# AIDynamicAction/rcognita

Measured on AMD Instinct MI355X. Metric: env-control-steps/sec (whole node), 3wrobot Nactor=10, higher is better.
Workload: dtype f64

## Files before the change

### include/rcg.h

```cpp
#ifndef RCG_H
#define RCG_H

#include <stdint.h>

#ifdef __cplusplus
extern "C" {
#endif

#define RCG_VERSION 124

#define RCG_MAX_DS 5
#define RCG_MAX_DU 2
#define RCG_MAX_CHI 7
#define RCG_MAX_PARS 5
#define RCG_MAX_DC 35
#define RCG_MAX_ROW 64
#define RCG_MAX_NACTOR 4096

typedef enum rcg_status {
  RCG_OK = 0,
  RCG_ERR_BAD_ARG = -1,
  RCG_ERR_HIP = -2,
  RCG_ERR_NO_DEVICE = -3,
  RCG_ERR_UNSUPPORTED = -4,
  RCG_ERR_NONFINITE = -5
} rcg_status;

typedef enum rcg_system { RCG_SYS_3WROBOT = 0, RCG_SYS_3WROBOT_NI = 1, RCG_SYS_2TANK = 2 } rcg_system;
#define RCG_SYS_USER_BASE 16
typedef enum rcg_mode { RCG_MODE_MPC = 0, RCG_MODE_RQL = 1, RCG_MODE_SQL = 2 } rcg_mode;
typedef enum rcg_stage { RCG_STAGE_QUADRATIC = 0, RCG_STAGE_BIQUADRATIC = 1 } rcg_stage;
typedef enum rcg_critic_struct {
  RCG_CRITIC_QUAD_LIN = 0,
  RCG_CRITIC_QUADRATIC = 1,
  RCG_CRITIC_QUAD_NOMIX = 2,
  RCG_CRITIC_QUAD_MIX = 3
} rcg_critic_struct;
typedef enum rcg_dtype { RCG_F32 = 0, RCG_F64 = 1 } rcg_dtype;
typedef enum rcg_where { RCG_HOST = 0, RCG_DEVICE = 1 } rcg_where;

#define RCG_FLAG_HAS_TARGET 0x1
#define RCG_FLAG_PER_ENV_PARS 0x2
#define RCG_FLAG_REF_LAG 0x4
#define RCG_FLAG_ACCUM_EVERY_SUBSTEP 0x8
#define RCG_FLAG_NO_CLIP 0x10
#define RCG_FLAG_DISTURB 0x20

typedef enum rcg_field {
  RCG_FIELD_STATE = 0,
  RCG_FIELD_ACTION = 1,
  RCG_FIELD_ACCUM = 2,
  RCG_FIELD_STEP_IDX = 3,
  RCG_FIELD_EPISODE_IDX = 4,
  RCG_FIELD_STATUS = 5,
  RCG_FIELD_PARS = 6,
  RCG_FIELD_STATE_INIT = 7,
  RCG_FIELD_STATE_PREV = 8,
  RCG_FIELD_BEST_J = 9,
  RCG_FIELD_BEST_IDX = 10,
  RCG_FIELD_W_CRITIC = 11,
  RCG_FIELD_W_PREV = 12,
  RCG_FIELD_OBS_BUF = 13,
  RCG_FIELD_ACT_BUF = 14,
  RCG_FIELD_RETURNS = 15,
  RCG_FIELD_ACTION_SQN = 16,
  RCG_FIELD_DISTURB = 17,
  RCG_FIELD_SUBSTEP_IDX = 18,
  RCG_FIELD_COUNT_ = 19
} rcg_field;

typedef struct rcg_cfg {
  int32_t struct_size;
  int32_t sys_id;
  int32_t batch;
  int32_t dtype;
  int32_t device;
  int32_t n_actor;
  int32_t mode;
  int32_t stage_obj_struct;
  int32_t critic_struct;
  int32_t n_critic;
  int32_t buffer_size;
  int32_t substeps_per_tick;
  int32_t flags;
  int32_t critic_every_ticks;
  double dt_sim;
  double sampling_time;
  double pred_step_size;
  double gamma;
  double pars[8];
  double ctrl_bnds[4];
  double R1[49];
  double R2[49];
  double target[8];
  double action_init[4];
  double w_init[40];
  double w_min[40];
  double w_max[40];
  double pars_disturb[6];
  double disturb_init[2];
  uint64_t seed;
  int64_t env_id_base;
} rcg_cfg;

typedef struct rcg_summary {
  double count;
  double sum;
  double sumsq;
  double min;
  double max;
  double n_failed;
} rcg_summary;

typedef struct rcg_handle rcg_handle;

int rcg_version(void);
const char* rcg_last_error(const rcg_handle* h);
int rcg_device_count(void);

int rcg_register_system(const char* name, const char* policy_src, int32_t ds, int32_t du, int32_t np, int32_t* sys_id);
int rcg_rtc_version(int32_t* major, int32_t* minor);
int rcg_system_info(int32_t sys_id, int32_t* ds, int32_t* du, int32_t* np, int32_t* has_jac);
int rcg_system_output_info(int32_t sys_id, int32_t* dy, int32_t* has_out, int32_t* has_out_jac);
int rcg_system_has_critic(int32_t sys_id, int32_t* has_critic);
int rcg_system_has_search(int32_t sys_id, int32_t* has_search);
int rcg_system_programs(int32_t sys_id, char* buf, int64_t cap, int64_t* need);

int rcg_create(const rcg_cfg* cfg, rcg_handle** out);
int rcg_destroy(rcg_handle* h);
int rcg_set_stream(rcg_handle* h, void* hip_stream);
int rcg_use_own_stream(rcg_handle* h);
int rcg_wait_stream(rcg_handle* h, void* producer_stream);
int rcg_release_stream(rcg_handle* h, void* consumer_stream);
int rcg_synchronize(rcg_handle* h);

int rcg_dev_alloc(rcg_handle* h, uint64_t bytes, void** dev_out);
int rcg_dev_free(rcg_handle* h, void* dev);
int rcg_memcpy_h2d(rcg_handle* h, void* dev_dst, const void* host_src, uint64_t bytes);
int rcg_memcpy_d2h(rcg_handle* h, void* host_dst, const void* dev_src, uint64_t bytes);

int rcg_set_field(rcg_handle* h, int field, const void* src, int where);
int rcg_get_field(rcg_handle* h, int field, void* dst, int where);
int64_t rcg_field_bytes(const rcg_handle* h, int field);
int rcg_field_ptr(rcg_handle* h, int field, void** dev_out);

int rcg_rhs(rcg_handle* h, const void* state, const void* action, void* dstate, void* clipped_action,
            int32_t n, int32_t clip);
int rcg_rhs_full(rcg_handle* h, const void* state, const void* disturb, const void* action, const void* xi,
                 void* dstate, void* ddisturb, void* clipped_action, int32_t n, int32_t clip);
int rcg_disturb_noise(rcg_handle* h, void* bits_out, void* xi_out);
int rcg_stage_obj(rcg_handle* h, const void* obs, const void* act, void* out, int32_t n);
int rcg_out(rcg_handle* h, const void* state, void* obs, int32_t n);
int rcg_critic(rcg_handle* h, const void* obs, const void* act, const void* w, void* out, int32_t n);
int rcg_actor_cost(rcg_handle* h, const void* cand, int32_t K, const void* obs, const void* state_sys,
                   const void* w, void* J);
int rcg_critic_cost(rcg_handle* h, const void* w, void* Jc);

int rcg_sim_step(rcg_handle* h, int32_t n_substeps);
int rcg_sim_step_h(rcg_handle* h, int32_t n_substeps, double step);
#define RCG_LOOP_DECIDE 1
#define RCG_LOOP_PUSH 2
#define RCG_LOOP_FIT 4
int rcg_loop_step(rcg_handle* h, const double* action_in, double step_h, int32_t n_substeps, int32_t flags, int32_t iters,
                  double* out);
int rcg_loop_step_begin(rcg_handle* h, const double* action_in, double step_h, int32_t n_substeps, int32_t flags, int32_t iters);
int rcg_loop_step_end(rcg_handle* h, double* out);
int rcg_actor_argmin(rcg_handle* h, const void* cand, int32_t K, const void* obs, const void* state_sys,
                     void* action, void* best_J, int32_t* best_idx);
int rcg_control_tick(rcg_handle* h, const void* cand, int32_t K);
int rcg_control_ticks(rcg_handle* h, int32_t T, int32_t K);
int rcg_control_tick_n(rcg_handle* h, const void* cand, int32_t K, int32_t T);
int rcg_set_tick_parts(rcg_handle* h, int32_t parts);
int rcg_join(rcg_handle* h);
int rcg_actor_optimize(rcg_handle* h, int32_t iters, const void* obs, const void* state_sys, const void* u_init,
                       void* u_opt, void* action, void* best_J, int32_t* n_iter);
int rcg_set_optimizer(rcg_handle* h, int32_t memory);
int rcg_set_optimizer_tol(rcg_handle* h, double ftol);
int rcg_control_tick_opt(rcg_handle* h, int32_t iters, int32_t warm_start);
int rcg_actor_search(rcg_handle* h, int32_t K, int32_t rounds, const void* obs, const void* state_sys, const void* centre,
                     void* u_best, void* action, void* best_J, int32_t* best_idx);
int rcg_control_tick_search(rcg_handle* h, int32_t K, int32_t rounds, int32_t warm_start);
int rcg_candidates_sample(rcg_handle* h, void* cand, int32_t K, int32_t round, const void* centre);
int rcg_nominal_action(rcg_handle* h, const void* obs, void* action, void* lyap, int32_t n, double ctrl_gain,
                       const double* ctrl_pars, int32_t clip);
int rcg_nominal_theta(rcg_handle* h, const void* obs, void* theta, int32_t n);
int rcg_control_tick_nominal(rcg_handle* h, double ctrl_gain, const double* ctrl_pars);
int rcg_critic_update(rcg_handle* h, int32_t do_fit);
int rcg_critic_fit(rcg_handle* h);
int rcg_episode_reset(rcg_handle* h);
int rcg_episode_stats(rcg_handle* h, int32_t from_accum, void* returns_out, rcg_summary* out);

int64_t rcg_tick_count(const rcg_handle* h);
int rcg_set_tick_count(rcg_handle* h, int64_t ticks);

typedef enum rcg_kernel { RCG_KERNEL_ACTOR = 0, RCG_KERNEL_SIM = 1, RCG_KERNEL_CRITIC = 2, RCG_KERNEL_COUNT_ = 3 } rcg_kernel;
#define RCG_PROFILE_PAUSE 0x80
int rcg_profile(rcg_handle* h, int32_t kernel_mask);
int rcg_profile_read(rcg_handle* h, int32_t kernel, double* total_ms, int64_t* launches);
int rcg_profile_samples(rcg_handle* h, int32_t kernel, double* ms_out, int64_t cap, int64_t* n_out);

typedef enum rcg_kernel_id {
  RCG_KID_NONE = 0,
  RCG_KID_ACTOR = 1,
  RCG_KID_ACTOR_DMA = 2,
  RCG_KID_TICKS = 3,
  RCG_KID_ACTOR_OPT = 4,
  RCG_KID_NOMINAL = 5,
  RCG_KID_SIM = 6,
  RCG_KID_SIM_V = 7,
  RCG_KID_SIM_DIST = 8,
  RCG_KID_CRITIC_FIT = 9,
  RCG_KID_ACTOR_DMA_PACKED = 10,
  RCG_KID_ACTOR_SEARCH = 11,
  RCG_KID_COUNT_ = 12
} rcg_kernel_id;
int rcg_last_launch(const rcg_handle* h, int32_t kind, int32_t* kernel_id, int32_t* variant, int32_t* envs_per_wave);
int rcg_last_launch_zero_w(const rcg_handle* h, int32_t kind, uint32_t* mask);
const char* rcg_kernel_name(int32_t kernel_id);

#ifdef __cplusplus
}
#endif
#endif
```

### rcognita_amd/_native.py

```python
from __future__ import annotations

import ctypes as C
import os
import sys

_HERE = os.path.dirname(os.path.abspath(__file__))
LIB_PATH = os.path.join(_HERE, "lib", "librcg.so")

RCG_VERSION = 124
OK, ERR_BAD_ARG, ERR_HIP, ERR_NO_DEVICE, ERR_UNSUPPORTED, ERR_NONFINITE = 0, -1, -2, -3, -4, -5
SYS_3WROBOT, SYS_3WROBOT_NI, SYS_2TANK = 0, 1, 2
MODE_MPC, MODE_RQL, MODE_SQL = 0, 1, 2
STAGE_QUADRATIC, STAGE_BIQUADRATIC = 0, 1
CRITIC_QUAD_LIN, CRITIC_QUADRATIC, CRITIC_QUAD_NOMIX, CRITIC_QUAD_MIX = 0, 1, 2, 3
F32, F64 = 0, 1
HOST, DEVICE = 0, 1
FLAG_HAS_TARGET, FLAG_PER_ENV_PARS, FLAG_REF_LAG, FLAG_ACCUM_EVERY_SUBSTEP, FLAG_NO_CLIP = 1, 2, 4, 8, 16
FLAG_DISTURB = 32
DIM_DISTURB = {0: 2, 1: 2, 2: 1}

(FIELD_STATE, FIELD_ACTION, FIELD_ACCUM, FIELD_STEP_IDX, FIELD_EPISODE_IDX, FIELD_STATUS, FIELD_PARS,
 FIELD_STATE_INIT, FIELD_STATE_PREV, FIELD_BEST_J, FIELD_BEST_IDX, FIELD_W_CRITIC, FIELD_W_PREV, FIELD_OBS_BUF,
 FIELD_ACT_BUF, FIELD_RETURNS, FIELD_ACTION_SQN, FIELD_DISTURB, FIELD_SUBSTEP_IDX) = range(19)
FIELD_COUNT = 19

MODE_IDS = {"MPC": MODE_MPC, "RQL": MODE_RQL, "SQL": MODE_SQL}
STAGE_IDS = {"quadratic": STAGE_QUADRATIC, "biquadratic": STAGE_BIQUADRATIC}
CRITIC_IDS = {"quad-lin": CRITIC_QUAD_LIN, "quadratic": CRITIC_QUADRATIC, "quad-nomix": CRITIC_QUAD_NOMIX,
              "quad-mix": CRITIC_QUAD_MIX}
SYS_IDS = {"3wrobot": SYS_3WROBOT, "3wrobotNI": SYS_3WROBOT_NI, "2tank": SYS_2TANK}
SYS_DIMS = {SYS_3WROBOT: (5, 2, 2), SYS_3WROBOT_NI: (3, 2, 0), SYS_2TANK: (2, 1, 5)}
SYS_DY = {}
SYS_USER_BASE = 16
MAX_DS, MAX_DU, MAX_PARS = 5, 2, 5

SYMBOLS = [
    "rcg_version", "rcg_last_error", "rcg_device_count", "rcg_create", "rcg_destroy", "rcg_set_stream", "rcg_use_own_stream",
    "rcg_synchronize", "rcg_dev_alloc", "rcg_dev_free", "rcg_memcpy_h2d", "rcg_memcpy_d2h", "rcg_set_field",
    "rcg_get_field", "rcg_field_bytes", "rcg_field_ptr", "rcg_rhs", "rcg_stage_obj", "rcg_critic",
    "rcg_actor_cost", "rcg_critic_cost", "rcg_sim_step", "rcg_sim_step_h", "rcg_actor_argmin", "rcg_control_tick",
    "rcg_critic_update", "rcg_control_ticks", "rcg_control_tick_n", "rcg_actor_optimize", "rcg_control_tick_opt", "rcg_nominal_action",
    "rcg_control_tick_nominal", "rcg_rhs_full", "rcg_disturb_noise", "rcg_episode_reset", "rcg_episode_stats", "rcg_tick_count", "rcg_set_tick_count", "rcg_profile", "rcg_profile_read",
    "rcg_profile_samples", "rcg_last_launch", "rcg_kernel_name", "rcg_wait_stream", "rcg_nominal_theta", "rcg_set_optimizer", "rcg_set_optimizer_tol", "rcg_set_tick_parts", "rcg_join", "rcg_loop_step", "rcg_loop_step_begin", "rcg_loop_step_end",
    "rcg_actor_search", "rcg_control_tick_search", "rcg_candidates_sample", "rcg_release_stream",
    "rcg_register_system", "rcg_rtc_version", "rcg_system_info", "rcg_system_output_info", "rcg_out",
    "rcg_system_has_critic", "rcg_system_programs", "rcg_critic_fit", "rcg_last_launch_zero_w", "rcg_system_has_search",
]
KERNEL_ACTOR, KERNEL_SIM, KERNEL_CRITIC = 0, 1, 2
(KID_NONE, KID_ACTOR, KID_ACTOR_DMA, KID_TICKS, KID_ACTOR_OPT, KID_NOMINAL, KID_SIM, KID_SIM_V, KID_SIM_DIST,
 KID_CRITIC_FIT, KID_ACTOR_DMA_PACKED, KID_ACTOR_SEARCH) = range(12)
DMA_MPC_G1, DMA_MPC, DMA_RQL_0, DMA_SQL_0 = 0, 1, 2, 6
LOOP_DECIDE, LOOP_PUSH, LOOP_FIT = 1, 2, 4
DMA_RQL_GEN_0 = 12
DMA_MPC_GEND, DMA_MPC_GENF = 10, 11


class RcgCfg(C.Structure):

    _fields_ = [
        ("struct_size", C.c_int32), ("sys_id", C.c_int32), ("batch", C.c_int32), ("dtype", C.c_int32),
        ("device", C.c_int32), ("n_actor", C.c_int32), ("mode", C.c_int32), ("stage_obj_struct", C.c_int32),
        ("critic_struct", C.c_int32), ("n_critic", C.c_int32), ("buffer_size", C.c_int32),
        ("substeps_per_tick", C.c_int32), ("flags", C.c_int32), ("critic_every_ticks", C.c_int32),
        ("dt_sim", C.c_double), ("sampling_time", C.c_double), ("pred_step_size", C.c_double), ("gamma", C.c_double),
        ("pars", C.c_double * 8), ("ctrl_bnds", C.c_double * 4), ("R1", C.c_double * 49), ("R2", C.c_double * 49),
        ("target", C.c_double * 8), ("action_init", C.c_double * 4), ("w_init", C.c_double * 40),
        ("w_min", C.c_double * 40), ("w_max", C.c_double * 40),
        ("pars_disturb", C.c_double * 6), ("disturb_init", C.c_double * 2), ("seed", C.c_uint64),
        ("env_id_base", C.c_int64),
    ]


class RcgSummary(C.Structure):
    _fields_ = [("count", C.c_double), ("sum", C.c_double), ("sumsq", C.c_double), ("min", C.c_double),
                ("max", C.c_double), ("n_failed", C.c_double)]


class NativeError(RuntimeError):
    def __init__(self, code, msg):
        super().__init__(f"librcg error {code}: {msg}")
        self.code = code


_lib = None


def use_library(path):
    global LIB_PATH
    if _lib is not None:
        raise RuntimeError("use_library: librcg is already loaded")
    LIB_PATH = os.path.abspath(path)


def lib():
    global _lib
    if _lib is not None:
        return _lib
    if not os.path.exists(LIB_PATH):
        raise ImportError(
            f"{LIB_PATH} not found: build the HIP library first (`make lib` at the repo root, or "
            "`python -c 'import __graft_entry__ as g; g.build()'`).  rcognita_amd has no CPU fallback."
        )
    torch = sys.modules.get("torch")
    if torch is not None and torch.cuda.is_available() and not torch.cuda.is_initialized():
        torch.cuda.init()
    L = C.CDLL(LIB_PATH)
    vp, i32, i64, u64 = C.c_void_p, C.c_int32, C.c_int64, C.c_uint64
    sig = {
        "rcg_version": (C.c_int, []),
        "rcg_last_error": (C.c_char_p, [vp]),
        "rcg_device_count": (C.c_int, []),
        "rcg_create": (C.c_int, [C.POINTER(RcgCfg), C.POINTER(vp)]),
        "rcg_destroy": (C.c_int, [vp]),
        "rcg_set_stream": (C.c_int, [vp, vp]),
        "rcg_use_own_stream": (C.c_int, [vp]),
        "rcg_synchronize": (C.c_int, [vp]),
        "rcg_dev_alloc": (C.c_int, [vp, u64, C.POINTER(vp)]),
        "rcg_dev_free": (C.c_int, [vp, vp]),
        "rcg_memcpy_h2d": (C.c_int, [vp, vp, vp, u64]),
        "rcg_memcpy_d2h": (C.c_int, [vp, vp, vp, u64]),
        "rcg_set_field": (C.c_int, [vp, C.c_int, vp, C.c_int]),
        "rcg_get_field": (C.c_int, [vp, C.c_int, vp, C.c_int]),
        "rcg_field_bytes": (i64, [vp, C.c_int]),
        "rcg_field_ptr": (C.c_int, [vp, C.c_int, C.POINTER(vp)]),
        "rcg_rhs": (C.c_int, [vp, vp, vp, vp, vp, i32, i32]),
        "rcg_stage_obj": (C.c_int, [vp, vp, vp, vp, i32]),
        "rcg_critic": (C.c_int, [vp, vp, vp, vp, vp, i32]),
        "rcg_actor_cost": (C.c_int, [vp, vp, i32, vp, vp, vp, vp]),
        "rcg_critic_cost": (C.c_int, [vp, vp, vp]),
        "rcg_sim_step": (C.c_int, [vp, i32]),
        "rcg_sim_step_h": (C.c_int, [vp, i32, C.c_double]),
        "rcg_actor_argmin": (C.c_int, [vp, vp, i32, vp, vp, vp, vp, vp]),
        "rcg_control_tick": (C.c_int, [vp, vp, i32]),
        "rcg_critic_update": (C.c_int, [vp, i32]),
        "rcg_control_ticks": (C.c_int, [vp, i32, i32]),
        "rcg_control_tick_n": (C.c_int, [vp, vp, i32, i32]),
        "rcg_actor_optimize": (C.c_int, [vp, i32, vp, vp, vp, vp, vp, vp, vp]),
        "rcg_control_tick_opt": (C.c_int, [vp, i32, i32]),
        "rcg_set_optimizer": (C.c_int, [vp, i32]),
        "rcg_set_tick_parts": (C.c_int, [vp, i32]),
        "rcg_set_optimizer_tol": (C.c_int, [vp, C.c_double]),
        "rcg_loop_step_begin": (C.c_int, [vp, vp, C.c_double, i32, i32, i32]),
        "rcg_loop_step_end": (C.c_int, [vp, vp]),
        "rcg_loop_step": (C.c_int, [vp, vp, C.c_double, i32, i32, i32, vp]),
        "rcg_join": (C.c_int, [vp]),
        "rcg_actor_search": (C.c_int, [vp, i32, i32, vp, vp, vp, vp, vp, vp, vp]),
        "rcg_control_tick_search": (C.c_int, [vp, i32, i32, i32]),
        "rcg_candidates_sample": (C.c_int, [vp, vp, i32, i32, vp]),
        "rcg_nominal_action": (C.c_int, [vp, vp, vp, vp, i32, C.c_double, C.POINTER(C.c_double), i32]),
        "rcg_control_tick_nominal": (C.c_int, [vp, C.c_double, C.POINTER(C.c_double)]),
        "rcg_nominal_theta": (C.c_int, [vp, vp, vp, i32]),
        "rcg_rhs_full": (C.c_int, [vp, vp, vp, vp, vp, vp, vp, vp, i32, i32]),
        "rcg_disturb_noise": (C.c_int, [vp, vp, vp]),
        "rcg_episode_reset": (C.c_int, [vp]),
        "rcg_episode_stats": (C.c_int, [vp, i32, vp, C.POINTER(RcgSummary)]),
        "rcg_tick_count": (i64, [vp]),
        "rcg_set_tick_count": (C.c_int, [vp, i64]),
        "rcg_profile": (C.c_int, [vp, i32]),
        "rcg_profile_read": (C.c_int, [vp, i32, C.POINTER(C.c_double), C.POINTER(i64)]),
        "rcg_profile_samples": (C.c_int, [vp, i32, C.POINTER(C.c_double), i64, C.POINTER(i64)]),
        "rcg_last_launch": (C.c_int, [vp, i32, C.POINTER(i32), C.POINTER(i32), C.POINTER(i32)]),
        "rcg_last_launch_zero_w": (C.c_int, [vp, i32, C.POINTER(C.c_uint32)]),
        "rcg_kernel_name": (C.c_char_p, [i32]),
        "rcg_wait_stream": (C.c_int, [vp, vp]),
        "rcg_release_stream": (C.c_int, [vp, vp]),
        "rcg_register_system": (C.c_int, [C.c_char_p, C.c_char_p, i32, i32, i32, C.POINTER(i32)]),
        "rcg_rtc_version": (C.c_int, [C.POINTER(i32), C.POINTER(i32)]),
        "rcg_system_info": (C.c_int, [i32, C.POINTER(i32), C.POINTER(i32), C.POINTER(i32), C.POINTER(i32)]),
        "rcg_system_output_info": (C.c_int, [i32, C.POINTER(i32), C.POINTER(i32), C.POINTER(i32)]),
        "rcg_out": (C.c_int, [vp, vp, vp, i32]),
        "rcg_system_has_critic": (C.c_int, [i32, C.POINTER(i32)]),
        "rcg_system_has_search": (C.c_int, [i32, C.POINTER(i32)]),
        "rcg_critic_fit": (C.c_int, [vp]),
        "rcg_system_programs": (C.c_int, [i32, C.c_char_p, i64, C.POINTER(i64)]),
    }
    for name, (res, args) in sig.items():
        fn = getattr(L, name)
        fn.restype = res
        fn.argtypes = args
    if L.rcg_version() != RCG_VERSION:
        raise ImportError(f"librcg.so version {L.rcg_version()} != binding version {RCG_VERSION}; rebuild")
    _lib = L
    return L


def last_error(handle=None) -> str:
    return lib().rcg_last_error(handle).decode("utf-8", "replace")


def check(rc, handle=None, allow=()):
    if rc != OK and rc not in allow:
        raise NativeError(rc, last_error(handle))
    return rc


def register_system(name: str, src: str, ds: int, du: int, np: int) -> dict:
    import time

    L = lib()
    sid = C.c_int32(-1)
    t0 = time.perf_counter()
    check(L.rcg_register_system(name.encode(), src.encode(), int(ds), int(du), int(np), C.byref(sid)))
    seconds = time.perf_counter() - t0
    SYS_DIMS[sid.value] = (int(ds), int(du), int(np))
    a, b = C.c_int32(0), C.c_int32(0)
    check(L.rcg_rtc_version(C.byref(a), C.byref(b)))
    jac = C.c_int32(0)
    check(L.rcg_system_info(sid.value, None, None, None, C.byref(jac)))
    dy, has_out, has_out_jac = C.c_int32(0), C.c_int32(0), C.c_int32(0)
    check(L.rcg_system_output_info(sid.value, C.byref(dy), C.byref(has_out), C.byref(has_out_jac)))
    SYS_DY[sid.value] = dy.value
    crit = C.c_int32(0)
    check(L.rcg_system_has_critic(sid.value, C.byref(crit)))
    srch = C.c_int32(0)
    check(L.rcg_system_has_search(sid.value, C.byref(srch)))
    return {"sys_id": sid.value, "name": name, "seconds": seconds, "hiprtc": (a.value, b.value), "has_jac": bool(jac.value),
            "dy": dy.value, "has_out": bool(has_out.value), "has_out_jac": bool(has_out_jac.value),
            "has_critic": bool(crit.value), "has_search": bool(srch.value)}


def system_programs(sys_id: int) -> list:
    L = lib()
    need = C.c_int64(0)
    check(L.rcg_system_programs(int(sys_id), None, 0, C.byref(need)))
    buf = C.create_string_buffer(max(int(need.value), 1))
    check(L.rcg_system_programs(int(sys_id), buf, len(buf), None))
    return [tuple(line.split("\t", 1)) for line in buf.value.decode().splitlines() if line]


def sys_dy(sys_id: int) -> int:
    return SYS_DY.get(int(sys_id), SYS_DIMS[int(sys_id)][0])
```

### rcognita_amd/csrc/rcg_actor_dma.hpp

```cpp
#pragma once
#include <hip/hip_ext.h>
#include "rcg_kernels.hpp"

#ifndef RCG_DMA_AUX
#define RCG_DMA_AUX 2
#endif
#ifndef RCG_DMA_PRIO
#define RCG_DMA_PRIO 0
#endif

namespace rcg {

enum : int {
  DMA_MPC_G1 = 0,
  DMA_MPC = 1,
  DMA_RQL_0 = 2 ,
  DMA_SQL_0 = 6 ,
  DMA_MPC_GEND = 10,
  DMA_MPC_GENF = 11,
  DMA_RQL_GEN_0 = 12 ,
  DMA_VARIANTS = 16
};
__host__ __device__ constexpr bool dma_is_sql(int v) { return v >= DMA_SQL_0 && v < DMA_MPC_GEND; }
__host__ __device__ constexpr bool dma_is_rql(int v) { return (v >= DMA_RQL_0 && v < DMA_SQL_0) || v >= DMA_RQL_GEN_0; }
__host__ __device__ constexpr int dma_cs(int v) {
  return v >= DMA_RQL_GEN_0 ? v - DMA_RQL_GEN_0 : (dma_is_sql(v) ? v - DMA_SQL_0 : (dma_is_rql(v) ? v - DMA_RQL_0 : 0));
}

__host__ __device__ constexpr int dma_dc(int cs, int ds, int du) {
  return cs == RCG_CRITIC_QUAD_LIN ? (ds + du) * (ds + du + 1) / 2 + (ds + du)
                                   : (cs == RCG_CRITIC_QUADRATIC ? (ds + du) * (ds + du + 1) / 2
                                                                 : (cs == RCG_CRITIC_QUAD_NOMIX ? ds + du : ds + ds * du + du));
}

__host__ __device__ constexpr int dma_wslot(int esz, int variant, int ds, int du) {
  const int dcmax = (dma_is_sql(variant) || dma_is_rql(variant)) ? dma_dc(dma_cs(variant), ds, du) : 0;
  return dcmax > 9 ? ((dcmax * esz + 15) / 16) * 16 : 0;
}

__device__ __forceinline__ void wave_argmin(float& bestJ, int& bestI) {
  const unsigned long long wkey = wave_min_u64(((unsigned long long)float_order_key(bestJ) << 32) | (unsigned)bestI);
  bestJ = float_from_order_key((unsigned)(wkey >> 32));
  bestI = (int)(unsigned)wkey;
}
__device__ __forceinline__ void wave_argmin(double& bestJ, int& bestI) {
  for (int m = 1; m < 64; m <<= 1) {
    const double oJ = __shfl_xor(bestJ, m, 64);
    const int oI = __shfl_xor(bestI, m, 64);
    if ((oJ < bestJ) || (oJ == bestJ && oI < bestI)) {
      bestJ = oJ;
      bestI = oI;
    }
  }
}
__device__ __forceinline__ void wave_argmin_reg(float& bestJ, int& bestI) { wave_argmin(bestJ, bestI); }
__device__ __forceinline__ void wave_argmin_reg(double& bestJ, int& bestI) {
#ifdef RCG_AB_SHFL_ARGMIN64
  wave_argmin(bestJ, bestI);
#else
  const double Jmin = wave_min_f64(bestJ);
  bestI = (int)wave_min_u32(bestJ == Jmin ? (unsigned)bestI : 0x7fffffffu);
  bestJ = Jmin;
#endif
}

template <typename Sys, typename real>
__host__ __device__ constexpr unsigned dma_zw_preset() {
  if constexpr (sizeof(real) == 8 && !HasOut<Sys>::value)
    return Sys::ZW_PRESET;
  else
    return 0u;
}

template <typename S, typename = void>
struct HasPrefix {
  static constexpr bool value = false;
};
template <typename S>
struct HasPrefix<S, void_t_<decltype(S::PFX_FREE)>> {
  static constexpr bool value = true;
};
template <typename S>
constexpr unsigned pfx_free() {
  if constexpr (HasPrefix<S>::value)
    return S::PFX_FREE;
  else
    return 0u;
}
template <typename S>
constexpr int pfx_heading() {
  if constexpr (HasPrefix<S>::value)
    return S::PFX_HEADING;
  else
    return -1;
}

__device__ __forceinline__ float uniform_r(float v) {
  return __uint_as_float((unsigned)__builtin_amdgcn_readfirstlane((int)__float_as_uint(v)));
}
__device__ __forceinline__ double uniform_r(double v) {
  const unsigned long long b = (unsigned long long)__double_as_longlong(v);
  const unsigned lo = (unsigned)__builtin_amdgcn_readfirstlane((int)(unsigned)b);
  const unsigned hi = (unsigned)__builtin_amdgcn_readfirstlane((int)(unsigned)(b >> 32));
  return __longlong_as_double((long long)(((unsigned long long)hi << 32) | lo));
}

template <int J, int NP, int SZ, int PIECE>
__device__ __forceinline__ void dma_pieces(const unsigned char* g, unsigned off, unsigned char* l) {
  typedef __attribute__((address_space(3))) void lds_void;
  typedef const __attribute__((address_space(1))) void glb_void;
  if constexpr (J < NP) {
    constexpr int BASE = (J * PIECE / 4096) * 4096;
    const unsigned char* const gb = g + (off + (unsigned)BASE);
    if constexpr (SZ == 16)
      __builtin_amdgcn_global_load_lds((glb_void*)gb, (lds_void*)(l + BASE), 16, J * PIECE - BASE, RCG_DMA_AUX);
    else
      __builtin_amdgcn_global_load_lds((glb_void*)gb, (lds_void*)(l + BASE), 4, J * PIECE - BASE, RCG_DMA_AUX);
    dma_pieces<J + 1, NP, SZ, PIECE>(g, off, l);
  }
}

__host__ __device__ constexpr int dma_rpl(int r, int esz) { return r * esz <= 24 ? 4 : (r * esz <= 32 ? 2 : 1); }

template <typename Sys, typename real, int R, bool TGT, int V, unsigned ZW = 0u>
__global__ __launch_bounds__(256) void k_actor_dma(const ActorArgs<real> A, const KParams<real> P) {
  constexpr int DS = Sys::DS, DY = sys_dy<Sys>(), DU = Sys::DU, NCHI = DY + DU, NP = Sys::NP;
  constexpr bool OUT = HasOut<Sys>::value;
  constexpr bool G1 = V == DMA_MPC_G1, SQL = dma_is_sql(V), RQL = dma_is_rql(V), CRIT = RQL || SQL;
  constexpr bool GEND = V == DMA_MPC_GEND, GENF = V == DMA_MPC_GENF, GEN = GEND || GENF;
  constexpr bool GENR = V >= DMA_RQL_GEN_0;
  static_assert(!(GEN || GENR) || TGT, "the generic-cost instances subtract a target (zeros for a handle without one)");
  static_assert(ZW == 0u || (G1 && sizeof(real) == 8 && !OUT && ZW == Sys::ZW_PRESET),
                "the zero-weight instance: DMA_MPC_G1, float64, no output map, the policy's preset mask");
  constexpr int CS = dma_cs(V);
  constexpr int DCMAX = CRIT ? dma_dc(CS, DY, DU) : 1;
  constexpr int ESZ = (int)sizeof(real);
  constexpr int WSLOT = dma_wslot(ESZ, V, DY, DU);
  constexpr bool WLDS = WSLOT > 0;
  constexpr int WREG = WLDS ? 1 : DCMAX;
  static_assert(R % DU == 0 && R >= DU && R <= 40, "row = N*du reals, at most 40 (f32: 160 bytes, f64: 320)");
  constexpr int N = R / DU;
  constexpr bool PFX = HasPrefix<Sys>::value && !OUT;
  constexpr unsigned FREE = PFX ? pfx_free<Sys>() : 0u;
  constexpr int HD = PFX ? pfx_heading<Sys>() : -1;
  constexpr bool TRIG0 = PFX && HD >= 0 && N >= 2;
  constexpr bool TRIG1 = TRIG0 && ((FREE >> (HD >= 0 ? HD : 0)) & 1u) && N >= 3;
  constexpr int RPL = dma_rpl(R, ESZ), TROWS = 64 * RPL;
  constexpr int TILE = TROWS * R * ESZ;
  constexpr int NFULL = TILE / 1024, NREM = (TILE % 1024) / 256;
  static_assert(NFULL * 1024 + NREM * 256 == TILE, "a tile is a whole number of 256-B segments");
  extern __shared__ __attribute__((aligned(16))) unsigned char smem_raw[];
  typedef __attribute__((address_space(3))) void lds_void;
  typedef const __attribute__((address_space(1))) void glb_void;

  const int lane = threadIdx.x & 63;
  const int wave_in_wg = __builtin_amdgcn_readfirstlane((int)(threadIdx.x >> 6));
  const long wave = (long)blockIdx.x * (blockDim.x >> 6) + wave_in_wg;
  const long B = P.B;
  const int K = A.K;
  const int T = (K + TROWS - 1) / TROWS;
  const int rem_rows = K % TROWS;
  const long env_hi = A.env_hi > 0 ? A.env_hi : B;
  const long env0 = A.env_lo + wave * A.gpw;
  if (env0 >= env_hi) return;
  const long env1 = env0 + A.gpw < env_hi ? env0 + A.gpw : env_hi;
  const int n_tiles = (int)(env1 - env0) * T;

  unsigned char* const tile = smem_raw + (size_t)wave_in_wg * TILE;
  const size_t env_stride = (size_t)K * (R * ESZ);
  const unsigned char* envb;
  {
    const unsigned long long p = (unsigned long long)(reinterpret_cast<const unsigned char*>(A.cand) + (size_t)env0 * env_stride);
    const unsigned lo = (unsigned)__builtin_amdgcn_readfirstlane((int)(unsigned)p);
    const unsigned hi = (unsigned)__builtin_amdgcn_readfirstlane((int)(unsigned)(p >> 32));
    envb = reinterpret_cast<const unsigned char*>(((unsigned long long)hi << 32) | lo);
  }
  const unsigned lane16 = (unsigned)lane * 16u, lane4 = (unsigned)lane * 4u;
  const int jspan = A.jwave ? A.gpw * K : K;
  real* const jstage = reinterpret_cast<real*>(smem_raw + (size_t)4 * TILE + (size_t)4 * WSLOT) + (size_t)wave_in_wg * jspan;
  real* const wl = reinterpret_cast<real*>(smem_raw + (size_t)4 * TILE + (size_t)wave_in_wg * WSLOT);

  auto issue_tile = [&](const unsigned char* g, int rows) {
    unsigned o16 = lane16, o4 = lane4;
    if (NFULL) asm volatile("" : "+v"(o16));
    if (NREM) asm volatile("" : "+v"(o4));
    asm volatile("" : "+s"(rows));
    if (rows == TROWS) {
      dma_pieces<0, NFULL, 16, 1024>(g, o16, tile);
      dma_pieces<0, NREM, 4, 256>(g + NFULL * 1024, o4, tile + NFULL * 1024);
    } else {
      const int vb = rows * (R * ESZ);
#pragma unroll
      for (int j = 0; j < NFULL; ++j)
        if ((int)o16 < vb - j * 1024)
          __builtin_amdgcn_global_load_lds((glb_void*)(g + (o16 + (unsigned)(j * 1024))), (lds_void*)(tile + j * 1024), 16, 0,
                                           RCG_DMA_AUX);
#pragma unroll
      for (int j = 0; j < NREM; ++j)
        if ((int)o4 < vb - (NFULL * 1024 + j * 256))
          __builtin_amdgcn_global_load_lds((glb_void*)(g + (o4 + (unsigned)(NFULL * 1024 + j * 256))),
                                           (lds_void*)(tile + NFULL * 1024 + j * 256), 4, 0, RCG_DMA_AUX);
    }
  };
  const int last_rows = rem_rows ? rem_rows : TROWS;
  auto rows_of = [&](int tt) -> int { return tt == T - 1 ? last_rows : TROWS; };

  real y0[DY], yn[sys_dxy<Sys>()], x0[DS], xn[DS], pv[NP > 0 ? NP : 1], pn[NP > 0 ? NP : 1], wc[WREG], wn[WREG];
  real wnl = 0;
  const bool lag = A.state_sys != A.obs;
#pragma unroll
  for (int i = 0; i < NP; ++i) pn[i] = P.pars[i];
#pragma unroll
  for (int i = 0; i < WREG; ++i) wn[i] = wc[i] = 0;
  constexpr int dc_rt = CRIT ? DCMAX : 0;
  auto fetch_env = [&](long b) {
    if (RCG_DBG(A, 4)) {
#pragma unroll
      for (int c = 0; c < sys_dxy<Sys>(); ++c) yn[c] = (real)0.5;
#pragma unroll
      for (int c = 0; c < DS; ++c) xn[c] = (real)0.5;
      return;
    }
    if constexpr (OUT) {
      load_obs_raw<Sys, real>(A.obs, A.obs_x, B, b, yn);
    } else {
#pragma unroll
      for (int c = 0; c < DS; ++c) yn[c] = A.obs[(long)c * B + b];
    }
    if (lag) {
#pragma unroll
      for (int c = 0; c < DS; ++c) xn[c] = A.state_sys[(long)c * B + b];
    }
    if (A.pars_env) {
#pragma unroll
      for (int i = 0; i < NP; ++i) pn[i] = A.pars_env[(long)i * B + b];
    }
    if (CRIT && WLDS) {
      if (lane < dc_rt) wnl = A.w[(long)lane * B + b];
    } else if (CRIT) {
#pragma unroll
      for (int i = 0; i < WREG; ++i) wn[i] = A.w[(long)i * B + b];
    }
  };

  constexpr bool TRI = GENF || GENR;
  constexpr int NSYM = TRI ? sym_len<NCHI>() : 1;
  real S1[NSYM], S2[NSYM];
  const bool biq = (GEN || GENR) && (P.stage_kind & STAGE_BIQUAD);
  const bool full_rt = GENF || (GENR && (P.stage_kind & STAGE_FULL));
  if constexpr (TRI) {
    if (full_rt) {
      load_sym<NCHI, real>(P.Rfull, S1);
    } else {
#pragma unroll
      for (int i = 0; i < NSYM; ++i) S1[i] = 0;
    }
    if (full_rt && biq) {
      load_sym<NCHI, real>(P.Rfull + 49, S2);
    } else {
#pragma unroll
      for (int i = 0; i < NSYM; ++i) S2[i] = 0;
    }
  }
  auto gen_stage = [&](const real* chi) -> real {
    real q;
    if (TRI && full_rt)
      q = quad_sym<NCHI, real>(S1, chi);
    else
      q = stage_diag<NCHI, real>(P, chi);
    if (biq) {
      real c2[NCHI];
#pragma unroll
      for (int i = 0; i < NCHI; ++i) c2[i] = chi[i] * chi[i];
      real q4;
      if (TRI && full_rt) {
        q4 = quad_sym<NCHI, real>(S2, c2);
      } else {
        q4 = 0;
#pragma unroll
        for (int i = 0; i < NCHI; ++i) q4 = fma_r(P.R2d[i] * c2[i], c2[i], q4);
      }
      q = q4 + q;
    }
    return q;
  };

  fetch_env(env0);
  issue_tile(envb, rows_of(0));

  const real h = P.h_pred;
  long b = env0;
  int t = 0;
  const bool env_pars = A.pars_env != nullptr;
  auto pre_env = Sys::template prepare<real>(pn);
  real x1s[DS], trig0[2] = {0, 0}, trig1[2] = {0, 0}, Sini[DY];
  real zw0 = 0;
#pragma unroll
  for (int c = 0; c < DS; ++c) x1s[c] = 0;
#pragma unroll
  for (int c = 0; c < DY; ++c) Sini[c] = 0;
  real bestJ = inf_r<real>();
  int bestI = 0x7fffffff;
  real bu[DU];
#pragma unroll
  for (int c = 0; c < DU; ++c) bu[c] = 0;
  real resJ = 0, resAcc = 0, resU[DU];
  int resI = 0;
#pragma unroll
  for (int c = 0; c < DU; ++c) resU[c] = 0;

  auto adopt_regs = [&]() {
    if constexpr (OUT) {
#pragma unroll
      for (int c = 0; c < DS; ++c) x0[c] = lag ? xn[c] : yn[c];
#pragma unroll
      for (int i = 0; i < NP; ++i) pv[i] = pn[i];
      pre_env = Sys::template prepare<real>(pv);
      obs_of_raw<Sys, real>(pre_env, A.obs_x, yn, y0);
    } else {
#pragma unroll
      for (int c = 0; c < DS; ++c) {
        y0[c] = yn[c];
        x0[c] = lag ? xn[c] : yn[c];
      }
    }
    if (CRIT && WLDS) {
      if (lane < dc_rt) wl[lane] = wnl;
      asm volatile("s_waitcnt lgkmcnt(0)" ::: "memory");
      __builtin_amdgcn_wave_barrier();
    } else if (CRIT) {
#pragma unroll
      for (int i = 0; i < WREG; ++i) wc[i] = wn[i];
    }
  };
  auto adopt_rest = [&]() {
    if constexpr (PFX) {
#pragma unroll
      for (int c = 0; c < DS; ++c) x0[c] = uniform_r(x0[c]);
      if constexpr (TRIG0) {
        sincos_sel<real, true>(x0[HD], &trig0[0], &trig0[1]);
        if constexpr (FREE != 0) {
          real uz[DU], d[DS];
#pragma unroll
          for (int c = 0; c < DU; ++c) uz[c] = 0;
          Sys::template rhs_trig<real>(pre_env, x0, uz, trig0[0], trig0[1], d);
#pragma unroll
          for (int c = 0; c < DS; ++c)
            if ((FREE >> c) & 1u) x1s[c] = uniform_r(fma_r(h, d[c], x0[c]));
        }
        if constexpr (TRIG1) {
          sincos_sel<real, true>(x1s[HD], &trig1[0], &trig1[1]);
          trig1[0] = uniform_r(trig1[0]);
          trig1[1] = uniform_r(trig1[1]);
        }
        if constexpr (FREE == 0) {
          trig0[0] = uniform_r(trig0[0]);
          trig0[1] = uniform_r(trig0[1]);
        }
      }
      if constexpr (G1) {
#pragma unroll
        for (int c = 0; c < DY; ++c) {
          if ((ZW >> c) & 1u) continue;
          const real chi0 = TGT ? y0[c] - P.target[c] : y0[c];
          real a = fma_r(chi0, chi0, (real)0);
          if (N >= 2 && ((FREE >> c) & 1u)) {
            const real chi1 = TGT ? x1s[c] - P.target[c] : x1s[c];
            a = fma_r(chi1, chi1, a);
          }
          Sini[c] = uniform_r(a);
        }
      }
    }
    if constexpr (ZW != 0u) {
      real z = 0;
#pragma unroll
      for (int i = 0; i < DY; ++i)
        if ((ZW >> i) & 1u) z = fma_r(P.R1d[i], y0[i] * y0[i], z);
      zw0 = uniform_r(z);
    }
    bestJ = inf_r<real>();
    bestI = 0x7fffffff;
  };
  const bool adopt_early = OUT || T == 1;

  for (int g = 0; g < n_tiles; ++g) {
    if (t == 0) {
      if constexpr (!OUT) {
        if (env_pars) pre_env = Sys::template prepare<real>(pn);
      }
      if (adopt_early) adopt_regs();
    }
    if constexpr (RCG_DMA_PRIO > 0 && ESZ == 8) __builtin_amdgcn_s_setprio(RCG_DMA_PRIO);
    asm volatile("s_waitcnt vmcnt(0)" ::: "memory");
    real rows[RPL][R];
#pragma unroll
    for (int j = 0; j < RPL; ++j) {
      const real* const myrow = reinterpret_cast<const real*>(tile) + (j * 64 + lane) * R;
#pragma unroll
      for (int i = 0; i < R; ++i) rows[j][i] = myrow[i];
    }
    asm volatile("s_waitcnt lgkmcnt(0)" ::: "memory");
    __builtin_amdgcn_wave_barrier();
    if (g + 1 < n_tiles) {
      if (t == T - 1) {
        fetch_env(b + 1);
        envb += env_stride;
        issue_tile(envb, rows_of(0));
      } else {
        issue_tile(envb + (size_t)(t + 1) * TILE, rows_of(t + 1));
      }
    }
    if constexpr (RCG_DMA_PRIO > 0 && ESZ == 8) __builtin_amdgcn_s_setprio(0);
    if (t == 0) {
      if (!adopt_early) adopt_regs();
      adopt_rest();
    }

#pragma unroll
    for (int j = 0; j < RPL; ++j) {
      const real* const cur = rows[j];
      real x[DS], y[DY];
      if constexpr (OUT) {
#pragma unroll
        for (int c = 0; c < DS; ++c) x[c] = x0[c];
#pragma unroll
        for (int c = 0; c < DY; ++c) y[c] = y0[c];
      } else {
#pragma unroll
        for (int c = 0; c < DS; ++c) {
          x[c] = x0[c];
          y[c] = y0[c];
        }
      }
      real J = 0, gk = 1;
      real S[NCHI];
#pragma unroll
      for (int i = 0; i < NCHI; ++i) S[i] = (PFX && G1 && i < DY) ? Sini[i < DY ? i : 0] : (real)0;
      real Phi[SQL ? DCMAX : 1];
#pragma unroll
      for (int i = 0; i < (SQL ? DCMAX : 1); ++i) Phi[i] = 0;
      auto wget = [&](int i) -> real { return WLDS ? wl[i] : wc[WLDS ? 0 : i]; };
      if (RCG_DBG(A, 1)) {
#pragma unroll
        for (int i = 0; i < R; ++i) J += cur[i];
      } else {
#pragma unroll
        for (int kk = 0; kk < N; ++kk) {
          if (kk > 0) {
            real d[DS];
            if constexpr (TRIG0 || TRIG1) {
              if (kk == 1 && TRIG0)
                Sys::template rhs_trig<real>(pre_env, x, &cur[(kk - 1) * DU], trig0[0], trig0[1], d);
              else if (kk == 2 && TRIG1)
                Sys::template rhs_trig<real>(pre_env, x, &cur[(kk - 1) * DU], trig1[0], trig1[1], d);
              else
                Sys::template rhs<real, true>(pre_env, x, &cur[(kk - 1) * DU], d);
            } else {
              Sys::template rhs<real, true>(pre_env, x, &cur[(kk - 1) * DU], d);
            }
#pragma unroll
            for (int c = 0; c < DS; ++c) {
              if (PFX && kk == 1 && ((FREE >> c) & 1u))
                x[c] = x1s[c];
              else
                x[c] = fma_r(h, d[c], x[c]);
              if constexpr (!OUT) y[c] = x[c];
            }
            if constexpr (OUT) sys_out<Sys, real, true>(pre_env, x, y);
          }
          real chi[NCHI];
#pragma unroll
          for (int c = 0; c < DY; ++c) chi[c] = TGT ? y[c] - P.target[c] : y[c];
#pragma unroll
          for (int c = 0; c < DU; ++c) chi[DY + c] = cur[kk * DU + c];
          if (G1) {
#pragma unroll
            for (int i = 0; i < NCHI; ++i) {
              if (PFX && i < DY && (kk == 0 || (kk == 1 && ((FREE >> i) & 1u)))) continue;
              if ((ZW >> i) & 1u) continue;
              S[i] = fma_r(chi[i], chi[i], S[i]);
            }
          } else if (SQL) {
            critic_phi_accum<DY, DU, real>(chi, y, &cur[kk * DU], Phi, CS);
          } else if (RQL && kk == N - 1) {
            J += critic_with<DY, DU, real>(chi, y, &cur[kk * DU], wget, CS);
          } else if (GEN || GENR) {
            J = fma_r(gk, gen_stage(chi), J);
            gk *= P.gamma;
          } else {
            J = fma_r(gk, stage_diag<NCHI, real>(P, chi), J);
            gk *= P.gamma;
          }
        }
        if (G1) {
#pragma unroll
          for (int i = 0; i < NCHI; ++i)
            if (!((ZW >> i) & 1u)) J = fma_r(P.R1d[i], S[i], J);
          if constexpr (ZW != 0u) {
#pragma unroll
            for (int i = 0; i < DY; ++i)
              if ((ZW >> i) & 1u) J = fma_r(P.R1d[i], y[i] * y[i], J);
#pragma unroll
            for (int c = 0; c < DU; ++c)
              if ((ZW >> (DY + c)) & 1u) J = fma_r(P.R1d[DY + c], cur[(N - 1) * DU + c] * cur[(N - 1) * DU + c], J);
            J += zw0;
          }
        }
        if (SQL) {
#pragma unroll
          for (int i = 0; i < DCMAX; ++i) J = fma_r(wget(i), Phi[i], J);
        }
      }

      const int k = t * TROWS + j * 64 + lane;
      const bool has_row = k < K;
      if (A.J && has_row) jstage[(A.jwave ? (int)(b - env0) * K : 0) + k] = J;
      const real Jc = (J != J) ? inf_r<real>() : J;
      if (has_row && (Jc < bestJ || bestI == 0x7fffffff)) {
        bestJ = Jc;
        bestI = k;
#pragma unroll
        for (int c = 0; c < DU; ++c) bu[c] = cur[c];
      }
    }

    if (A.J && (A.jwave ? g == n_tiles - 1 : t == T - 1)) {
      asm volatile("s_waitcnt lgkmcnt(0)" ::: "memory");
      __builtin_amdgcn_wave_barrier();
      real* const Jout = A.J + (A.jwave ? env0 : b) * K;
      const int n = A.jwave ? (int)(env1 - env0) * K : K;
      const int nbytes = n * ESZ;
      if ((nbytes & 1023) == 0) {
        const unsigned char* const src = reinterpret_cast<const unsigned char*>(jstage);
        unsigned char* const dst = reinterpret_cast<unsigned char*>(Jout);
        for (int i = lane * 16; i < nbytes; i += 1024)
          __builtin_nontemporal_store(*reinterpret_cast<const v4f*>(src + i), reinterpret_cast<v4f*>(dst + i));
      } else {
        for (int i = lane; i < n; i += 64) Jout[i] = jstage[i];
      }
    }
    if (++t == T) {
      if (RCG_DBG(A, 2)) {
        if (bestJ == (real)-12345.678f) A.best_J[b] = bestJ;
        if (lane == 0 && A.step_idx) atomicAdd(&A.step_idx[b], 1);
        t = 0;
        ++b;
        continue;
      }
      if constexpr (ZW != 0u)
        wave_argmin_reg(bestJ, bestI);
      else
        wave_argmin(bestJ, bestI);
      const int wl = __builtin_amdgcn_readfirstlane(bestI & 63);
#pragma unroll
      for (int c = 0; c < DU; ++c) bu[c] = readlane_r(bu[c], wl);
      real acc_inc = 0;
      if (A.accum) {
        real chi[NCHI];
#pragma unroll
        for (int c = 0; c < DY; ++c) chi[c] = TGT ? y0[c] - P.target[c] : y0[c];
#pragma unroll
        for (int c = 0; c < DU; ++c) chi[DY + c] = bu[c];
        acc_inc = ((GEN || GENR || SQL) ? stage_any<NCHI, real>(P, chi) : stage_diag<NCHI, real>(P, chi)) * P.sampling_time;
      }
      if (lane == (int)(b - env0)) {
        resJ = bestJ;
        resI = bestI;
        resAcc = acc_inc;
#pragma unroll
        for (int c = 0; c < DU; ++c) resU[c] = bu[c];
      }
      t = 0;
      ++b;
    }
  }

  if (lane < (int)(env1 - env0) && !RCG_DBG(A, 2)) {
    const long bb = env0 + lane;
#pragma unroll
    for (int c = 0; c < DU; ++c)
      if (A.action_out) A.action_out[(long)c * B + bb] = resU[c];
    if (A.best_J) A.best_J[bb] = resJ;
    if (A.best_idx) A.best_idx[bb] = resI;
    if (A.accum) atomicAdd(&A.accum[bb], resAcc);
    if (A.step_idx) atomicAdd(&A.step_idx[bb], 1);
  }
}

#if !defined(__HIPCC_RTC__)
template <typename real>
static inline unsigned dma_zero_w(unsigned preset, int variant, const ActorArgs<real>& A, const KParams<real>& P) {
#ifdef RCG_AB_NO_DMA_ZW
  return 0u;
#else
  return (preset != 0u && variant == DMA_MPC_G1 && !A.J && (P.zero_w & preset) == preset) ? preset : 0u;
#endif
}
template <typename Sys, typename real, int GROUP>
bool launch_dma(int r, int variant, dim3 grid, dim3 block, size_t lds, hipStream_t s, const ActorArgs<real>& A,
                const KParams<real>& P, hipEvent_t ev_a, hipEvent_t ev_b);
#endif

template <typename real>
constexpr int dma_max_row() {
  return 40;
}

}
```

### rcognita_amd/csrc/rcg_api.hip

```cpp
#include <cstdarg>
#include <cstdio>
#include <cstdlib>
#include <cstring>

#include "rcg_disturb.hpp"
#include "rcg_handle.hpp"
#include "rcg_search.hpp"

using namespace rcg;

static thread_local std::string g_err = "";

int rcg_fail(rcg_handle* h, int code, const char* fmt, ...) {
  char buf[512];
  va_list ap;
  va_start(ap, fmt);
  vsnprintf(buf, sizeof buf, fmt, ap);
  va_end(ap);
  if (h)
    h->err = buf;
  else
    g_err = buf;
  return code;
}
// ... 82 lines not shown
  bool full = false;
  const bool biq = c.stage_obj_struct == RCG_STAGE_BIQUADRATIC;
  for (int i = 0; i < n; ++i)
    for (int j = 0; j < n; ++j) {
      rfull_host[i * n + j] = (real)c.R1[i * n + j];
      rfull_host[49 + i * n + j] = biq ? (real)c.R2[i * n + j] : (real)0;
      if (i != j && (c.R1[i * n + j] != 0.0 || (biq && c.R2[i * n + j] != 0.0))) full = true;
    }
  for (int i = 0; i < n; ++i) {
    P->R1d[i] = (real)c.R1[i * n + i];
    P->R2d[i] = biq ? (real)c.R2[i * n + i] : (real)0;
  }
  for (int i = 0; i < h->dy; ++i) P->target[i] = (c.flags & RCG_FLAG_HAS_TARGET) ? (real)c.target[i] : (real)0;
  P->gamma = (real)c.gamma;
  P->h_pred = (real)c.pred_step_size;
  P->dt_sim = (real)c.dt_sim;
  P->sampling_time = (real)c.sampling_time;
  P->B = c.batch;
  P->n_actor = c.n_actor;
  P->mode = c.mode;
  P->critic_struct = c.critic_struct;
  P->dc = h->dc;
  P->n_critic = c.n_critic;
  P->buffer_size = c.buffer_size;
  P->stage_kind = (full ? STAGE_FULL : 0) | (biq ? STAGE_BIQUAD : 0);
  P->zero_w = 0u;
  if (!full && !biq)
    for (int i = 0; i < n; ++i)
      if (c.R1[i * n + i] == 0.0) P->zero_w |= 1u << i;
  P->has_target = (c.flags & RCG_FLAG_HAS_TARGET) ? 1 : 0;
  P->clip = (c.flags & RCG_FLAG_NO_CLIP) ? 0 : 1;
  P->per_env_pars = (c.flags & RCG_FLAG_PER_ENV_PARS) ? 1 : 0;
  P->ref_lag = (c.flags & RCG_FLAG_REF_LAG) ? 1 : 0;
  P->accum_every_substep = (c.flags & RCG_FLAG_ACCUM_EVERY_SUBSTEP) ? 1 : 0;
}

template <typename real>
__global__ void k_fill(real* p, long n, real v) {
  const long i = (long)blockIdx.x * blockDim.x + threadIdx.x;
  if (i < n) p[i] = v;
}

template <typename real>
static int fill_rows(rcg_handle* h, void* base, int rows, const double* vals) {
  const long B = h->cfg.batch;
  for (int r = 0; r < rows; ++r)
    hipLaunchKernelGGL(k_fill<real>, dim3(blocks_for(B)), dim3(256), 0, h->stream, (real*)base + (long)r * B, B,
                       (real)vals[r]);
  HIPCHK(h, hipGetLastError());
  return RCG_OK;
}

extern "C" {

int rcg_version(void) { return RCG_VERSION; }

const char* rcg_last_error(const rcg_handle* h) { return h ? h->err.c_str() : g_err.c_str(); }

int rcg_system_info(int32_t sys_id, int32_t* ds, int32_t* du, int32_t* np, int32_t* has_jac) {
  RtcDims d{0, 0, 0, true, 0, false, false};
  if (sys_id >= 0 && sys_id <= 2)
    d = RtcDims{kDims[sys_id][0], kDims[sys_id][1], kDims[sys_id][2], true, kDims[sys_id][0], false, false};
  else if (!(sys_id >= RCG_SYS_USER_BASE && rtc_lookup(sys_id, &d)))
    return rcg_fail(nullptr, RCG_ERR_BAD_ARG, "rcg_system_info: bad sys_id %d", sys_id);
  if (ds) *ds = d.ds;
  if (du) *du = d.du;
  if (np) *np = d.np;
  if (has_jac) *has_jac = d.has_jac ? 1 : 0;
  return RCG_OK;
}

int rcg_system_output_info(int32_t sys_id, int32_t* dy, int32_t* has_out, int32_t* has_out_jac) {
  RtcDims d{0, 0, 0, false, 0, false, false};
  if (sys_id >= 0 && sys_id <= 2)
    d.dy = kDims[sys_id][0];
  else if (!(sys_id >= RCG_SYS_USER_BASE && rtc_lookup(sys_id, &d)))
    return rcg_fail(nullptr, RCG_ERR_BAD_ARG, "rcg_system_output_info: bad sys_id %d", sys_id);
  if (dy) *dy = d.dy;
  if (has_out) *has_out = d.has_out ? 1 : 0;
  if (has_out_jac) *has_out_jac = d.has_out_jac ? 1 : 0;
  return RCG_OK;
}

int rcg_device_count(void) {
  int n = 0;
  if (hipGetDeviceCount(&n) != hipSuccess) return 0;
  return n;
}

int rcg_create(const rcg_cfg* cfg, rcg_handle** out) {
  if (!cfg || !out) return rcg_fail(nullptr, RCG_ERR_BAD_ARG, "rcg_create: null argument");
  *out = nullptr;
  if (cfg->struct_size != (int32_t)sizeof(rcg_cfg))
    return rcg_fail(nullptr, RCG_ERR_BAD_ARG, "rcg_create: struct_size %d != sizeof(rcg_cfg) %zu (ABI mismatch)",
                    cfg->struct_size, sizeof(rcg_cfg));
  RtcDims rd{0, 0, 0, false, 0, false, false};
  const RtcSystem* rtc = cfg->sys_id >= RCG_SYS_USER_BASE ? rtc_lookup(cfg->sys_id, &rd) : nullptr;
  if ((cfg->sys_id < 0 || cfg->sys_id > 2) && !rtc)
    return rcg_fail(nullptr, RCG_ERR_BAD_ARG, "rcg_create: bad sys_id %d", cfg->sys_id);
  if (cfg->batch < 1) return rcg_fail(nullptr, RCG_ERR_BAD_ARG, "rcg_create: batch must be >= 1");
  if (cfg->dtype != RCG_F32 && cfg->dtype != RCG_F64) return rcg_fail(nullptr, RCG_ERR_BAD_ARG, "rcg_create: bad dtype");
  if (cfg->mode < 0 || cfg->mode > 2) return rcg_fail(nullptr, RCG_ERR_BAD_ARG, "rcg_create: bad mode %d", cfg->mode);
  if (cfg->stage_obj_struct < 0 || cfg->stage_obj_struct > 1)
    return rcg_fail(nullptr, RCG_ERR_BAD_ARG, "rcg_create: bad stage_obj_struct");
  if (cfg->critic_struct < 0 || cfg->critic_struct > 3)
    return rcg_fail(nullptr, RCG_ERR_BAD_ARG, "rcg_create: bad critic_struct");
  const int ds = rtc ? rd.ds : kDims[cfg->sys_id][0], du = rtc ? rd.du : kDims[cfg->sys_id][1], np = rtc ? rd.np : kDims[cfg->sys_id][2];
  if (rtc && cfg->mode != RCG_MODE_MPC && !rd.has_critic)
    return rcg_fail(nullptr, RCG_ERR_UNSUPPORTED, "rcg_create: a system registered at run time runs MPC only (no RQL / SQL critic kernels)");
  if (dim_critic(cfg->critic_struct, rtc ? rd.dy : ds, du) > RCG_MAX_DC)
    return rcg_fail(nullptr, RCG_ERR_UNSUPPORTED, "rcg_create: dim_critic %d (dim_output %d, dim_input %d) beyond the limit %d",
                    dim_critic(cfg->critic_struct, rtc ? rd.dy : ds, du), rtc ? rd.dy : ds, du, RCG_MAX_DC);
  if (rtc && (cfg->flags & RCG_FLAG_DISTURB))
    return rcg_fail(nullptr, RCG_ERR_UNSUPPORTED, "rcg_create: a system registered at run time has no disturbance model");
  if (cfg->n_actor < 1 || cfg->n_actor > RCG_MAX_NACTOR)
    return rcg_fail(nullptr, RCG_ERR_BAD_ARG, "rcg_create: need 1 <= Nactor <= %d", RCG_MAX_NACTOR);
  if (cfg->substeps_per_tick < 1)
    return rcg_fail(nullptr, RCG_ERR_BAD_ARG, "rcg_create: substeps_per_tick must be >= 1");
  if (cfg->buffer_size < 0) return rcg_fail(nullptr, RCG_ERR_BAD_ARG, "rcg_create: buffer_size < 0");
  if (cfg->mode != RCG_MODE_MPC && cfg->buffer_size < 2)
    return rcg_fail(nullptr, RCG_ERR_BAD_ARG, "rcg_create: RQL/SQL need buffer_size >= 2");

  int ndev = 0;
  if (hipGetDeviceCount(&ndev) != hipSuccess || ndev < 1)
    return rcg_fail(nullptr, RCG_ERR_NO_DEVICE, "rcg_create: no HIP device visible; librcg has no CPU fallback");
  if (cfg->device < 0 || cfg->device >= ndev)
    return rcg_fail(nullptr, RCG_ERR_BAD_ARG, "rcg_create: device %d out of range (%d visible)", cfg->device, ndev);
  DeviceGuard dev_guard(cfg->device);
  {
    int cur = -1;
    if (hipGetDevice(&cur) != hipSuccess || cur != cfg->device)
      return rcg_fail(nullptr, RCG_ERR_HIP, "rcg_create: cannot make device %d current", cfg->device);
  }

  rcg_handle* h = new rcg_handle();
  h->cfg = *cfg;
  h->ds = ds;
  h->du = du;
  h->np = np;
  h->rtc_has_out = rtc && rd.has_out;
  h->dy = rtc ? rd.dy : ds;
  h->nchi = h->dy + du;
  h->dc = dim_critic(cfg->critic_struct, h->dy, du);
  h->esz = cfg->dtype == RCG_F64 ? 8 : 4;
  h->stream = nullptr;
  h->own_stream = nullptr;
  h->bounce = nullptr;
  h->tick_parts = 0;
  h->split_stream[0] = h->split_stream[1] = nullptr;
  h->split_fork = h->split_join[0] = h->split_join[1] = nullptr;
  h->split_pending = false;
  h->sub_lo = h->sub_hi = 0;
  h->probe = 0;
  h->d_summary = nullptr;
  h->d_const = nullptr;
  h->fit_scratch = nullptr;
  h->fit_scratch_bytes = 0;
  h->loop_seq = 0;
  h->loop_io.on = false;
  h->loop_pending = false;
  h->loop_pin = nullptr;
  h->sqn_alt = nullptr;
  h->loop_pending_decided = false;
  h->prof_mask = 0;
  h->prof_stride = 1;
  memset(h->prof_seen, 0, sizeof h->prof_seen);
  h->tick_count = 0;
  h->opt_ftol = 0.0;
  h->opt_memory = -1;
  h->cur_a = h->cur_b = nullptr;
  h->scope_due = false;
  h->order_ev = nullptr;
  h->release_ev = nullptr;
  memset(h->last, 0, sizeof h->last);
  h->rtc = rtc;
  h->sys = rtc ? &kVtRtc
               : (cfg->sys_id == RCG_SYS_3WROBOT ? &kVt3WRobot : (cfg->sys_id == RCG_SYS_3WROBOT_NI ? &kVt3WRobotNI : &kVt2Tank));
  memset(h->prof_ms, 0, sizeof h->prof_ms);
  memset(h->prof_n, 0, sizeof h->prof_n);
  memset(h->f, 0, sizeof h->f);
  memset(h->fbytes, 0, sizeof h->fbytes);
  if (h->cfg.buffer_size > 0) {
    if (h->cfg.n_critic > h->cfg.buffer_size - 1) h->cfg.n_critic = h->cfg.buffer_size - 1;
  }
  bool any_bnd = false;
  for (int i = 0; i < 2 * du; ++i) any_bnd = any_bnd || cfg->ctrl_bnds[i] != 0.0;
  if (!any_bnd) h->cfg.flags |= RCG_FLAG_NO_CLIP;

  if (hipMalloc(&h->d_const, kConstBytes) != hipSuccess) {
    rcg_fail(nullptr, RCG_ERR_HIP, "rcg_create: allocating the constant block");
    delete h;
    return RCG_ERR_HIP;
  }
  {
    unsigned char blk[kConstBytes];
    memset(blk, 0, sizeof blk);
    build_params<float>(h, &h->p32, reinterpret_cast<float*>(blk), reinterpret_cast<const float*>(h->d_const));
    build_params<double>(h, &h->p64, reinterpret_cast<double*>(blk + kConstR64),
                         reinterpret_cast<const double*>((unsigned char*)h->d_const + kConstR64));
    double* wc = reinterpret_cast<double*>(blk + kConstW);
    for (int i = 0; i < 40; ++i) {
      wc[i] = cfg->w_init[i];
      wc[40 + i] = cfg->w_min[i];
      wc[80 + i] = cfg->w_max[i];
    }
    hipError_t er = hipMemcpy(h->d_const, blk, sizeof blk, hipMemcpyHostToDevice);
    if (er != hipSuccess) {
      rcg_fail(nullptr, RCG_ERR_HIP, "rcg_create: uploading the constant block: %s", hipGetErrorString(er));
      rcg_destroy(h);
      return RCG_ERR_HIP;
    }
  }

  const size_t B = (size_t)cfg->batch, e = h->esz;
  h->fbytes[RCG_FIELD_STATE] = ds * B * e;
  h->fbytes[RCG_FIELD_ACTION] = du * B * e;
  h->fbytes[RCG_FIELD_ACCUM] = B * e;
  h->fbytes[RCG_FIELD_STEP_IDX] = B * 4;
  h->fbytes[RCG_FIELD_EPISODE_IDX] = B * 4;
  h->fbytes[RCG_FIELD_STATUS] = B * 4;
  h->fbytes[RCG_FIELD_PARS] = ((cfg->flags & RCG_FLAG_PER_ENV_PARS) && np > 0) ? np * B * e : 0;
  h->fbytes[RCG_FIELD_STATE_INIT] = ds * B * e;
  h->fbytes[RCG_FIELD_STATE_PREV] = ds * B * e;
  h->fbytes[RCG_FIELD_BEST_J] = B * e;
  h->fbytes[RCG_FIELD_BEST_IDX] = B * 4;
  h->fbytes[RCG_FIELD_RETURNS] = B * e;
  h->fbytes[RCG_FIELD_ACTION_SQN] = (size_t)cfg->n_actor * du * B * e;
  const int dd = cfg->sys_id == RCG_SYS_2TANK ? 1 : 2;
  if (cfg->flags & RCG_FLAG_DISTURB) {
    h->fbytes[RCG_FIELD_DISTURB] = dd * B * e;
    h->fbytes[RCG_FIELD_SUBSTEP_IDX] = B * 4;
  }
  if (cfg->buffer_size > 0) {
    h->fbytes[RCG_FIELD_W_CRITIC] = h->dc * B * e;
    h->fbytes[RCG_FIELD_W_PREV] = h->dc * B * e;
    h->fbytes[RCG_FIELD_OBS_BUF] = (size_t)cfg->buffer_size * h->dy * B * e;
    h->fbytes[RCG_FIELD_ACT_BUF] = (size_t)cfg->buffer_size * du * B * e;
  }
  for (int i = 0; i < RCG_FIELD_COUNT_; ++i) {
    if (!h->fbytes[i]) continue;
    hipError_t er = hipMalloc(&h->f[i], h->fbytes[i]);
    if (er == hipSuccess) er = hipMemsetAsync(h->f[i], 0, h->fbytes[i], h->stream);
    if (er != hipSuccess) {
      rcg_fail(nullptr, RCG_ERR_HIP, "rcg_create: allocating field %d (%zu bytes): %s", i, h->fbytes[i],
               hipGetErrorString(er));
      rcg_destroy(h);
      return RCG_ERR_HIP;
    }
  }
  if (hipMalloc((void**)&h->d_summary, 6 * sizeof(double)) != hipSuccess) {
    rcg_fail(nullptr, RCG_ERR_HIP, "rcg_create: allocating summary scratch");
    rcg_destroy(h);
    return RCG_ERR_HIP;
  }
  int rc = RCG_OK;
  const bool crit = cfg->buffer_size > 0;
  if (cfg->dtype == RCG_F64) {
    rc = fill_rows<double>(h, h->f[RCG_FIELD_ACTION], du, cfg->action_init);
    if (rc == RCG_OK && crit) rc = fill_rows<double>(h, h->f[RCG_FIELD_W_CRITIC], h->dc, cfg->w_init);
    if (rc == RCG_OK && crit) rc = fill_rows<double>(h, h->f[RCG_FIELD_W_PREV], h->dc, cfg->w_init);
  } else {
    rc = fill_rows<float>(h, h->f[RCG_FIELD_ACTION], du, cfg->action_init);
    if (rc == RCG_OK && crit) rc = fill_rows<float>(h, h->f[RCG_FIELD_W_CRITIC], h->dc, cfg->w_init);
    if (rc == RCG_OK && crit) rc = fill_rows<float>(h, h->f[RCG_FIELD_W_PREV], h->dc, cfg->w_init);
  }
  if (rc == RCG_OK && (cfg->flags & RCG_FLAG_DISTURB))
    rc = cfg->dtype == RCG_F64 ? fill_rows<double>(h, h->f[RCG_FIELD_DISTURB], dd, cfg->disturb_init)
                               : fill_rows<float>(h, h->f[RCG_FIELD_DISTURB], dd, cfg->disturb_init);
  if (rc == RCG_OK && hipStreamSynchronize(h->stream) != hipSuccess)
    rc = rcg_fail(h, RCG_ERR_HIP, "rcg_create: synchronising the initial fills");
  if (rc != RCG_OK) {
    g_err = h->err;
    rcg_destroy(h);
    return rc;
  }
  *out = h;
  return RCG_OK;
}

int rcg_destroy(rcg_handle* h) {
  DeviceGuard dev_guard(h);
  if (!h) return RCG_OK;
  (void)hipStreamSynchronize(h->stream);
  for (int i = 0; i < RCG_FIELD_COUNT_; ++i)
    if (h->f[i]) (void)hipFree(h->f[i]);
  if (h->own_stream) (void)hipStreamDestroy(h->own_stream);
  for (int p = 0; p < 2; ++p) {
    if (h->split_stream[p]) {
      (void)hipStreamSynchronize(h->split_stream[p]);
      (void)hipStreamDestroy(h->split_stream[p]);
    }
    if (h->split_join[p]) (void)hipEventDestroy(h->split_join[p]);
  }
  if (h->split_fork) (void)hipEventDestroy(h->split_fork);
  if (h->bounce) (void)hipHostFree(h->bounce);
  if (h->loop_pin) (void)hipHostFree(h->loop_pin);
  if (h->sqn_alt) (void)hipFree(h->sqn_alt);
  if (h->d_summary) (void)hipFree(h->d_summary);
  if (h->d_const) (void)hipFree(h->d_const);
  if (h->fit_scratch) (void)hipFree(h->fit_scratch);
  for (auto& p : h->ev_pending) {
    (void)hipEventDestroy(p.a);
    (void)hipEventDestroy(p.b);
  }
  for (auto e : h->ev_free) (void)hipEventDestroy(e);
  if (h->order_ev) (void)hipEventDestroy(h->order_ev);
  if (h->release_ev) (void)hipEventDestroy(h->release_ev);
  delete h;
  return RCG_OK;
}

int rcg_set_stream(rcg_handle* h, void* hip_stream) {
  DeviceGuard dev_guard(h);
  if (!h) return RCG_ERR_BAD_ARG;
  if ((hipStream_t)hip_stream == h->stream) return RCG_OK;
  (void)prof_drain(h);
  HIPCHK(h, hipStreamSynchronize(h->stream));
  h->stream = (hipStream_t)hip_stream;
  return RCG_OK;
}

int rcg_use_own_stream(rcg_handle* h) {
  DeviceGuard dev_guard(h);
  if (!h) return RCG_ERR_BAD_ARG;
  if (!h->own_stream) HIPCHK(h, hipStreamCreateWithFlags(&h->own_stream, hipStreamNonBlocking));
  return rcg_set_stream(h, (void*)h->own_stream);
}

int rcg_wait_stream(rcg_handle* h, void* producer_stream) {
  DeviceGuard dev_guard(h);
  if (!h) return RCG_ERR_BAD_ARG;
  if ((hipStream_t)producer_stream == h->stream) return RCG_OK;
  if (!h->order_ev) HIPCHK(h, hipEventCreateWithFlags(&h->order_ev, hipEventDisableTiming));
  HIPCHK(h, hipEventRecord(h->order_ev, (hipStream_t)producer_stream));
  HIPCHK(h, hipStreamWaitEvent(h->stream, h->order_ev, 0));
  return RCG_OK;
}

int rcg_release_stream(rcg_handle* h, void* consumer_stream) {
  DeviceGuard dev_guard(h);
  if (!h) return RCG_ERR_BAD_ARG;
  if ((hipStream_t)consumer_stream == h->stream) return RCG_OK;
  if (!h->release_ev) HIPCHK(h, hipEventCreateWithFlags(&h->release_ev, hipEventDisableTiming));
  HIPCHK(h, hipEventRecord(h->release_ev, h->stream));
  HIPCHK(h, hipStreamWaitEvent((hipStream_t)consumer_stream, h->release_ev, 0));
  return RCG_OK;
}

int rcg_synchronize(rcg_handle* h) {
  DeviceGuard dev_guard(h);
  if (!h) return RCG_ERR_BAD_ARG;
  HIPCHK(h, hipStreamSynchronize(h->stream));
  return RCG_OK;
}

int rcg_dev_alloc(rcg_handle* h, uint64_t bytes, void** dev_out) {
  DeviceGuard dev_guard(h);
  if (!h || !dev_out) return RCG_ERR_BAD_ARG;
  HIPCHK(h, hipMalloc(dev_out, bytes ? bytes : 16));
  return RCG_OK;
}

int rcg_dev_free(rcg_handle* h, void* dev) {
  DeviceGuard dev_guard(h);
// ... 649 lines not shown
  DeviceGuard dev_guard(h);
  if (!h || !obs || (!action && !lyap) || n < 1)
    return rcg_fail(h, RCG_ERR_BAD_ARG, "rcg_nominal_action: obs and one of action/lyap are required, n >= 1");
  return h->sys->nominal(h, obs, action, lyap, nullptr, n, ctrl_gain, ctrl_pars, clip, false);
}

int rcg_nominal_theta(rcg_handle* h, const void* obs, void* theta, int32_t n) {
  DeviceGuard dev_guard(h);
  if (!h || !obs || !theta || n < 1) return rcg_fail(h, RCG_ERR_BAD_ARG, "rcg_nominal_theta: obs, theta and n >= 1 are required");
  if (h->cfg.sys_id != RCG_SYS_3WROBOT)
    return rcg_fail(h, RCG_ERR_UNSUPPORTED, "rcg_nominal_theta: only CtrlNominal3WRobot has a theta search");
  return h->sys->nominal(h, obs, nullptr, nullptr, theta, n, 1.0, nullptr, 0, false);
}

int rcg_control_tick_nominal(rcg_handle* h, double ctrl_gain, const double* ctrl_pars) {
  DeviceGuard dev_guard(h);
  if (!h) return RCG_ERR_BAD_ARG;
  if (h->cfg.sys_id == RCG_SYS_2TANK)
    return rcg_fail(h, RCG_ERR_UNSUPPORTED, "rcg_control_tick_nominal: the reference defines no nominal controller for 2tank");
  if (h->rtc)
    return rcg_fail(h, RCG_ERR_UNSUPPORTED, "rcg_control_tick_nominal: not available for a system registered at run time");
  int rc = h->sys->sim_step(h, h->cfg.substeps_per_tick);
  if (rc) return rc;
  rc = h->sys->nominal(h, h->f[RCG_FIELD_STATE], h->f[RCG_FIELD_ACTION], nullptr, nullptr, h->cfg.batch, ctrl_gain,
                       ctrl_pars, 1, true);
  if (rc == RCG_OK) h->tick_count += 1;
  return rc;
}

int rcg_episode_reset(rcg_handle* h) {
  DeviceGuard dev_guard(h);
  if (!h) return RCG_ERR_BAD_ARG;
  const long B = h->cfg.batch;
  h->tick_count = 0;
  if (h->cfg.dtype == RCG_F64)
    hipLaunchKernelGGL((k_episode_reset<double>), dim3(blocks_for(B)), dim3(256), 0, h->stream,
                       (double*)h->f[RCG_FIELD_STATE], (double*)h->f[RCG_FIELD_STATE_PREV],
                       (const double*)h->f[RCG_FIELD_STATE_INIT], (double*)h->f[RCG_FIELD_ACTION],
                       (double*)h->f[RCG_FIELD_ACCUM], (double*)h->f[RCG_FIELD_RETURNS],
                       (int32_t*)h->f[RCG_FIELD_STEP_IDX], (int32_t*)h->f[RCG_FIELD_EPISODE_IDX],
                       (uint32_t*)h->f[RCG_FIELD_STATUS], h->ds, h->du, h->cfg.action_init[0], h->cfg.action_init[1], B);
  else
    hipLaunchKernelGGL((k_episode_reset<float>), dim3(blocks_for(B)), dim3(256), 0, h->stream,
                       (float*)h->f[RCG_FIELD_STATE], (float*)h->f[RCG_FIELD_STATE_PREV],
                       (const float*)h->f[RCG_FIELD_STATE_INIT], (float*)h->f[RCG_FIELD_ACTION],
                       (float*)h->f[RCG_FIELD_ACCUM], (float*)h->f[RCG_FIELD_RETURNS],
                       (int32_t*)h->f[RCG_FIELD_STEP_IDX], (int32_t*)h->f[RCG_FIELD_EPISODE_IDX],
                       (uint32_t*)h->f[RCG_FIELD_STATUS], h->ds, h->du, (float)h->cfg.action_init[0],
                       (float)h->cfg.action_init[1], B);
  HIPCHK(h, hipGetLastError());
  if (h->cfg.flags & RCG_FLAG_DISTURB) {
    const int dd = h->cfg.sys_id == RCG_SYS_2TANK ? 1 : 2;
    const int rc = h->cfg.dtype == RCG_F64 ? fill_rows<double>(h, h->f[RCG_FIELD_DISTURB], dd, h->cfg.disturb_init)
                                           : fill_rows<float>(h, h->f[RCG_FIELD_DISTURB], dd, h->cfg.disturb_init);
    if (rc) return rc;
    HIPCHK(h, hipMemsetAsync(h->f[RCG_FIELD_SUBSTEP_IDX], 0, h->fbytes[RCG_FIELD_SUBSTEP_IDX], h->stream));
  }
  return RCG_OK;
}

int rcg_episode_stats(rcg_handle* h, int32_t from_accum, void* returns_out, rcg_summary* out) {
  DeviceGuard dev_guard(h);
  if (!h || !out) return rcg_fail(h, RCG_ERR_BAD_ARG, "rcg_episode_stats: out is required");
  const int field = from_accum ? RCG_FIELD_ACCUM : RCG_FIELD_RETURNS;
  const long B = h->cfg.batch;
  if (h->cfg.dtype == RCG_F64)
    hipLaunchKernelGGL((k_stats<double>), dim3(1), dim3(1024), 0, h->stream, (const double*)h->f[field],
                       (const uint32_t*)h->f[RCG_FIELD_STATUS], B, h->d_summary);
  else
    hipLaunchKernelGGL((k_stats<float>), dim3(1), dim3(1024), 0, h->stream, (const float*)h->f[field],
                       (const uint32_t*)h->f[RCG_FIELD_STATUS], B, h->d_summary);
  HIPCHK(h, hipGetLastError());
  double s[6];
  HIPCHK(h, hipMemcpyAsync(s, h->d_summary, sizeof s, hipMemcpyDeviceToHost, h->stream));
  if (returns_out)
    HIPCHK(h, hipMemcpyAsync(returns_out, h->f[field], h->fbytes[field], hipMemcpyDeviceToHost, h->stream));
  HIPCHK(h, hipStreamSynchronize(h->stream));
  out->count = s[0];
  out->sum = s[1];
  out->sumsq = s[2];
  out->min = s[3];
  out->max = s[4];
  out->n_failed = s[5];
  return s[5] > 0 ? rcg_fail(h, RCG_ERR_NONFINITE, "rcg_episode_stats: %.0f env(s) hit a non-finite state", s[5])
                  : RCG_OK;
}

int64_t rcg_tick_count(const rcg_handle* h) { return h ? (int64_t)h->tick_count : -1; }

int rcg_set_tick_count(rcg_handle* h, int64_t ticks) {
  if (!h) return RCG_ERR_BAD_ARG;
  if (ticks < 0) return rcg_fail(h, RCG_ERR_BAD_ARG, "rcg_set_tick_count: ticks must be >= 0");
  h->tick_count = (long)ticks;
  return RCG_OK;
}

int rcg_profile(rcg_handle* h, int32_t enable) {
  DeviceGuard dev_guard(h);
  if (!h) return RCG_ERR_BAD_ARG;
  if (((unsigned)enable & 0xffu) == RCG_PROFILE_PAUSE) {
    h->prof_mask = 0;
    return RCG_OK;
  }
  const int drain_rc = prof_drain(h);
  h->prof_mask = (unsigned)enable & 0x7fu;
  h->prof_stride = (((unsigned)enable >> 8) & 0xfffu) ? (((unsigned)enable >> 8) & 0xfffu) : 1u;
  const unsigned skip = (unsigned)enable >> 20;
  for (int k = 0; k < RCG_KERNEL_COUNT_; ++k)
    h->prof_seen[k] = skip ? (uint64_t)h->prof_stride - (uint64_t)(skip % h->prof_stride) : 0;
  if (enable) {
    memset(h->prof_ms, 0, sizeof h->prof_ms);
    memset(h->prof_n, 0, sizeof h->prof_n);
    for (auto& v : h->prof_samples) v.clear();
  }
  return drain_rc;
}

int rcg_profile_read(rcg_handle* h, int32_t kernel, double* total_ms, int64_t* launches) {
  DeviceGuard dev_guard(h);
  if (!h || kernel < 0 || kernel >= RCG_KERNEL_COUNT_)
    return rcg_fail(h, RCG_ERR_BAD_ARG, "rcg_profile_read: bad kernel id");
  const int drain_rc = prof_drain(h);
  if (total_ms) *total_ms = h->prof_ms[kernel];
  if (launches) *launches = h->prof_n[kernel];
  return drain_rc;
}

int rcg_profile_samples(rcg_handle* h, int32_t kernel, double* ms_out, int64_t cap, int64_t* n_out) {
  DeviceGuard dev_guard(h);
  if (!h || kernel < 0 || kernel >= RCG_KERNEL_COUNT_ || cap < 0 || (cap > 0 && !ms_out))
    return rcg_fail(h, RCG_ERR_BAD_ARG, "rcg_profile_samples: bad argument");
  const int drain_rc = prof_drain(h);
  const std::vector<float>& v = h->prof_samples[kernel];
  const int64_t n = (int64_t)v.size();
  for (int64_t i = 0; i < n && i < cap; ++i) ms_out[i] = (double)v[(size_t)i];
  if (n_out) *n_out = n;
  return drain_rc;
}

int rcg_last_launch(const rcg_handle* h, int32_t kind, int32_t* kernel_id, int32_t* variant, int32_t* envs_per_wave) {
  if (!h || kind < 0 || kind >= RCG_KERNEL_COUNT_) return RCG_ERR_BAD_ARG;
  if (kernel_id) *kernel_id = h->last[kind].kernel_id;
  if (variant) *variant = h->last[kind].variant;
  if (envs_per_wave) *envs_per_wave = h->last[kind].envs_per_wave;
  return RCG_OK;
}

int rcg_last_launch_zero_w(const rcg_handle* h, int32_t kind, uint32_t* mask) {
  if (!h || !mask || kind < 0 || kind >= RCG_KERNEL_COUNT_) return RCG_ERR_BAD_ARG;
  *mask = h->last[kind].zero_w;
  return RCG_OK;
}

const char* rcg_kernel_name(int32_t kernel_id) {
  static const char* const names[RCG_KID_COUNT_] = {"none",        "k_actor",   "k_actor_dma", "k_ticks",    "k_actor_opt",
                                                    "k_nominal",   "k_sim",     "k_sim_v",     "k_sim_dist", "k_critic_fit",
                                                    "k_actor_dma_packed", "k_actor_search"};
  return (kernel_id >= 0 && kernel_id < RCG_KID_COUNT_) ? names[kernel_id] : "?";
}

}
```

### rcognita_amd/csrc/rcg_dma_launch.hpp

```cpp
#pragma once

#include "rcg_actor_dma.hpp"
#include "rcg_actor_dma_packed.hpp"

namespace rcg {

template <typename Sys, typename real, int GROUP, int R>
static bool launch_dma_r(int r, int variant, dim3 grid, dim3 block, size_t lds, hipStream_t s, const ActorArgs<real>& A,
                         const KParams<real>& P, hipEvent_t ev_a, hipEvent_t ev_b) {
  if constexpr (R > dma_max_row<real>()) {
    return false;
  } else {
    if (r != R) return launch_dma_r<Sys, real, GROUP, R + 1>(r, variant, grid, block, lds, s, A, P, ev_a, ev_b);
    if constexpr (R % Sys::DU != 0) {
      return false;
    } else {
#define RCG_DMA_LAUNCH(FN)                                                                                           \
  {                                                                                                                  \
    auto fn = FN;                                                                                                    \
    if (lds > 64 * 1024)      \
      (void)hipFuncSetAttribute(reinterpret_cast<const void*>(fn), hipFuncAttributeMaxDynamicSharedMemorySize,       \
                                (int)lds);                                                                           \
    if (ev_a)                                                                                                        \
      hipExtLaunchKernelGGL(fn, grid, block, (std::uint32_t)lds, s, ev_a, ev_b, 0, A, P);                            \
    else                                                                                                             \
      hipLaunchKernelGGL(fn, grid, block, lds, s, A, P);                                                             \
    return true;                                                                                                     \
  }
#define RCG_DMA_CASE(V) \
  case V:               \
    RCG_DMA_LAUNCH((k_actor_dma<Sys, real, R, ((V) >= DMA_MPC_GEND ? true : Sys::TGT), V>))
      if constexpr (GROUP == 0) {
        constexpr unsigned ZWP = dma_zw_preset<Sys, real>();
        if constexpr (ZWP != 0u) {
          if (dma_zero_w<real>(ZWP, variant, A, P) != 0u) RCG_DMA_LAUNCH((k_actor_dma<Sys, real, R, Sys::TGT, DMA_MPC_G1, ZWP>))
        }
        switch (variant) {
          RCG_DMA_CASE(DMA_MPC_G1)
          RCG_DMA_CASE(DMA_MPC)
        }
      } else if constexpr (GROUP == 6) {
        switch (variant) {
          RCG_DMA_CASE(DMA_MPC_GEND)
          RCG_DMA_CASE(DMA_MPC_GENF)
        }
      } else if constexpr (GROUP == 7) {
        switch (variant) {
          RCG_DMA_CASE(DMA_RQL_GEN_0 + RCG_CRITIC_QUAD_LIN)
          RCG_DMA_CASE(DMA_RQL_GEN_0 + RCG_CRITIC_QUADRATIC)
          RCG_DMA_CASE(DMA_RQL_GEN_0 + RCG_CRITIC_QUAD_NOMIX)
          RCG_DMA_CASE(DMA_RQL_GEN_0 + RCG_CRITIC_QUAD_MIX)
        }
      } else if constexpr (GROUP == 1) {
        switch (variant) {
          RCG_DMA_CASE(DMA_SQL_0 + RCG_CRITIC_QUAD_LIN)
          RCG_DMA_CASE(DMA_SQL_0 + RCG_CRITIC_QUADRATIC)
          RCG_DMA_CASE(DMA_SQL_0 + RCG_CRITIC_QUAD_NOMIX)
          RCG_DMA_CASE(DMA_SQL_0 + RCG_CRITIC_QUAD_MIX)
        }
      } else {
        switch (variant) {
          RCG_DMA_CASE(DMA_RQL_0 + RCG_CRITIC_QUAD_LIN)
          RCG_DMA_CASE(DMA_RQL_0 + RCG_CRITIC_QUADRATIC)
          RCG_DMA_CASE(DMA_RQL_0 + RCG_CRITIC_QUAD_NOMIX)
          RCG_DMA_CASE(DMA_RQL_0 + RCG_CRITIC_QUAD_MIX)
        }
      }
#undef RCG_DMA_CASE
#undef RCG_DMA_LAUNCH
      return false;
    }
  }
}

template <typename Sys, typename real, int GROUP>
bool launch_dma(int r, int variant, dim3 grid, dim3 block, size_t lds, hipStream_t s, const ActorArgs<real>& A,
                const KParams<real>& P, hipEvent_t ev_a, hipEvent_t ev_b) {
  return launch_dma_r<Sys, real, GROUP, 1>(r, variant, grid, block, lds, s, A, P, ev_a, ev_b);
}

template <typename Sys, typename real, int GROUP, int R>
static bool launch_dma_packed_r(int r, int variant, dim3 grid, dim3 block, size_t lds, hipStream_t s,
                                const ActorArgs<real>& A, const KParams<real>& P, hipEvent_t ev_a, hipEvent_t ev_b) {
  if constexpr (R > dma_max_row<real>()) {
    return false;
  } else {
    if (r != R) return launch_dma_packed_r<Sys, real, GROUP, R + 1>(r, variant, grid, block, lds, s, A, P, ev_a, ev_b);
    if constexpr (R % Sys::DU != 0) {
      return false;
    } else {
#define RCG_DMAP_CASE(V)                                                                                             \
  case V: {                                                                                                          \
    if constexpr ((V) >= DMA_RQL_0 &&                                                                                \
                  !packed_critic_ok(dma_dc(((V) >= DMA_SQL_0 ? (V)-DMA_SQL_0 : (V)-DMA_RQL_0), sys_dy<Sys>(), Sys::DU), \
                                    (int)sizeof(real))) {                                                            \
      return false;       \
    } else {                                                                                                         \
      auto fn = k_actor_dma_packed<Sys, real, R, Sys::TGT, V>;                                                       \
      if (lds > 64 * 1024)                                                                                           \
        (void)hipFuncSetAttribute(reinterpret_cast<const void*>(fn), hipFuncAttributeMaxDynamicSharedMemorySize,     \
                                  (int)lds);                                                                         \
      if (ev_a)                                                                                                      \
        hipExtLaunchKernelGGL(fn, grid, block, (std::uint32_t)lds, s, ev_a, ev_b, 0, A, P);                          \
      else                                                                                                           \
        hipLaunchKernelGGL(fn, grid, block, lds, s, A, P);                                                           \
      return true;                                                                                                   \
    }                                                                                                                \
  }
      if constexpr (GROUP == 3) {
        switch (variant) {
          RCG_DMAP_CASE(DMA_MPC_G1)
          RCG_DMAP_CASE(DMA_MPC)
        }
      } else if constexpr (GROUP == 4) {
        switch (variant) {
          RCG_DMAP_CASE(DMA_SQL_0 + RCG_CRITIC_QUAD_LIN)
          RCG_DMAP_CASE(DMA_SQL_0 + RCG_CRITIC_QUADRATIC)
          RCG_DMAP_CASE(DMA_SQL_0 + RCG_CRITIC_QUAD_NOMIX)
          RCG_DMAP_CASE(DMA_SQL_0 + RCG_CRITIC_QUAD_MIX)
        }
      } else {
        switch (variant) {
          RCG_DMAP_CASE(DMA_RQL_0 + RCG_CRITIC_QUAD_LIN)
          RCG_DMAP_CASE(DMA_RQL_0 + RCG_CRITIC_QUADRATIC)
          RCG_DMAP_CASE(DMA_RQL_0 + RCG_CRITIC_QUAD_NOMIX)
          RCG_DMAP_CASE(DMA_RQL_0 + RCG_CRITIC_QUAD_MIX)
        }
      }
#undef RCG_DMAP_CASE
      return false;
    }
  }
}

template <typename Sys, typename real, int GROUP>
bool launch_dma_packed(int r, int variant, dim3 grid, dim3 block, size_t lds, hipStream_t s, const ActorArgs<real>& A,
                       const KParams<real>& P, hipEvent_t ev_a, hipEvent_t ev_b) {
  return launch_dma_packed_r<Sys, real, GROUP, 1>(r, variant, grid, block, lds, s, A, P, ev_a, ev_b);
}

}
```

### rcognita_amd/csrc/rcg_handle.hpp

```cpp
#pragma once
#include <hip/hip_ext.h>
#include <hip/hip_runtime.h>

#include <cstdint>
#include <cstdio>
#include <cstdlib>
#include <map>
#include <string>
#include <vector>

#include "rcg_actor_opt.hpp"
#include "rcg_kernels.hpp"

struct rcg_handle {
  rcg_cfg cfg;
  int ds, du, np, dc, nchi;
  int dy;
  bool rtc_has_out;
  size_t esz;
  hipStream_t stream;
  hipStream_t own_stream;
  void* f[RCG_FIELD_COUNT_];
  size_t fbytes[RCG_FIELD_COUNT_];
  double* d_summary;
  long tick_count;
  int opt_memory;
  double opt_ftol;
  void* d_const;
  struct {
    bool on;
    const double* act_in;
    int n_substeps, dc;
    double *out, *flag, seq;
  } loop_io;
  bool loop_pending;
  int loop_pending_row;
  bool loop_pending_decided;
  void* sqn_alt;
  void* loop_pin;
  uint64_t loop_seq;
  void* fit_scratch;
  size_t fit_scratch_bytes;
  rcg::KParams<float> p32;
  rcg::KParams<double> p64;
  const struct SysVTable* sys;
  const struct RtcSystem* rtc;
  std::map<std::string, hipFunction_t> rtc_fn;
  std::string err;
  unsigned prof_mask;
  unsigned prof_stride;
  uint64_t prof_seen[RCG_KERNEL_COUNT_];
  std::vector<hipEvent_t> ev_free;
  struct Pending {
    hipEvent_t a, b;
    int kernel;
  };
  std::vector<Pending> ev_pending;
  double prof_ms[RCG_KERNEL_COUNT_];
  int64_t prof_n[RCG_KERNEL_COUNT_];
  std::vector<float> prof_samples[RCG_KERNEL_COUNT_];
  hipEvent_t cur_a, cur_b;
  bool scope_due;
  hipEvent_t order_ev;
  hipEvent_t release_ev;
  void* bounce;
  int tick_parts;
  hipStream_t split_stream[2];
  hipEvent_t split_fork, split_join[2];
  bool split_pending;
  int sub_lo, sub_hi;
  int probe;
  struct LastLaunch {
    int32_t kernel_id, variant, envs_per_wave;
    uint32_t zero_w;
  } last[RCG_KERNEL_COUNT_];
};
static constexpr size_t kProfMaxSamples = 65536;

static constexpr size_t kBounceBytes = 16384;
static constexpr int kSplitMinBatch = 65536;
static constexpr int kVariantSplitBit = 4096;
static inline void note_launch(rcg_handle* h, int kind, int kernel_id, int variant, int envs_per_wave) {
  h->last[kind].kernel_id = kernel_id;
  h->last[kind].variant = variant | (h->sub_hi > 0 ? kVariantSplitBit : 0);
  h->last[kind].envs_per_wave = envs_per_wave;
  h->last[kind].zero_w = 0u;
}

static constexpr size_t kConstR64 = 512, kConstW = 1296, kConstBytes = 2256;
static constexpr int kFitMaxRows = 8;

int rcg_fail(rcg_handle* h, int code, const char* fmt, ...);

#define HIPCHK(h, call)                                                                                 \
  do {                                                                                                  \
    hipError_t e_ = (call);                                                                             \
    if (e_ != hipSuccess)                                                                               \
      return rcg_fail((h), RCG_ERR_HIP, "%s failed: %s (%s:%d)", #call, hipGetErrorString(e_), __FILE__, \
                      __LINE__);                                                                        \
  } while (0)

struct ProfScope {
  rcg_handle* h;
  hipEvent_t a, b;
  int kernel;
  bool on;
  ProfScope(rcg_handle* h_, int kernel_)
      : h(h_), a(nullptr), b(nullptr), kernel(kernel_), on((h_->prof_mask >> kernel_) & 1u) {
    if (!on) return;
    if ((h->prof_seen[kernel]++ % h->prof_stride) != 0) {
      on = false;
      return;
    }
    for (hipEvent_t* e : {&a, &b}) {
      if (!h->ev_free.empty()) {
        *e = h->ev_free.back();
        h->ev_free.pop_back();
      } else if (hipEventCreate(e) != hipSuccess) {
        if (a) h->ev_free.push_back(a);
        a = b = nullptr;
        on = false;
        return;
      }
    }
    h->cur_a = a;
    h->cur_b = b;
    h->scope_due = true;
  }
  ~ProfScope() {
    if (!on) return;
    h->scope_due = false;
    if (h->cur_a == nullptr) {
      h->ev_pending.push_back({a, b, kernel});
    } else {
      h->cur_a = h->cur_b = nullptr;
      h->ev_free.push_back(a);
      h->ev_free.push_back(b);
    }
  }
  ProfScope(const ProfScope&) = delete;
  ProfScope& operator=(const ProfScope&) = delete;
};

struct ProfPair {
  hipEvent_t a, b;
};
static inline ProfPair prof_take(rcg_handle* h) {
  const ProfPair p{h->cur_a, h->cur_b};
  h->cur_a = h->cur_b = nullptr;
#ifdef RCG_DEV
  if (h->scope_due) {
    if (!p.a) {
      fprintf(stderr, "librcg (dev): a second launch inside one due ProfScope would go untimed\n");
      abort();
    }
  }
#endif
  return p;
}
static inline void prof_give_back(rcg_handle* h, const ProfPair& p) {
  h->cur_a = p.a;
  h->cur_b = p.b;
}

#define RCG_LAUNCH(h, kern, grid, block, lds, ...)                                                                 \
  do {                                                                                                             \
    rcg_handle* h__ = (h);                                                                                         \
    const ProfPair pp__ = prof_take(h__);                                                                          \
    if (pp__.a) {                                                                                                  \
      hipExtLaunchKernelGGL(kern, grid, block, (std::uint32_t)(lds), h__->stream, pp__.a, pp__.b, 0, __VA_ARGS__); \
    } else {                                                                                                       \
      hipLaunchKernelGGL(kern, grid, block, lds, h__->stream, __VA_ARGS__);                                        \
    }                                                                                                              \
  } while (0)

template <typename real>
inline const rcg::KParams<real>& params(const rcg_handle* h);
template <>
inline const rcg::KParams<float>& params<float>(const rcg_handle* h) {
  return h->p32;
}
template <>
inline const rcg::KParams<double>& params<double>(const rcg_handle* h) {
  return h->p64;
}

static inline int opt_memory_of(const rcg_handle* h) {
  if (h->opt_memory >= 0) return h->opt_memory;
  const bool generic = !(h->cfg.mode == RCG_MODE_MPC && h->p32.stage_kind == 0);
  const int dcw = h->cfg.mode != RCG_MODE_MPC ? h->dc : 0;
  int mem = generic ? 4 : 0;
  while (mem > 0 && (size_t)rcg::opt_lds_reals(h->cfg.n_actor, h->ds, h->du, h->np, dcw, mem, h->dy) * h->esz > (size_t)160 * 1024) --mem;
  return mem;
}
static inline size_t opt_wave_lds_bytes(const rcg_handle* h) {
  const int dcw = h->cfg.mode != RCG_MODE_MPC ? h->dc : 0;
  return (size_t)rcg::opt_lds_reals(h->cfg.n_actor, h->ds, h->du, h->np, dcw, opt_memory_of(h), h->dy) * h->esz;
}

static inline unsigned blocks_for(long n, int bs = 256) { return (unsigned)((n + bs - 1) / bs); }

struct SysVTable {
  int (*rhs)(rcg_handle*, const void* state, const void* action, void* dstate, void* clipped, int32_t n, int32_t clip);
  int (*stage_obj)(rcg_handle*, const void* obs, const void* act, void* out, int32_t n);
  int (*critic)(rcg_handle*, const void* obs, const void* act, const void* w, void* out, int32_t n);
  int (*critic_cost)(rcg_handle*, const void* w, void* Jc);
  int (*actor)(rcg_handle*, const char* who, const void* cand, int K, const void* obs, const void* state_sys,
               const void* w, void* J, void* action, void* best_J, int32_t* best_idx, bool tick, bool sim_first);
  int (*sim_step)(rcg_handle*, int32_t n_substeps);
  int (*critic_update)(rcg_handle*, int32_t n_substeps , int32_t do_push, int32_t do_fit);
  int (*optimize)(rcg_handle*, int32_t iters, const void* obs, const void* state_sys, const void* u_init, int shift,
                  void* u_opt, void* action, void* best_J, int32_t* n_iter, bool tick, bool sim_first);
  int (*nominal)(rcg_handle*, const void* obs, void* action, void* lyap, void* theta, int32_t n, double gain,
                 const double* ctrl_pars, int32_t clip, bool tick);
  int (*ticks)(rcg_handle*, int32_t T, int32_t K, const void* cand);
  int (*rhs_full)(rcg_handle*, const void* state, const void* disturb, const void* action, const void* xi, void* dstate,
                  void* ddisturb, void* clipped, int32_t n, int32_t clip);
  int (*search)(rcg_handle*, int32_t K, int32_t rounds, int32_t round0, const void* obs, const void* state_sys,
                const void* centre, int shift, void* u_best, void* action, void* best_J, int32_t* best_idx, bool tick,
                bool sim_first);
  int (*ticks_mem)(rcg_handle*, int32_t T, int32_t K, const void* cand);
  int (*loop)(rcg_handle*, const double* act_in, int32_t n_substeps, int32_t do_sim, int32_t do_tail, int32_t decided, int32_t dc,
              double* out, double* flag, double seq);
};
extern const SysVTable kVt3WRobot, kVt3WRobotNI, kVt2Tank;

struct RtcDims {
  int ds, du, np;
  bool has_jac;
  int dy;
  bool has_out;
  bool has_out_jac;
  bool has_critic;
  bool has_search;
};
const RtcSystem* rtc_lookup(int sys_id, RtcDims* dims);
int rtc_out(rcg_handle* h, const void* state, void* obs, int32_t n);
int rtc_prepare_tick(rcg_handle* h, const void* cand, int32_t K);
int rtc_prepare_tick_opt(rcg_handle* h);
int rtc_prepare_tick_search(rcg_handle* h, int32_t K, int32_t rounds, int32_t warm);
extern const SysVTable kVtRtc;
void rcg_set_thread_error(const std::string& text);
// ... 1 lines not shown
```

### rcognita_amd/csrc/rcg_kernels.hpp

```cpp
#pragma once
#include <stdint.h>

#include <type_traits>

#include "../../include/rcg.h"
#include "rcg_systems.hpp"

namespace rcg {

enum : int { STAGE_FULL = 1, STAGE_BIQUAD = 2 };

#ifdef RCG_DEV
#define RCG_DBG(A, bit) ((A).dbg & (bit))
#else
#define RCG_DBG(A, bit) 0
#endif

template <typename real>
struct KParams {
  real pars[RCG_MAX_PARS];
  real lo[RCG_MAX_DU], hi[RCG_MAX_DU];
  const real* __restrict__ Rfull;
  real R1d[RCG_MAX_CHI], R2d[RCG_MAX_CHI];
  real target[RCG_MAX_DS];
// ... 134 lines not shown
    }
  }
  return q;
}
template <int NCHI, typename real>
__device__ __forceinline__ real stage_any(const KParams<real>& P, const real* chi) {
  return stage_with<NCHI, real>(P, chi, P.stage_kind);
}

template <int DS, int DU, typename real, typename WGet>
__device__ __forceinline__ real critic_with(const real* chi, const real* y, const real* u, WGet w, const int cs) {
  constexpr int NCHI = DS + DU;
  real acc = 0;
  if (cs == RCG_CRITIC_QUAD_LIN || cs == RCG_CRITIC_QUADRATIC) {
    int idx = 0;
#pragma unroll
    for (int i = 0; i < NCHI; ++i)
#pragma unroll
      for (int j = i; j < NCHI; ++j) acc = fma_r(w(idx++), chi[i] * chi[j], acc);
    if (cs == RCG_CRITIC_QUAD_LIN) {
#pragma unroll
      for (int i = 0; i < NCHI; ++i) acc = fma_r(w(idx++), chi[i], acc);
    }
  } else if (cs == RCG_CRITIC_QUAD_NOMIX) {
#pragma unroll
    for (int i = 0; i < NCHI; ++i) acc = fma_r(w(i), chi[i] * chi[i], acc);
  } else {
#pragma unroll
    for (int i = 0; i < DS; ++i) acc = fma_r(w(i), y[i] * y[i], acc);
#pragma unroll
    for (int i = 0; i < DS; ++i)
#pragma unroll
      for (int c = 0; c < DU; ++c) acc = fma_r(w(DS + i * DU + c), y[i] * u[c], acc);
#pragma unroll
    for (int c = 0; c < DU; ++c) acc = fma_r(w(DS + DS * DU + c), u[c] * u[c], acc);
  }
  return acc;
}
template <int DS, int DU>
__host__ __device__ constexpr int critic_dim(int cs) {
  return cs == RCG_CRITIC_QUAD_LIN ? (DS + DU) * (DS + DU + 1) / 2 + (DS + DU)
                                   : (cs == RCG_CRITIC_QUADRATIC ? (DS + DU) * (DS + DU + 1) / 2
                                                                 : (cs == RCG_CRITIC_QUAD_NOMIX ? DS + DU : DS + DS * DU + DU));
}
template <int DS, int DU, typename real>
__device__ __forceinline__ void critic_phi_accum(const real* chi, const real* y, const real* u, real* Phi, const int cs) {
  constexpr int NCHI = DS + DU;
  if (cs == RCG_CRITIC_QUAD_LIN || cs == RCG_CRITIC_QUADRATIC) {
    int idx = 0;
#pragma unroll
    for (int i = 0; i < NCHI; ++i)
#pragma unroll
      for (int j = i; j < NCHI; ++j) {
        Phi[idx] = fma_r(chi[i], chi[j], Phi[idx]);
        ++idx;
      }
    if (cs == RCG_CRITIC_QUAD_LIN) {
#pragma unroll
      for (int i = 0; i < NCHI; ++i) {
        Phi[idx] += chi[i];
        ++idx;
      }
    }
  } else if (cs == RCG_CRITIC_QUAD_NOMIX) {
#pragma unroll
    for (int i = 0; i < NCHI; ++i) Phi[i] = fma_r(chi[i], chi[i], Phi[i]);
  } else {
#pragma unroll
    for (int i = 0; i < DS; ++i) Phi[i] = fma_r(y[i], y[i], Phi[i]);
#pragma unroll
    for (int i = 0; i < DS; ++i)
#pragma unroll
      for (int c = 0; c < DU; ++c) Phi[DS + i * DU + c] = fma_r(y[i], u[c], Phi[DS + i * DU + c]);
#pragma unroll
    for (int c = 0; c < DU; ++c) Phi[DS + DS * DU + c] = fma_r(u[c], u[c], Phi[DS + DS * DU + c]);
  }
}

template <int DS, int DU, typename real, typename WGet>
__device__ __forceinline__ real critic_value(const KParams<real>& P, const real* chi, const real* y,
                                             const real* u, WGet w) {
  return critic_with<DS, DU, real>(chi, y, u, w, P.critic_struct);
}

template <typename Sys, typename real>
__device__ __forceinline__ typename Sys::template Pre<real> load_pre(const KParams<real>& P,
                                                                     const real* pars_env, long b) {
  real pv[Sys::NP > 0 ? Sys::NP : 1];
#pragma unroll
  for (int i = 0; i < Sys::NP; ++i) pv[i] = pars_env ? pars_env[(long)i * P.B + b] : P.pars[i];
  return Sys::template prepare<real>(pv);
}

__device__ __forceinline__ void pin_value(float& v) { asm volatile("" : "+v"(v)); }
__device__ __forceinline__ void pin_value(double& v) { asm volatile("" : "+v"(v)); }

template <typename Sys, typename real>
__device__ __forceinline__ void rk4_step(const typename Sys::template Pre<real>& pre, real* x, const real* u,
                                         real dt) {
  constexpr int DS = Sys::DS;
  const real h = dt, hh = (real)0.5 * dt, h6 = dt / (real)6;
  real k1[DS], k2[DS], k3[DS], k4[DS], t[DS];
  Sys::template rhs<real>(pre, x, u, k1);
#pragma unroll
  for (int c = 0; c < DS; ++c) t[c] = fma_r(hh, k1[c], x[c]);
  Sys::template rhs<real>(pre, t, u, k2);
#pragma unroll
  for (int c = 0; c < DS; ++c) t[c] = fma_r(hh, k2[c], x[c]);
  Sys::template rhs<real>(pre, t, u, k3);
#pragma unroll
  for (int c = 0; c < DS; ++c) t[c] = fma_r(h, k3[c], x[c]);
  Sys::template rhs<real>(pre, t, u, k4);
#pragma unroll
  for (int c = 0; c < DS; ++c) {
    pin_value(k1[c]);
    pin_value(k2[c]);
    pin_value(k3[c]);
    pin_value(k4[c]);
  }
#pragma unroll
  for (int c = 0; c < DS; ++c) x[c] = fma_r(h6, ((k1[c] + (real)2 * k2[c]) + (real)2 * k3[c]) + k4[c], x[c]);
}

template <typename real>
struct ActorArgs {
  const real* cand;
  const real* obs;
  const real* state_sys;
  const real* pars_env;
  const real* w;
  real* J;
  real* action_out;
  real* best_J;
  int32_t* best_idx;
  real* accum;
  int32_t* step_idx;
  int K;
  int Kp;
  int G;
  int n_tiles;
  int grid_g;
  int vec_ok;
  int gpw;
  int jwave;
  int no_multi;
  int dbg;
  int env_lo, env_hi;
  real* sim_state;
  real* sim_state_prev;
  const real* sim_action;
  uint32_t* sim_status;
  int sim_n_sub;
  int obs_x;
};

typedef float v4f __attribute__((ext_vector_type(4)));

template <typename real>
__device__ __forceinline__ void stage_tile(const real* __restrict__ g, real* __restrict__ l, int n,
                                           int lane, int vec_ok) {
  if (vec_ok) {
    const int nv = (int)(((long)n * (long)sizeof(real)) >> 4);
    const v4f* __restrict__ gv = reinterpret_cast<const v4f*>(g);
    v4f* __restrict__ lv = reinterpret_cast<v4f*>(l);
    const int nfull = nv >> 6;
    for (int base = 0; base < nfull; base += 8) {
      const int cnt = nfull - base;
      v4f r[8];
#pragma unroll
      for (int j = 0; j < 8; ++j)
        if (j < cnt) r[j] = __builtin_nontemporal_load(&gv[(base + j) * 64 + lane]);
#pragma unroll
      for (int j = 0; j < 8; ++j)
        if (j < cnt) lv[(base + j) * 64 + lane] = r[j];
    }
    const int i = nfull * 64 + lane;
    if (i < nv) lv[i] = __builtin_nontemporal_load(&gv[i]);
  } else {
    for (int i = lane; i < n; i += 64) l[i] = g[i];
  }
}

template <int DU, typename real>
__device__ __forceinline__ void gen_candidate(const KParams<real>& P, int g, int k, real* ugen) {
  const real den = (real)(g > 1 ? g - 1 : 1);
  if (DU == 1) {
    ugen[0] = fma_r((real)k, (P.hi[0] - P.lo[0]) / den, P.lo[0]);
  } else {
    const int gi = k / g, gj = k - gi * g;
    ugen[0] = fma_r((real)gi, (P.hi[0] - P.lo[0]) / den, P.lo[0]);
    ugen[DU - 1] = fma_r((real)gj, (P.hi[DU - 1] - P.lo[DU - 1]) / den, P.lo[DU - 1]);
  }
}

template <typename Sys, typename real, bool TGT, bool STREAM, int MODE_C, int SK_C, int CS_C, bool G1 = false, unsigned ZW = 0u,
          int NC = 0, typename WGet>
__device__ __forceinline__ real rollout_cost(const KParams<real>& P, const typename Sys::template Pre<real>& pre, int N_rt,
                                             const real* xs, const real* y0, const real* urow, const real* ugen,
                                             WGet wget, real* u0) {
  constexpr int DS = Sys::DS, DY = sys_dy<Sys>(), DU = Sys::DU, NCHI = DY + DU;
  const int N = NC > 0 ? NC : N_rt;
  const int mode = MODE_C >= 0 ? MODE_C : P.mode;
  const int sk = SK_C >= 0 ? SK_C : P.stage_kind;
  const int cs = CS_C >= 0 ? CS_C : P.critic_struct;
  const real h = P.h_pred;
  constexpr bool OUT = HasOut<Sys>::value;
  real x[DS], y[DY];
  if constexpr (OUT) {
#pragma unroll
    for (int c = 0; c < DS; ++c) x[c] = xs[c];
#pragma unroll
    for (int c = 0; c < DY; ++c) y[c] = y0[c];
  } else {
#pragma unroll
    for (int c = 0; c < DS; ++c) {
      x[c] = xs[c];
      y[c] = y0[c];
    }
  }
  static_assert(!G1 || ((MODE_C == RCG_MODE_MPC || MODE_C == RCG_MODE_RQL) && SK_C == 0),
                "the per-component sum is a variant of the diagonal-R1 stage sums (MPC: all N steps, RQL: the first N - 1)");
  real J = 0, gk = 1;
  real u[DU], up[DU];
  real S[G1 ? NCHI : 1];
#pragma unroll
  for (int i = 0; i < (G1 ? NCHI : 1); ++i) S[i] = 0;
  constexpr bool SUMF = MODE_C == RCG_MODE_SQL && CS_C >= 0;
  constexpr int NPHI = SUMF ? critic_dim<DY, DU>(CS_C >= 0 ? CS_C : 0) : 1;
  real Phi[NPHI];
#pragma unroll
  for (int i = 0; i < NPHI; ++i) Phi[i] = 0;
#pragma unroll
  for (int c = 0; c < DU; ++c) up[c] = 0;
  real zw0 = 0;
#pragma unroll
  for (int i = 0; i < DY; ++i)
    if (G1 && ((ZW >> i) & 1u)) zw0 = fma_r(P.R1d[i], y0[i] * y0[i], zw0);
#define RCG_ROLLOUT_STEP                                                                                             \
_Pragma("unroll")                                                                                                        \
    for (int c = 0; c < DU; ++c) u[c] = STREAM ? urow[kk * DU + c] : ugen[c];                                         \
    if (kk == 0) {                                                                                                    \
_Pragma("unroll")                                                                                                        \
      for (int c = 0; c < DU; ++c) u0[c] = u[c];                                                                      \
    } else {                                                                                                          \
      real d[DS];                                                                                                     \
                                                                                                                      \
                                                                                                                      \
      Sys::template rhs<real, true>(pre, x, up, d);                                                                   \
_Pragma("unroll")                                                                                                        \
      for (int c = 0; c < DS; ++c) {                                                                                  \
        x[c] = fma_r(h, d[c], x[c]);                                                                                  \
        if constexpr (!OUT) y[c] = x[c];                                                    \
      }                                                                                                               \
      if constexpr (OUT) sys_out<Sys, real, true>(pre, x, y);                                                         \
    }                                                                                                                 \
    real chi[NCHI];                                                                                                   \
    make_chi<DY, DU, TGT, real>(P, y, u, chi);                                                                        \
    if (G1 && (MODE_C == RCG_MODE_MPC || kk < N - 1)) {                                                               \
_Pragma("unroll")                                                                                                        \
      for (int i = 0; i < NCHI; ++i)                                                                                  \
        if (!((ZW >> i) & 1u)) S[G1 ? i : 0] = fma_r(chi[i], chi[i], S[G1 ? i : 0]);                                  \
    } else if (G1) {                                                                                                  \
      J += critic_with<DY, DU, real>(chi, y, u, wget, cs);                                                            \
    } else if (mode == RCG_MODE_MPC) {                                                                                \
      J = fma_r(gk, stage_with<NCHI, real>(P, chi, sk), J);                                                           \
    } else if (mode == RCG_MODE_RQL) {                                                                                \
      if (kk < N - 1)                                                                                                 \
        J = fma_r(gk, stage_with<NCHI, real>(P, chi, sk), J);                                                         \
      else                                                                                                            \
        J += critic_with<DY, DU, real>(chi, y, u, wget, cs);                                                          \
    } else if (SUMF) {                                                                                                \
      critic_phi_accum<DY, DU, real>(chi, y, u, Phi, CS_C);                                                           \
    } else {                                                                                                          \
      J += critic_with<DY, DU, real>(chi, y, u, wget, cs);                                                            \
    }                                                                                                                 \
    if (!G1) gk *= P.gamma;                                                                                           \
_Pragma("unroll")                                                                                                        \
    for (int c = 0; c < DU; ++c) up[c] = u[c];                                                                        \
                                                                                                                      \
  if constexpr (NC > 0) {
#pragma unroll
    for (int kk = 0; kk < NC; ++kk) {
      RCG_ROLLOUT_STEP
    }
  } else {
    for (int kk = 0; kk < N; ++kk) {
      RCG_ROLLOUT_STEP
    }
  }
#undef RCG_ROLLOUT_STEP
  if (G1) {
#pragma unroll
    for (int i = 0; i < NCHI; ++i)
      if (!((ZW >> i) & 1u)) J = fma_r(P.R1d[i], S[G1 ? i : 0], J);
#ifndef RCG_AB_NO_ZWP
#pragma unroll
    for (int i = 0; i < DY; ++i)
      if ((ZW >> i) & 1u) J = fma_r(P.R1d[i], y[i] * y[i], J);
    J += zw0;
#endif
  }
  if (SUMF) {
#pragma unroll
    for (int i = 0; i < NPHI; ++i) J = fma_r(wget(i), Phi[i], J);
  }
  return J;
// ... 814 lines not shown
```

### rcognita_amd/csrc/rcg_rtc.hip

```cpp
#include <hip/hiprtc.h>

#include <cctype>
#include <map>
#include <memory>
#include <mutex>
#include <tuple>

#include "rcg_rtc_headers.inc"
#include "rcg_sysops.hpp"

using namespace rcg;

namespace {

struct RtcProgram {
  std::string code;
  std::map<std::string, std::string> lowered;
  std::map<int, hipModule_t> module;
  std::map<std::pair<int, std::string>, hipFunction_t> fn;
};

}

struct RtcSystem {
  int id;
  std::string name, src;
  RtcDims dims;
  bool tgt;
  unsigned zw;
  RtcProgram core[2];
  std::map<std::tuple<int, int, int, int>, std::unique_ptr<RtcProgram>> dma;
  std::map<std::tuple<int, int, int>, std::unique_ptr<RtcProgram>> critic;
  std::map<std::tuple<int, int, int, int>, std::unique_ptr<RtcProgram>> search;
  std::vector<std::string> compiled;
};

namespace {

std::mutex g_mu;
std::vector<std::unique_ptr<RtcSystem>> g_sys;

const char* const kSysExpr = "rcg::RcgRtcSys";
const char* const kOpts[] = {"--offload-arch=gfx950", "-O3", "-std=c++17", "-ffp-contract=fast"};

template <typename real>
const char* real_name() {
  return sizeof(real) == 8 ? "double" : "float";
}

bool is_identifier(const char* s) {
  if (!s || !(isalpha((unsigned char)s[0]) || s[0] == '_')) return false;
  for (const char* p = s; *p; ++p)
    if (!(isalnum((unsigned char)*p) || *p == '_')) return false;
  return strlen(s) < 128;
}

std::string unit_source(const RtcSystem& S, bool critic = false, bool search = false) {
  char dims[1536];
  snprintf(dims, sizeof dims,
           "static_assert(RcgRtcSys::DS == %d, \"rcg_register_system: %s::DS differs from the declared ds\");\n"
           "static_assert(RcgRtcSys::DU == %d, \"rcg_register_system: %s::DU differs from the declared du\");\n"
           "static_assert(RcgRtcSys::NP == %d, \"rcg_register_system: %s::NP differs from the declared np\");\n"
           "static_assert(RcgRtcSys::HAS_OUT || RcgRtcSys::DY == RcgRtcSys::DS, \"rcg_register_system: %s::DY differs from DS "
           "but %s defines no out (without an output map the observation is the state)\");\n",
           S.dims.ds, S.name.c_str(), S.dims.du, S.name.c_str(), S.dims.np, S.name.c_str(), S.name.c_str(), S.name.c_str());
  const std::string& N = S.name;
  return std::string(critic ? "#include \"rcg_critic_fit_ml.hpp\"\n#include \"rcg_critic_fit_gen.hpp\"\n" : "") +
         (search ? "#include \"rcg_search.hpp\"\n" : "") +
         "#include \"rcg_actor_dma_packed.hpp\"\n#include \"rcg_actor_opt.hpp\"\nnamespace rcg {\n#line 1 \"" + N + ".policy\"\n" +
         S.src +
         "\n#line 1 \"rcg_rtc_adapter\"\n"
         "namespace rtc {\n"
         "template <class...> using void_t = void;\n"
         "template <class S, class = void> struct tgt { static constexpr bool v = false; };\n"
         "template <class S> struct tgt<S, void_t<decltype(S::TGT)>> { static constexpr bool v = S::TGT; };\n"
         "template <class S, class = void> struct zw { static constexpr unsigned v = 0u; };\n"
         "template <class S> struct zw<S, void_t<decltype(S::ZW_PRESET)>> { static constexpr unsigned v = S::ZW_PRESET; };\n"
         "template <class S, class = void> struct su1 { static constexpr unsigned v = 0u; };\n"
         "template <class S> struct su1<S, void_t<decltype(S::SHARED_U1)>> { static constexpr unsigned v = S::SHARED_U1; };\n"
         "template <class S, class = void> struct jac { static constexpr bool v = false; };\n"
         "template <class S> struct jac<S, void_t<decltype(&S::template jac_T<float, true>)>> { static constexpr bool v = true; };\n"
         "template <class S, class = void> struct out { static constexpr bool v = false; };\n"
         "template <class S> struct out<S, void_t<decltype(&S::template out<float, true>)>> { static constexpr bool v = true; };\n"
         "template <class S, class = void> struct ojac { static constexpr bool v = false; };\n"
         "template <class S> struct ojac<S, void_t<decltype(&S::template out_jac_T<float, true>)>> { static constexpr bool v = true; };\n"
         "template <class S, class = void> struct dy { static constexpr int v = S::DS; };\n"
         "template <class S> struct dy<S, void_t<decltype(S::DY)>> { static constexpr int v = S::DY; };\n"
         "template <class S, class = void> struct crit { static constexpr bool v = false; };\n"
         "template <class S> struct crit<S, void_t<decltype(S::CRITIC)>> { static constexpr bool v = S::CRITIC; };\n"
         "template <class S, class = void> struct srch { static constexpr bool v = false; };\n"
         "template <class S> struct srch<S, void_t<decltype(S::SEARCH)>> { static constexpr bool v = S::SEARCH; };\n"
         "template <bool TGT, bool JAC, int DY, bool OUT, bool OJAC, bool CRIT, bool SRCH, unsigned ZW> __global__ void k_rtc_probe() {}\n"
         "}  // namespace rtc\n"
         "struct RcgRtcSys : " + N + " {\n"
         "  static constexpr bool TGT = rtc::tgt<" + N + ">::v;\n"
         "  static constexpr unsigned ZW_PRESET = rtc::zw<" + N + ">::v;\n"
         "  static constexpr unsigned SHARED_U1 = rtc::su1<" + N + ">::v;\n"
         "  static constexpr bool HAS_OUT = rtc::out<" + N + ">::v;\n"
         "  static constexpr int DY = rtc::dy<" + N + ">::v;\n"
         "};\n" +
         dims + "}  // namespace rcg\n";
}

int compile(const std::string& src, const std::string& file, const std::vector<std::string>& exprs, RtcProgram* out,
            std::string* log) {
  std::vector<const char*> names, texts;
  for (int i = 0; i < kRtcHeaderCount; ++i) {
    names.push_back(kRtcHeaderNames[i]);
    texts.push_back(kRtcHeaderTexts[i]);
  }
  for (const char* stub : {"hip/hip_runtime.h", "hip/hip_ext.h"}) {
    names.push_back(stub);
    texts.push_back("\n");
  }
  hiprtcProgram prog;
  if (hiprtcCreateProgram(&prog, src.c_str(), file.c_str(), (int)names.size(), texts.data(), names.data()) != HIPRTC_SUCCESS) {
    *log = "hiprtcCreateProgram failed";
    return RCG_ERR_HIP;
  }
  for (const auto& e : exprs) hiprtcAddNameExpression(prog, e.c_str());
  const hiprtcResult rc = hiprtcCompileProgram(prog, (int)(sizeof kOpts / sizeof kOpts[0]), kOpts);
  size_t n = 0;
  hiprtcGetProgramLogSize(prog, &n);
  std::string text(n, '\0');
  if (n) hiprtcGetProgramLog(prog, &text[0]);
  while (!text.empty() && text.back() == '\0') text.pop_back();
  if (rc != HIPRTC_SUCCESS) {
    *log = std::string(hiprtcGetErrorString(rc)) + ":\n" + text;
    hiprtcDestroyProgram(&prog);
    return RCG_ERR_BAD_ARG;
  }
  n = 0;
  hiprtcGetCodeSize(prog, &n);
  out->code.assign(n, '\0');
  if (n) hiprtcGetCode(prog, &out->code[0]);
  for (const auto& e : exprs) {
    const char* low = nullptr;
    if (hiprtcGetLoweredName(prog, e.c_str(), &low) != HIPRTC_SUCCESS || !low) {
      *log = "hiprtcGetLoweredName: no instance " + e;
      hiprtcDestroyProgram(&prog);
      return RCG_ERR_HIP;
    }
    out->lowered[e] = low;
  }
  hiprtcDestroyProgram(&prog);
  return n ? RCG_OK : RCG_ERR_HIP;
}

std::string tf(bool b) { return b ? "true" : "false"; }

template <typename real>
std::string expr_rhs() {
  return std::string("rcg::k_rhs<") + kSysExpr + ", " + real_name<real>() + ">";
}
template <typename real>
std::string expr_stage_obj() {
  return std::string("rcg::k_stage_obj<") + kSysExpr + ", " + real_name<real>() + ">";
}
template <typename real>
std::string expr_out() {
  return std::string("rcg::k_out<") + kSysExpr + ", " + real_name<real>() + ">";
}
template <typename real>
std::string expr_sim(bool tgt) {
  return std::string("rcg::k_sim<") + kSysExpr + ", " + real_name<real>() + ", " + tf(tgt) + ">";
}
template <typename real>
std::string expr_actor(bool gen, bool tgt, bool str, bool direct) {
  return std::string("rcg::k_actor<") + kSysExpr + ", " + real_name<real>() + ", " + tf(gen) + ", " + tf(tgt) + ", " + tf(str) +
         (direct ? ", false, true>" : ">");
}
template <typename real>
std::string expr_opt(bool tgt, bool gen, bool pairs) {
  return std::string("rcg::k_actor_opt<") + kSysExpr + ", " + real_name<real>() + ", " + tf(tgt) + ", " + tf(gen) + ", " + tf(pairs) +
         ">";
}
template <typename real>
std::string expr_dma(bool packed, int R, int variant, bool sys_tgt, unsigned zw) {
  const bool tgt = (!packed && variant >= DMA_MPC_GEND) ? true : sys_tgt;
  return std::string(packed ? "rcg::k_actor_dma_packed<" : "rcg::k_actor_dma<") + kSysExpr + ", " + real_name<real>() + ", " +
         std::to_string(R) + ", " + tf(tgt) + ", " + std::to_string(variant) + (zw ? ", " + std::to_string(zw) + "u>" : ">");
}

template <typename real>
std::string expr_critic() {
  return std::string("rcg::k_critic<") + kSysExpr + ", " + real_name<real>() + ">";
}
template <typename real>
std::string expr_critic_cost() {
  return std::string("rcg::k_critic_cost<") + kSysExpr + ", " + real_name<real>() + ">";
}
template <typename real>
std::string expr_fit(int cs, int form) {
  const std::string head = std::string("<") + kSysExpr + ", " + real_name<real>() + ", " + std::to_string(cs);
  if (form == FIT_FORM_GEN) return "rcg::k_critic_fit_gen" + head + ">";
  if (form == FIT_FORM_3ML) return "rcg::k_critic_fit_ml" + head + ", 3>";
  return "rcg::k_critic_fit" + head + ", " + std::to_string(form == FIT_FORM_3 ? 3 : kFitMaxRows) + ">";
}
template <typename real>
std::string expr_search(bool generic, bool tgt, int nc) {
  return std::string("rcg::k_actor_search<") + kSysExpr + ", " + real_name<real>() + ", " + tf(generic) + ", " + tf(tgt) + ", " +
         std::to_string(nc) + ">";
}

template <typename real>
std::vector<std::string> core_exprs(const RtcDims& d) {
  const bool has_jac = d.has_jac && (!d.has_out || d.has_out_jac);
  std::vector<std::string> e{expr_rhs<real>(), expr_stage_obj<real>(), expr_sim<real>(false), expr_sim<real>(true)};
  if (d.has_out) e.push_back(expr_out<real>());
  for (int g = 0; g < 2; ++g)
    for (int t = 0; t < 2; ++t) {
      for (int s = 0; s < 2; ++s) e.push_back(expr_actor<real>(g, t, s, false));
      if (g) e.push_back(expr_actor<real>(true, t, true, true));
    }
  if (has_jac)
    for (int sel = 0; sel < 8; ++sel) e.push_back(expr_opt<real>(sel & 2, sel & 4, sel & 1));
  return e;
}

int function(rcg_handle* h, RtcProgram& P, const std::string& expr, hipFunction_t* fn) {
  const int dev = h->cfg.device;
  auto it = P.fn.find({dev, expr});
  if (it != P.fn.end()) {
    *fn = it->second;
    return RCG_OK;
  }
  auto low = P.lowered.find(expr);
  if (low == P.lowered.end()) return rcg_fail(h, RCG_ERR_HIP, "runtime system: no compiled instance %s", expr.c_str());
  if (!P.module.count(dev)) {
    hipModule_t m = nullptr;
    HIPCHK(h, hipModuleLoadData(&m, P.code.data()));
    P.module[dev] = m;
  }
  hipFunction_t f = nullptr;
  HIPCHK(h, hipModuleGetFunction(&f, P.module[dev], low->second.c_str()));
  P.fn[{dev, expr}] = f;
  *fn = f;
  return RCG_OK;
}

template <typename real>
int core_function(rcg_handle* h, const std::string& expr, hipFunction_t* fn) {
  auto hit = h->rtc_fn.find(expr);
  if (hit != h->rtc_fn.end()) {
    *fn = hit->second;
    return RCG_OK;
  }
  std::lock_guard<std::mutex> lock(g_mu);
  RtcSystem& S = *const_cast<RtcSystem*>(h->rtc);
  const int rc = function(h, S.core[sizeof(real) == 8 ? 1 : 0], expr, fn);
  if (rc == RCG_OK) h->rtc_fn[expr] = *fn;
  return rc;
}

template <typename real>
int dma_function(rcg_handle* h, bool packed, int R, int variant, unsigned zw, hipFunction_t* fn) {
  RtcSystem& S = *const_cast<RtcSystem*>(h->rtc);
  const std::string expr = expr_dma<real>(packed, R, variant, S.tgt, zw);
  auto hit = h->rtc_fn.find(expr);
  if (hit != h->rtc_fn.end()) {
    *fn = hit->second;
    return RCG_OK;
  }
  const auto key = std::make_tuple(sizeof(real) == 8 ? 1 : 0, packed ? 1 : 0, R, variant | (zw ? 256 : 0));
  bool have;
  {
    std::lock_guard<std::mutex> lock(g_mu);
    have = S.dma.count(key) != 0;
  }
  std::unique_ptr<RtcProgram> P;
  if (!have) {
    P.reset(new RtcProgram);
    std::string log;
    const int rc = compile(unit_source(S), S.name + "_dma.hip", {expr}, P.get(), &log);
    if (rc) {
      h->err = "runtime system " + S.name + ": compiling " + expr + ": " + log;
      return RCG_ERR_HIP;
    }
  }
  std::lock_guard<std::mutex> lock(g_mu);
  auto it = S.dma.find(key);
  if (it == S.dma.end()) {
    it = S.dma.emplace(key, std::move(P)).first;
    S.compiled.push_back(S.name + "_dma.hip\t" + expr);
  }
  const int rc = function(h, *it->second, expr, fn);
  if (rc == RCG_OK) h->rtc_fn[expr] = *fn;
  return rc;
}

template <typename real>
int critic_functions(rcg_handle* h, int form, hipFunction_t* f_critic, hipFunction_t* f_cost, hipFunction_t* f_fit) {
  RtcSystem& S = *const_cast<RtcSystem*>(h->rtc);
  if (!S.dims.has_critic) return RCG_ERR_UNSUPPORTED;
  const int cs = h->cfg.critic_struct;
  const std::string e[3] = {expr_critic<real>(), expr_critic_cost<real>(), expr_fit<real>(cs, form)};
  hipFunction_t* const out[3] = {f_critic, f_cost, f_fit};
  bool all = true;
  for (int i = 0; i < 3; ++i) {
    if (!out[i]) continue;
    auto hit = h->rtc_fn.find(e[i]);
    if (hit != h->rtc_fn.end())
      *out[i] = hit->second;
    else
      all = false;
  }
  if (all) return RCG_OK;
  const auto key = std::make_tuple(sizeof(real) == 8 ? 1 : 0, cs, form);
  bool have;
  {
    std::lock_guard<std::mutex> lock(g_mu);
    have = S.critic.count(key) != 0;
  }
  const std::string file = S.name + "_critic.hip";
  std::unique_ptr<RtcProgram> P;
  if (!have) {
    P.reset(new RtcProgram);
    std::string log;
    const int rc = compile(unit_source(S, true), file, {e[0], e[1], e[2]}, P.get(), &log);
    if (rc) {
      h->err = "runtime system " + S.name + ": compiling the critic program (" + e[2] + "): " + log;
      return RCG_ERR_HIP;
    }
  }
  std::lock_guard<std::mutex> lock(g_mu);
  auto it = S.critic.find(key);
  if (it == S.critic.end()) {
    it = S.critic.emplace(key, std::move(P)).first;
    for (const auto& x : e) S.compiled.push_back(file + "\t" + x);
  }
  for (int i = 0; i < 3; ++i) {
    if (!out[i]) continue;
    const int rc = function(h, *it->second, e[i], out[i]);
    if (rc) return rc;
    h->rtc_fn[e[i]] = *out[i];
  }
  return RCG_OK;
}

template <typename real>
int search_function(rcg_handle* h, const SearchPlan& L, hipFunction_t* fn) {
  RtcSystem& S = *const_cast<RtcSystem*>(h->rtc);
  const bool tgt = L.tgt;
  const std::string expr = expr_search<real>(L.generic, tgt, L.nc);
  auto hit = h->rtc_fn.find(expr);
  if (hit != h->rtc_fn.end()) {
    *fn = hit->second;
    return RCG_OK;
  }
  const auto key = std::make_tuple(sizeof(real) == 8 ? 1 : 0, L.generic ? 1 : 0, tgt ? 1 : 0, L.nc);
  bool have;
  {
    std::lock_guard<std::mutex> lock(g_mu);
    have = S.search.count(key) != 0;
  }
  const std::string file = S.name + "_search.hip";
  std::unique_ptr<RtcProgram> P;
  if (!have) {
    P.reset(new RtcProgram);
    std::string log;
    const int rc = compile(unit_source(S, false, true), file, {expr}, P.get(), &log);
    if (rc) {
      h->err = "runtime system " + S.name + ": compiling " + expr + ": " + log;
      return rc;
    }
  }
  std::lock_guard<std::mutex> lock(g_mu);
  auto it = S.search.find(key);
  if (it == S.search.end()) {
    it = S.search.emplace(key, std::move(P)).first;
    S.compiled.push_back(file + "\t" + expr);
  }
  const int rc = function(h, *it->second, expr, fn);
  if (rc == RCG_OK) h->rtc_fn[expr] = *fn;
  return rc;
}

int refuse_search(rcg_handle* h, const char* who) {
  return rcg_fail(h, RCG_ERR_UNSUPPORTED,
                  "%s: not available for a system registered at run time whose policy does not opt in with SEARCH (%s)", who,
                  h->rtc ? h->rtc->name.c_str() : "?");
}

int refuse_critic(rcg_handle* h, const char* who) {
  return rcg_fail(h, RCG_ERR_UNSUPPORTED,
                  "%s: not available for a system registered at run time whose policy does not opt in with CRITIC (%s)", who,
                  h->rtc ? h->rtc->name.c_str() : "?");
}

int launch(rcg_handle* h, hipFunction_t f, dim3 grid, dim3 block, size_t lds, void** args) {
  const ProfPair pp = prof_take(h);
  hipError_t e;
  if (pp.a)
    e = hipExtModuleLaunchKernel(f, grid.x * block.x, grid.y * block.y, grid.z * block.z, block.x, block.y, block.z, lds,
                                 h->stream, args, nullptr, pp.a, pp.b, 0);
  else
    e = hipModuleLaunchKernel(f, grid.x, grid.y, grid.z, block.x, block.y, block.z, (unsigned)lds, h->stream, args, nullptr);
  if (e != hipSuccess) return rcg_fail(h, RCG_ERR_HIP, "runtime system: kernel launch failed: %s", hipGetErrorString(e));
  return RCG_OK;
}

int refuse(rcg_handle* h, const char* who) {
  return rcg_fail(h, RCG_ERR_UNSUPPORTED, "%s: not available for a system registered at run time (%s)", who,
                  h->rtc ? h->rtc->name.c_str() : "?");
}

int rtc_rhs(rcg_handle* h, const void* state, const void* action, void* dstate, void* clipped, int32_t n, int32_t clip) {
  return by_dtype(h, [&](auto r) {
    using real = decltype(r);
    hipFunction_t f;
    int rc = core_function<real>(h, expr_rhs<real>(), &f);
    if (rc) return rc;
    const real* st = (const real*)state;
    const real* ac = (const real*)action;
    real* ds = (real*)dstate;
    real* cl = (real*)clipped;
    const real* pe = (h->f[RCG_FIELD_PARS] && n == h->cfg.batch) ? (const real*)h->f[RCG_FIELD_PARS] : nullptr;
    long nn = n;
    int ci = clip;
    KParams<real> P = params<real>(h);
    void* args[] = {&st, &ac, &ds, &cl, &pe, &nn, &ci, &P};
    return launch(h, f, dim3(blocks_for(n)), dim3(256), 0, args);
  });
}

int rtc_stage_obj(rcg_handle* h, const void* obs, const void* act, void* out, int32_t n) {
  return by_dtype(h, [&](auto r) {
    using real = decltype(r);
    hipFunction_t f;
    int rc = core_function<real>(h, expr_stage_obj<real>(), &f);
    if (rc) return rc;
    const real* o = (const real*)obs;
    const real* a = (const real*)act;
    real* y = (real*)out;
    long nn = n;
    KParams<real> P = params<real>(h);
    void* args[] = {&o, &a, &y, &nn, &P};
    return launch(h, f, dim3(blocks_for(n)), dim3(256), 0, args);
  });
}

template <typename real>
int sim_step(rcg_handle* h, int32_t n_substeps) {
  hipFunction_t f;
  int rc = core_function<real>(h, expr_sim<real>((h->cfg.flags & RCG_FLAG_HAS_TARGET) != 0), &f);
  if (rc) return rc;
  SimArgs<real> A = sim_args<real>(h, n_substeps);
  KParams<real> P = params<real>(h);
  void* args[] = {&A, &P};
  ProfScope prof_scope(h, RCG_KERNEL_SIM);
  note_launch(h, RCG_KERNEL_SIM, RCG_KID_SIM, 0, 64);
  return launch(h, f, dim3(blocks_for(h->cfg.batch)), dim3(256), 0, args);
}

int rtc_sim_step(rcg_handle* h, int32_t n_substeps) {
  return by_dtype(h, [&](auto r) { return sim_step<decltype(r)>(h, n_substeps); });
}

struct ActorPick {
  bool packed, dma;
  unsigned zero_w;
  hipFunction_t f;
};
template <typename real>
int resolve_actor_instance(rcg_handle* h, const ActorArgs<real>& A, const ActorPlan& L, bool streamed, ActorPick* p) {
  p->packed = L.pack_ok && !(L.variant >= DMA_RQL_0 && !packed_critic_ok(h->dc, (int)sizeof(real)));
  p->dma = !p->packed && L.dma_ok;
  const RtcSystem& S = *h->rtc;
  p->zero_w = (p->dma && sizeof(real) == 8 && !S.dims.has_out) ? dma_zero_w<real>(S.zw, L.variant, A, params<real>(h)) : 0u;
  if (p->packed || p->dma) return dma_function<real>(h, p->packed, L.R, L.variant, p->zero_w, &p->f);
  return core_function<real>(h, expr_actor<real>(L.long_row || L.generic, L.tgt, streamed, L.long_row), &p->f);
}

template <typename real>
int actor(rcg_handle* h, const char* who, const void* cand, int K, const void* obs, const void* state_sys, const void* w, void* J,
          void* action, void* best_J, int32_t* best_idx, bool tick, bool sim_first) {
  const RtcSystem& S = *h->rtc;
  ActorArgs<real> A;
  ActorPlan L;
  int rc = actor_plan<real>(h, who, S.dims.ds, S.dims.du, S.tgt, cand, K, obs, state_sys, w, J, action, best_J, best_idx, tick,
                            sim_first, A, L);
  if (rc) return rc;
  if (h->probe == 1) {
    h->probe = (L.dma_ok && !L.pack_ok) ? 3 : 2;
    return RCG_OK;
  }
  if (h->sub_hi > 0 && !(L.dma_ok && !L.pack_ok))
    return rcg_fail(h, RCG_ERR_UNSUPPORTED, "%s: a split tick needs the k_actor_dma shape", who);
  ActorPick pick;
  rc = resolve_actor_instance<real>(h, A, L, cand != nullptr, &pick);
  if (rc) return rc;
  const bool packed = pick.packed, dma = pick.dma;
  hipFunction_t const f = pick.f;
  const bool fuse_sim = packed && L.fuse_sim;
  if (sim_first && !fuse_sim) {
    rc = sim_step<real>(h, h->cfg.substeps_per_tick);
    if (rc) return rc;
  }
  KParams<real> P = params<real>(h);
  ProfScope prof_scope(h, RCG_KERNEL_ACTOR);
  if (packed) {
    ActorArgs<real> Ap = packed_args(h, A, L);
    void* args[] = {&Ap, &P};
    rc = launch(h, f, L.pack_grid, dim3(256), L.pack_lds, args);
    if (rc == RCG_OK) note_launch(h, RCG_KERNEL_ACTOR, RCG_KID_ACTOR_DMA_PACKED, L.variant | (fuse_sim ? 16 : 0), (int)L.pack_gpw);
    return rc;
  }
  if (dma) {
    ActorArgs<real> Ad = dma_args(h, A, L);
    void* args[] = {&Ad, &P};
    rc = launch(h, f, L.dma_grid, dim3(256), L.dma_lds, args);
    if (rc == RCG_OK) {
      note_launch(h, RCG_KERNEL_ACTOR, RCG_KID_ACTOR_DMA, L.variant, (int)L.dma_gpw);
      h->last[RCG_KERNEL_ACTOR].zero_w = pick.zero_w;
    }
    return rc;
  }
  void* args[] = {&A, &P};
  rc = launch(h, f, dim3(L.blocks), dim3(64 * L.wpb), L.long_row ? 0 : L.lds, args);
  if (rc == RCG_OK)
    note_launch(h, RCG_KERNEL_ACTOR, RCG_KID_ACTOR,
                L.long_row ? (1 | (L.tgt ? 2 : 0) | 4 | 16) : ((L.generic ? 1 : 0) | (L.tgt ? 2 : 0) | (cand ? 4 : 0)), A.G);
  return rc;
}

int rtc_actor(rcg_handle* h, const char* who, const void* cand, int K, const void* obs, const void* state_sys, const void* w,
              void* J, void* action, void* best_J, int32_t* best_idx, bool tick, bool sim_first) {
  return by_dtype(h, [&](auto r) {
    return actor<decltype(r)>(h, who, cand, K, obs, state_sys, w, J, action, best_J, best_idx, tick, sim_first);
  });
}

int rtc_optimize(rcg_handle* h, int32_t iters, const void* obs, const void* state_sys, const void* u_init, int shift, void* u_opt,
                 void* action, void* best_J, int32_t* n_iter, bool tick, bool sim_first) {
  if (!h->rtc->dims.has_jac)
    return rcg_fail(h, RCG_ERR_UNSUPPORTED, "rcg_actor_optimize: the policy %s defines no jac_T (the optimiser's adjoint sweep)",
                    h->rtc->name.c_str());
  if (h->rtc->dims.has_out && !h->rtc->dims.has_out_jac)
    return rcg_fail(h, RCG_ERR_UNSUPPORTED,
                    "rcg_actor_optimize: the policy %s defines out but no out_jac_T (the adjoint of its output map)",
                    h->rtc->name.c_str());
  if (h->loop_io.on) return refuse(h, "rcg_loop_step");
  return by_dtype(h, [&](auto r) {
    using real = decltype(r);
    const rcg_cfg& c = h->cfg;
    OptArgs<real> A;
    int wpb;
    size_t lds;
    int rc = opt_plan<real>(h, h->du, iters, obs, state_sys, u_init, shift, u_opt, action, best_J, n_iter, tick, A, wpb, lds);
    if (rc) return rc;
    KParams<real> P = params<real>(h);
    const bool generic = !(c.mode == RCG_MODE_MPC && P.stage_kind == 0);
    const bool tgt = c.flags & RCG_FLAG_HAS_TARGET;
    const bool pairs = A.memory > 0;
    hipFunction_t f;
    rc = core_function<real>(h, expr_opt<real>(tgt, generic, pairs), &f);
    if (rc) return rc;
    if (tick && sim_first) {
      rc = sim_step<real>(h, c.substeps_per_tick);
      if (rc) return rc;
    }
    ProfScope prof_scope(h, RCG_KERNEL_ACTOR);
    void* args[] = {&A, &P};
    rc = launch(h, f, dim3(blocks_for(c.batch, wpb * OPT_G)), dim3(64 * wpb), lds, args);
    if (rc == RCG_OK)
      note_launch(h, RCG_KERNEL_ACTOR, RCG_KID_ACTOR_OPT, (generic ? 1 : 0) | (tgt ? 2 : 0) | (pairs ? 4 : 0), OPT_G);
    return rc;
  });
}

int rtc_critic(rcg_handle* h, const void* obs, const void* act, const void* w, void* out, int32_t n) {
  if (!h->rtc->dims.has_critic) return refuse(h, "rcg_critic");
  return by_dtype(h, [&](auto r) {
    using real = decltype(r);
    hipFunction_t f;
    int rc = critic_functions<real>(h, fit_form_of(h->cfg.n_critic - 1, h->dc, false), &f, nullptr, nullptr);
    if (rc) return rc;
    const real* o = (const real*)obs;
    const real* a = (const real*)act;
    const real* ww = (const real*)w;
    real* y = (real*)out;
    long nn = n;
    KParams<real> P = params<real>(h);
    void* args[] = {&o, &a, &ww, &y, &nn, &P};
    return launch(h, f, dim3(blocks_for(n)), dim3(256), 0, args);
  });
}

int rtc_critic_cost(rcg_handle* h, const void* w, void* Jc) {
  if (!h->rtc->dims.has_critic) return refuse(h, "rcg_critic_cost");
  return by_dtype(h, [&](auto r) {
    using real = decltype(r);
    hipFunction_t f;
    int rc = critic_functions<real>(h, fit_form_of(h->cfg.n_critic - 1, h->dc, false), nullptr, &f, nullptr);
    if (rc) return rc;
    const real* ww = w ? (const real*)w : (const real*)h->f[RCG_FIELD_W_CRITIC];
    const real* wp = (const real*)h->f[RCG_FIELD_W_PREV];
    const real* ob = (const real*)h->f[RCG_FIELD_OBS_BUF];
    const real* ab = (const real*)h->f[RCG_FIELD_ACT_BUF];
    real* jc = (real*)Jc;
    KParams<real> P = params<real>(h);
    void* args[] = {&ww, &wp, &ob, &ab, &jc, &P};
    return launch(h, f, dim3(blocks_for(h->cfg.batch)), dim3(256), 0, args);
  });
}

int rtc_critic_update(rcg_handle* h, int32_t n_substeps, int32_t do_push, int32_t do_fit) {
  if (!h->rtc->dims.has_critic) return refuse(h, "the critic update");
  return by_dtype(h, [&](auto r) {
    using real = decltype(r);
    hipFunction_t f;
    int rc = critic_functions<real>(h, fit_form_of(h->cfg.n_critic - 1, h->dc, false), nullptr, nullptr, &f);
    if (rc) return rc;
    ProfScope prof_scope(h, RCG_KERNEL_CRITIC);
    FitArgs<real> F;
    FitPlan L;
    rc = fit_plan<real>(h, n_substeps, do_push, do_fit, false, F, L);
    if (rc) return rc;
    KParams<double> P64 = h->p64;
    KParams<real> P = params<real>(h);
    double* scratch = (double*)h->fit_scratch;
    void* args[] = {&F, &P64, &P, &scratch};
    rc = launch(h, f, L.grid, L.block, 0, args);
    if (rc == RCG_OK) note_launch(h, RCG_KERNEL_CRITIC, RCG_KID_CRITIC_FIT, L.variant, L.epw);
    return rc;
  });
}
int rtc_nominal(rcg_handle* h, const void*, void*, void*, void*, int32_t, double, const double*, int32_t, bool) {
  return refuse(h, "the nominal controller");
}
int rtc_ticks(rcg_handle* h, int32_t, int32_t, const void*) { return refuse(h, "rcg_control_ticks"); }
int rtc_rhs_full(rcg_handle* h, const void*, const void*, const void*, const void*, void*, void*, void*, int32_t, int32_t) {
  return refuse(h, "rcg_rhs_full");
}
int rtc_search(rcg_handle* h, int32_t K, int32_t rounds, int32_t round0, const void* obs, const void* state_sys, const void* centre,
               int shift, void* u_best, void* action, void* best_J, int32_t* best_idx, bool tick, bool sim_first) {
  if (!h->rtc->dims.has_search) return refuse_search(h, "rcg_actor_search");
  return by_dtype(h, [&](auto r) {
    using real = decltype(r);
    const RtcSystem& S = *h->rtc;
    SearchArgs<real> A;
    SearchPlan L;
    int rc = search_plan<real>(h, S.dims.du, S.tgt, K, rounds, round0, obs, state_sys, centre, shift, u_best, action, best_J,
                               best_idx, tick, A, L);
    if (rc) return rc;
    hipFunction_t f;
    rc = search_function<real>(h, L, &f);
    if (rc) return rc;
    if (tick && sim_first) {
      rc = sim_step<real>(h, h->cfg.substeps_per_tick);
      if (rc) return rc;
    }
    KParams<real> P = params<real>(h);
    ProfScope prof_scope(h, RCG_KERNEL_ACTOR);
    void* args[] = {&A, &P};
    rc = launch(h, f, L.grid, L.block, L.lds, args);
    if (rc == RCG_OK) note_launch(h, RCG_KERNEL_ACTOR, RCG_KID_ACTOR_SEARCH, L.variant, 1);
    return rc;
  });
}
int rtc_loop(rcg_handle* h, const double*, int32_t, int32_t, int32_t, int32_t, int32_t, double*, double*, double) {
  return refuse(h, "rcg_loop_step");
}

int probe(RtcSystem& S, std::string* log) {
  const std::string pol = "rcg::" + S.name;
  const std::string e = std::string("rcg::rtc::k_rtc_probe<") + kSysExpr + "::TGT, rcg::rtc::jac<" + pol + ">::v, " + kSysExpr +
// ... 218 lines not shown
```

### rcognita_amd/csrc/rcg_sysops.hpp

```cpp
#pragma once
#include <cmath>
#include <cstdlib>
#include <cstring>
#include <type_traits>

#include "rcg_actor_dma.hpp"
#include "rcg_actor_dma_packed.hpp"
#include "rcg_critic_fit_ml.hpp"
#include "rcg_actor_opt.hpp"
#include "rcg_critic_fit.hpp"
#include "rcg_critic_fit_gen.hpp"
#include "rcg_disturb.hpp"
#include "rcg_handle.hpp"
#include "rcg_loop.hpp"
#include "rcg_nominal.hpp"
#include "rcg_search.hpp"
#include "rcg_ticks.hpp"

namespace rcg {

template <typename F>
static int by_dtype(rcg_handle* h, F&& f) {
  return h->cfg.dtype == RCG_F64 ? f(double{}) : f(float{});
}
// ... 151 lines not shown
      const dim3 gridv(blocks_for(h->cfg.batch / VEC));
      if (h->cfg.flags & RCG_FLAG_HAS_TARGET)
        RCG_LAUNCH(h, (k_sim_v<Sys, real, true>), gridv, dim3(256), 0, A, params<real>(h));
      else
        RCG_LAUNCH(h, (k_sim_v<Sys, real, false>), gridv, dim3(256), 0, A, params<real>(h));
      note_launch(h, RCG_KERNEL_SIM, RCG_KID_SIM_V, 0, 64 * (int)VEC);
    } else if (h->cfg.flags & RCG_FLAG_HAS_TARGET)
      RCG_LAUNCH(h, (k_sim<Sys, real, true>), dim3(blocks_for(h->cfg.batch)), dim3(256), 0, A,
                         params<real>(h));
    else
      RCG_LAUNCH(h, (k_sim<Sys, real, false>), dim3(blocks_for(h->cfg.batch)), dim3(256), 0, A,
                         params<real>(h));
    HIPCHK(h, hipGetLastError());
    return (int)RCG_OK;
  });
}

#ifdef RCG_DEV
static int fit_lanes_knob();
#endif

constexpr int kFitLanesMinDc = 9;

enum { FIT_FORM_3 = 0, FIT_FORM_3ML = 1, FIT_FORM_ROWS = 2, FIT_FORM_GEN = 3 };
struct FitPlan {
  int form;
  dim3 grid, block;
  int variant;
  int epw;
};
static inline int fit_form_of(int m, int dc, bool force_ml) {
  if (m > kFitMaxRows) return FIT_FORM_GEN;
  if (m > 3) return FIT_FORM_ROWS;
  return (dc >= kFitLanesMinDc || force_ml) ? FIT_FORM_3ML : FIT_FORM_3;
}
template <typename real>
static int fit_plan(rcg_handle* h, int32_t n_substeps, int32_t do_push, int32_t do_fit, bool force_ml, FitArgs<real>& F, FitPlan& L) {
  const int m = h->cfg.n_critic - 1;
  memset(&F, 0, sizeof F);
  F.w_critic = (real*)h->f[RCG_FIELD_W_CRITIC];
  F.w_prev = (real*)h->f[RCG_FIELD_W_PREV];
  F.obs_buf = (real*)h->f[RCG_FIELD_OBS_BUF];
  F.act_buf = (real*)h->f[RCG_FIELD_ACT_BUF];
  F.wcfg = reinterpret_cast<const double*>((unsigned char*)h->d_const + kConstW);
  F.do_sim = n_substeps > 0;
  F.do_push = do_push;
  F.do_fit = do_fit;
  F.state = (const real*)h->f[RCG_FIELD_STATE];
  F.action = (const real*)h->f[RCG_FIELD_ACTION];
  F.sim.state = (real*)h->f[RCG_FIELD_STATE];
  F.sim.state_prev = (real*)h->f[RCG_FIELD_STATE_PREV];
  F.sim.action = (const real*)h->f[RCG_FIELD_ACTION];
  F.sim.pars_env = (const real*)h->f[RCG_FIELD_PARS];
  F.sim.accum = (real*)h->f[RCG_FIELD_ACCUM];
  F.sim.status = (uint32_t*)h->f[RCG_FIELD_STATUS];
  F.sim.n_sub = n_substeps;
  F.env_lo = h->sub_lo;
  F.env_hi = h->sub_hi;
  const long n_env = h->sub_hi > 0 ? h->sub_hi - h->sub_lo : h->cfg.batch;
  L.form = fit_form_of(m, h->dc, force_ml);
  const bool gen = L.form == FIT_FORM_GEN, fit_ml = L.form == FIT_FORM_3ML;
  L.block = dim3(64);
  L.grid = dim3(blocks_for(n_env, fit_ml ? 64 / FIT_L : 64));
  L.variant = h->cfg.critic_struct + 16 * (m <= 3 ? 3 : (gen ? 0 : kFitMaxRows)) + (F.do_sim ? 256 : 0) + (do_fit ? 512 : 0) +
              (fit_ml ? 1024 : 0) + (gen ? 2048 : 0);
  L.epw = fit_ml ? 16 : 64;
  if (gen && do_fit) {
    const size_t need = (size_t)fit_gen_scratch_doubles(m, h->dc) * (size_t)h->cfg.batch * sizeof(double);
    if (h->fit_scratch_bytes < need) {
      if (h->fit_scratch) {
        HIPCHK(h, hipStreamSynchronize(h->stream));
        HIPCHK(h, hipFree(h->fit_scratch));
        h->fit_scratch = nullptr;
        h->fit_scratch_bytes = 0;
      }
      if (hipMalloc(&h->fit_scratch, need) != hipSuccess) {
        (void)hipGetLastError();
        return rcg_fail(h, RCG_ERR_HIP, "critic fit with %d TD rows: cannot allocate %zu bytes of scratch for %d envs", m, need,
                        h->cfg.batch);
      }
      h->fit_scratch_bytes = need;
    }
  }
  return RCG_OK;
}

template <typename Sys, typename real, int CS>
static void launch_fit3(rcg_handle* h, const FitArgs<real>& F, const FitPlan& L) {
  constexpr int DC = CriticDim<CS, sys_dy<Sys>(), Sys::DU>::value;
  if constexpr (DC >= kFitLanesMinDc) {
    RCG_LAUNCH(h, (k_critic_fit_ml<Sys, real, CS, 3>), L.grid, L.block, 0, F, h->p64, params<real>(h));
  } else {
#ifdef RCG_DEV
    if (L.form == FIT_FORM_3ML) {
      RCG_LAUNCH(h, (k_critic_fit_ml<Sys, real, CS, 3>), L.grid, L.block, 0, F, h->p64, params<real>(h));
      return;
    }
#endif
    RCG_LAUNCH(h, (k_critic_fit<Sys, real, CS, 3>), L.grid, L.block, 0, F, h->p64, params<real>(h));
  }
}

template <typename Sys>
int op_critic_update(rcg_handle* h, int32_t n_substeps, int32_t do_push, int32_t do_fit) {
  return by_dtype(h, [&](auto r) {
    using real = decltype(r);
    ProfScope prof_scope(h, RCG_KERNEL_CRITIC);
    FitArgs<real> F;
    FitPlan L;
#ifdef RCG_DEV
    const bool force_ml = fit_lanes_knob() == FIT_L;
#else
    const bool force_ml = false;
#endif
    const int rc = fit_plan<real>(h, n_substeps, do_push, do_fit, force_ml, F, L);
    if (rc) return rc;
#define RCG_FIT(CS)                                                                                                    \
  do {                                                                                                                 \
    if (L.form == FIT_FORM_3 || L.form == FIT_FORM_3ML)                                                                \
      launch_fit3<Sys, real, CS>(h, F, L);                                                                             \
    else if (L.form == FIT_FORM_ROWS)                                                                                  \
      RCG_LAUNCH(h, (k_critic_fit<Sys, real, CS, kFitMaxRows>), L.grid, L.block, 0, F, h->p64, params<real>(h));       \
    else                                                                                                               \
      RCG_LAUNCH(h, (k_critic_fit_gen<Sys, real, CS>), L.grid, L.block, 0, F, h->p64, params<real>(h),                 \
                 (double*)h->fit_scratch);                                                                             \
  } while (0)
    switch (h->cfg.critic_struct) {
      case RCG_CRITIC_QUAD_LIN: RCG_FIT(RCG_CRITIC_QUAD_LIN); break;
      case RCG_CRITIC_QUADRATIC: RCG_FIT(RCG_CRITIC_QUADRATIC); break;
      case RCG_CRITIC_QUAD_NOMIX: RCG_FIT(RCG_CRITIC_QUAD_NOMIX); break;
      default: RCG_FIT(RCG_CRITIC_QUAD_MIX); break;
    }
#undef RCG_FIT
    note_launch(h, RCG_KERNEL_CRITIC, RCG_KID_CRITIC_FIT, L.variant, L.epw);
    HIPCHK(h, hipGetLastError());
    return (int)RCG_OK;
  });
}

struct DevKnobs {
  int dbg = 0;
  bool force_plain = false, no_g1 = false;
  long gpw = 0;
  long lds_pad = 0;
  int per_cu = 0;
  long plain_lds = 0;
  bool mpc_only = false;
  bool no_gen_multi = false;
  bool no_pack = false;
  int fit_lanes = 0;
  int dma_min_k = 33;
  bool no_tick_fuse = false;
  bool no_pk = false;
};
static inline const DevKnobs& dev_knobs() {
  static const DevKnobs k = [] {
    DevKnobs v;
#ifdef RCG_DEV
    if (const char* e = getenv("RCG_DBG")) v.dbg = atoi(e);
    if (const char* e = getenv("RCG_ACTOR_KERNEL")) v.force_plain = !strcmp(e, "plain");
    if (const char* e = getenv("RCG_GPW")) v.gpw = atol(e);
    if (const char* e = getenv("RCG_LDS_PAD")) v.lds_pad = atol(e);
    if (const char* e = getenv("RCG_PER_CU")) v.per_cu = atoi(e);
    if (const char* e = getenv("RCG_PLAIN_LDS")) v.plain_lds = atol(e);
    v.mpc_only = getenv("RCG_DMA_MPC_ONLY") != nullptr;
    v.no_gen_multi = getenv("RCG_NO_GEN_MULTI") != nullptr;
    v.no_g1 = getenv("RCG_NO_G1") != nullptr;
    v.no_pack = getenv("RCG_NO_PACK") != nullptr;
    v.no_pk = getenv("RCG_NO_PK") != nullptr;
    v.no_tick_fuse = getenv("RCG_NO_TICK_FUSE") != nullptr;
    if (const char* e = getenv("RCG_DMA_MINK")) v.dma_min_k = atoi(e);
    if (const char* e = getenv("RCG_FIT_LANES")) v.fit_lanes = atoi(e);
#endif
    return v;
  }();
  return k;
}
#ifdef RCG_DEV
static int fit_lanes_knob() { return dev_knobs().fit_lanes; }
#endif

template <typename Sys>
int op_ticks(rcg_handle* h, int32_t T, int32_t K, const void* cand);

struct ActorPlan {
  int R;
  size_t row_bytes;
  bool long_row;
  bool generic, tgt;
  int wpb;
  size_t lds;
  unsigned blocks;
  int variant;
  bool dma_ok, pack_ok;
  bool fuse_sim;
  long pack_gpw;
  dim3 pack_grid;
  size_t pack_lds;
  long dma_gpw;
  dim3 dma_grid;
  size_t dma_lds;
  int dma_jwave;
};

template <typename real>
static int actor_plan(rcg_handle* h, const char* who, int DS, int DU, bool sys_tgt, const void* cand, int K, const void* obs,
                      const void* state_sys, const void* w, void* J, void* action, void* best_J, int32_t* best_idx, bool tick,
                      bool sim_first, ActorArgs<real>& A, ActorPlan& L) {
  const rcg_cfg& c = h->cfg;
  if (K < 1) return rcg_fail(h, RCG_ERR_BAD_ARG, "%s: K must be >= 1", who);
  memset(&A, 0, sizeof A);
  A.cand = (const real*)cand;
  A.obs = obs ? (const real*)obs : (const real*)h->f[RCG_FIELD_STATE];
  if (state_sys)
    A.state_sys = (const real*)state_sys;
  else if (obs)
    A.state_sys = (const real*)obs;
  else
    A.state_sys = (const real*)h->f[(tick && (c.flags & RCG_FLAG_REF_LAG)) ? RCG_FIELD_STATE_PREV : RCG_FIELD_STATE];
  A.obs_x = obs ? 0 : 1;
  if (obs && !state_sys && h->dy != h->ds)
    return rcg_fail(h, RCG_ERR_BAD_ARG, "%s: an observation of dim_output %d != dim_state %d needs state_sys", who, h->dy, h->ds);
  A.pars_env = (const real*)h->f[RCG_FIELD_PARS];
  A.w = w ? (const real*)w : (const real*)h->f[RCG_FIELD_W_CRITIC];
  if (c.mode != RCG_MODE_MPC && !A.w)
    return rcg_fail(h, RCG_ERR_BAD_ARG, "%s: RQL/SQL need critic weights (buffer_size > 0 or an explicit w)", who);
  A.J = (real*)J;
  A.action_out = (real*)action;
  A.best_J = (real*)best_J;
  A.best_idx = best_idx;
  A.accum = (tick && !(c.flags & RCG_FLAG_ACCUM_EVERY_SUBSTEP)) ? (real*)h->f[RCG_FIELD_ACCUM] : nullptr;
  A.step_idx = tick ? (int32_t*)h->f[RCG_FIELD_STEP_IDX] : nullptr;
  A.K = K;
  if (K >= 64) {
    A.Kp = 64;
    A.G = 1;
    A.n_tiles = (K + 63) / 64;
  } else {
    int kp = 1;
    while (kp < K) kp <<= 1;
    A.Kp = kp;
    A.G = 64 / kp;
    A.n_tiles = 1;
  }
  A.grid_g = 0;
  A.no_multi = dev_knobs().no_gen_multi ? 1 : 0;
  if (!cand) {
    if (DU == 1) {
      A.grid_g = K;
    } else {
      int g = (int)std::floor(std::sqrt((double)K) + 1e-9);
      if (g * g != K)
        return rcg_fail(h, RCG_ERR_BAD_ARG, "%s: generated grid for du = 2 needs a square K (got %d)", who, K);
      A.grid_g = g;
    }
  }
  const int R = c.n_actor * DU;
  const size_t row_bytes = (size_t)R * sizeof(real);
  L.R = R;
  L.row_bytes = row_bytes;
  A.vec_ok = (cand && row_bytes % 16 == 0 && ((uintptr_t)cand % 16) == 0) ? 1 : 0;
  const long B = c.batch;
  const long n_waves = (B + A.G - 1) / A.G;
  int wpb = 4;
  const bool long_row = cand && R > RCG_MAX_ROW;
  size_t lds_per_wave = (cand && !long_row) ? 64 * row_bytes : 0;
  while (wpb > 1 && lds_per_wave * wpb > 64 * 1024) wpb >>= 1;
  size_t lds = lds_per_wave * wpb;
  if (cand && (size_t)dev_knobs().plain_lds > lds) lds = (size_t)dev_knobs().plain_lds;
  L.long_row = long_row;
  L.wpb = wpb;
  L.lds = lds;
  L.blocks = (unsigned)((n_waves + wpb - 1) / wpb);
  const KParams<real>& P = params<real>(h);
  const bool generic = !(c.mode == RCG_MODE_MPC && P.stage_kind == 0);
  const bool tgt = (c.flags & RCG_FLAG_HAS_TARGET) != 0;
  L.generic = generic;
  L.tgt = tgt;

  const DevKnobs& knobs = dev_knobs();
  A.dbg = knobs.dbg;
  constexpr size_t esz = sizeof(real);
  const size_t tile = (size_t)64 * dma_rpl(R, (int)esz) * R * esz;
  const bool mode_ok = c.mode == RCG_MODE_MPC || !knobs.mpc_only;
  const bool std_cost = P.stage_kind == 0 && (tgt == sys_tgt || !tgt);
  const bool gen_cost = c.mode == RCG_MODE_MPC && P.stage_kind != 0 && !knobs.force_plain;
  const bool gen_rql = c.mode == RCG_MODE_RQL && !std_cost && !knobs.force_plain;
  const bool sql_any = c.mode == RCG_MODE_SQL && (tgt == sys_tgt || !tgt);
  int variant;
  if (gen_cost)
    variant = (P.stage_kind & STAGE_FULL) ? DMA_MPC_GENF : DMA_MPC_GEND;
  else if (c.mode == RCG_MODE_MPC)
    variant = (c.gamma == 1.0 && !knobs.no_g1) ? DMA_MPC_G1 : DMA_MPC;
  else if (c.mode == RCG_MODE_RQL)
    variant = (gen_rql ? DMA_RQL_GEN_0 : DMA_RQL_0) + c.critic_struct;
  else
    variant = DMA_SQL_0 + c.critic_struct;
  L.variant = variant;
  const size_t wslot = (size_t)4 * dma_wslot((int)esz, variant, h->dy, DU);
  const bool slab16 = ((size_t)K * row_bytes) % 16 == 0;
  const int dma_min_k = (c.mode != RCG_MODE_MPC && knobs.dma_min_k > 20) ? 20 : knobs.dma_min_k;
  L.dma_ok = cand && ((uintptr_t)cand % 16) == 0 && K >= dma_min_k && slab16 && R <= dma_max_row<real>() &&
             (std_cost || gen_cost || gen_rql || sql_any) && mode_ok && !knobs.force_plain &&
             !(A.J && 4 * tile + wslot + 4 * esz * K > (size_t)160 * 1024);
  const int pack_g = (K >= 4 && K <= 32) ? 64 / K : 0;
  L.pack_ok = cand && ((uintptr_t)cand % 16) == 0 && pack_g >= 2 && slab16 && R <= dma_max_row<real>() && P.stage_kind == 0 &&
              mode_ok && (tgt == sys_tgt || !tgt) && !knobs.force_plain && !knobs.no_pack;
  L.fuse_sim = L.pack_ok && tick && sim_first && !obs && !state_sys && !A.J &&
               !(c.flags & (RCG_FLAG_DISTURB | RCG_FLAG_ACCUM_EVERY_SUBSTEP)) && !knobs.no_tick_fuse;
  {
    long gpw = pack_g;
    while (pack_g > 0 && gpw * 2 <= 64 && B / (gpw * 2) >= 4096) gpw *= 2;
    if (pack_g > 0 && knobs.gpw > 0 && knobs.gpw % pack_g == 0 && knobs.gpw <= 64) gpw = knobs.gpw;
    const long pw = gpw > 0 ? (B + gpw - 1) / gpw : 0;
    const size_t full_tile = (size_t)64 * R * esz;
    size_t lds_req = 4 * full_tile + (A.J ? 4 * esz * (size_t)gpw * K : 0) + (L.fuse_sim ? 4 * esz * 2 * DS * 64 : 0);
    const size_t cap = knobs.per_cu == 2 ? (size_t)56 * 1024 : (knobs.per_cu == 8 ? 0 : (size_t)36 * 1024);
    if (lds_req < cap) lds_req = cap;
    L.pack_gpw = gpw;
    L.pack_grid = dim3((unsigned)((pw + 3) / 4));
    L.pack_lds = lds_req;
  }
  {
    const long Bn = h->sub_hi > 0 ? h->sub_hi - h->sub_lo : B;
    long gpw = 1;
    while (gpw < 16 && Bn / (gpw * 2) >= 8192) gpw *= 2;
    if (knobs.gpw > 0) gpw = knobs.gpw;
    gpw = gpw < 1 ? 1 : (gpw > 64 ? 64 : gpw);
    const long pw = (Bn + gpw - 1) / gpw;
    const bool long_slab = (size_t)gpw * K * row_bytes >= (size_t)16 * 1024 * esz;
    const bool valu_heavy = variant == DMA_MPC_GENF ||
                            variant >= DMA_RQL_GEN_0 ||
                            ((dma_is_rql(variant) || dma_is_sql(variant)) && (size_t)dma_dc(dma_cs(variant), h->dy, DU) * esz >= 68);
    const int per_cu = knobs.per_cu > 0 ? knobs.per_cu : ((row_bytes >= 20 * esz && long_slab && !valu_heavy) ? 2 : 4);
    const int jwave = (A.J && 4 * tile + wslot + 4 * esz * gpw * K <= (size_t)64 * 1024) ? 1 : 0;
    size_t lds_req = 4 * tile + wslot + (A.J ? 4 * esz * K * (jwave ? gpw : 1) : 0);
    if (knobs.lds_pad > 0) {
      lds_req += (size_t)knobs.lds_pad;
    } else if (knobs.lds_pad == 0) {
      const size_t want = per_cu <= 2 ? (size_t)56 * 1024 : (per_cu <= 4 ? (size_t)36 * 1024 : 0);
      if (lds_req < want) lds_req = want;
    }
    L.dma_gpw = gpw;
    L.dma_grid = dim3((unsigned)((pw + 3) / 4));
    L.dma_lds = lds_req;
    L.dma_jwave = jwave;
  }
  return RCG_OK;
}

template <typename real>
static ActorArgs<real> packed_args(const rcg_handle* h, const ActorArgs<real>& A, const ActorPlan& L) {
  ActorArgs<real> Ap = A;
  Ap.G = 64 / A.K;
  Ap.gpw = (int)L.pack_gpw;
  Ap.jwave = 1;
  if (L.fuse_sim) {
    Ap.sim_state = (real*)h->f[RCG_FIELD_STATE];
    Ap.sim_state_prev = (real*)h->f[RCG_FIELD_STATE_PREV];
    Ap.sim_action = (const real*)h->f[RCG_FIELD_ACTION];
    Ap.sim_status = (uint32_t*)h->f[RCG_FIELD_STATUS];
    Ap.sim_n_sub = h->cfg.substeps_per_tick;
  }
  return Ap;
}
template <typename real>
static ActorArgs<real> dma_args(const rcg_handle* h, const ActorArgs<real>& A, const ActorPlan& L) {
  ActorArgs<real> Ad = A;
  Ad.gpw = (int)L.dma_gpw;
  Ad.env_lo = h->sub_lo;
  Ad.env_hi = h->sub_hi;
  Ad.jwave = L.dma_jwave;
  return Ad;
}

template <typename Sys, typename real>
static int launch_actor(rcg_handle* h, const char* who, const void* cand, int K, const void* obs,
                        const void* state_sys, const void* w, void* J, void* action, void* best_J, int32_t* best_idx,
                        bool tick, bool sim_first) {
  const rcg_cfg& c = h->cfg;
  ActorArgs<real> A;
  ActorPlan L;
  {
    const int rc = actor_plan<real>(h, who, Sys::DS, Sys::DU, Sys::TGT, cand, K, obs, state_sys, w, J, action, best_J, best_idx,
                                    tick, sim_first, A, L);
    if (rc) return rc;
  }
  const KParams<real>& P = params<real>(h);
  const DevKnobs& knobs = dev_knobs();
  const int R = L.R, wpb = L.wpb, variant = L.variant;
  const size_t lds = L.lds;
  const unsigned blocks = L.blocks;
  const bool generic = L.generic, tgt = L.tgt, dma_ok = L.dma_ok, pack_ok = L.pack_ok, fuse_sim = L.fuse_sim;
  if (h->probe == 1) {
    h->probe = (dma_ok && !pack_ok) ? 3 : 2;
    return RCG_OK;
  }
  if (h->sub_hi > 0 && !(dma_ok && !pack_ok))
    return rcg_fail(h, RCG_ERR_UNSUPPORTED, "%s: a split tick needs the k_actor_dma shape", who);
  if constexpr (std::is_same<real, float>::value && GenPk<Sys>::supported && GenPk<Sys>::fuse_tick) {
    if (tick && sim_first && !cand && !generic && !tgt && c.gamma == 1.0 && Sys::ZW_PRESET != 0u &&
        (P.zero_w & Sys::ZW_PRESET) == Sys::ZW_PRESET && K >= 256 && A.n_tiles % 4 == 0 && A.grid_g > 0 &&
        (64 % A.grid_g) == 0 && !A.no_multi && !knobs.no_pk && !knobs.no_tick_fuse && !(c.flags & RCG_FLAG_DISTURB) && !obs &&
        !state_sys &&
        action == h->f[RCG_FIELD_ACTION] && best_J == h->f[RCG_FIELD_BEST_J] && (void*)best_idx == h->f[RCG_FIELD_BEST_IDX])
      return op_ticks<Sys>(h, 1, K, nullptr);
  }
  if (sim_first && !fuse_sim) {
    int rc = op_sim_step<Sys>(h, c.substeps_per_tick);
    if (rc) return rc;
  }
  ProfScope prof_scope(h, RCG_KERNEL_ACTOR);
  if (pack_ok) {
    const ProfPair pp = prof_take(h);
    const ActorArgs<real> Ap = packed_args(h, A, L);
    const dim3 grid = L.pack_grid, block(256);
    const size_t lds_req = L.pack_lds;
    const bool launched =
        variant < DMA_RQL_0    ? launch_dma_packed<Sys, real, 3>(R, variant, grid, block, lds_req, h->stream, Ap, P, pp.a, pp.b)
        : variant >= DMA_SQL_0 ? launch_dma_packed<Sys, real, 4>(R, variant, grid, block, lds_req, h->stream, Ap, P, pp.a, pp.b)
                               : launch_dma_packed<Sys, real, 5>(R, variant, grid, block, lds_req, h->stream, Ap, P, pp.a, pp.b);
    if (launched) {
      note_launch(h, RCG_KERNEL_ACTOR, RCG_KID_ACTOR_DMA_PACKED, variant | (fuse_sim ? 16 : 0), (int)L.pack_gpw);
      HIPCHK(h, hipGetLastError());
      return RCG_OK;
    }
    prof_give_back(h, pp);
    if (fuse_sim) {
      int rc = op_sim_step<Sys>(h, c.substeps_per_tick);
      if (rc) return rc;
    }
  }
  if (dma_ok) {
    const ActorArgs<real> Ad = dma_args(h, A, L);
    const dim3 grid = L.dma_grid, block(256);
    const size_t lds_req = L.dma_lds;
    bool ok = false;
    const ProfPair pp = prof_take(h);
    if (variant >= DMA_RQL_GEN_0)
      ok = launch_dma<Sys, real, 7>(R, variant, grid, block, lds_req, h->stream, Ad, P, pp.a, pp.b);
    else if (variant >= DMA_MPC_GEND)
      ok = launch_dma<Sys, real, 6>(R, variant, grid, block, lds_req, h->stream, Ad, P, pp.a, pp.b);
    else if (variant < DMA_RQL_0)
      ok = launch_dma<Sys, real, 0>(R, variant, grid, block, lds_req, h->stream, Ad, P, pp.a, pp.b);
    else if (variant >= DMA_SQL_0)
      ok = launch_dma<Sys, real, 1>(R, variant, grid, block, lds_req, h->stream, Ad, P, pp.a, pp.b);
    else
      ok = launch_dma<Sys, real, 2>(R, variant, grid, block, lds_req, h->stream, Ad, P, pp.a, pp.b);
    if (!ok) prof_give_back(h, pp);
    if (ok) {
      note_launch(h, RCG_KERNEL_ACTOR, RCG_KID_ACTOR_DMA, variant, (int)L.dma_gpw);
      h->last[RCG_KERNEL_ACTOR].zero_w = dma_zero_w<real>(dma_zw_preset<Sys, real>(), variant, Ad, P);
      HIPCHK(h, hipGetLastError());
      return RCG_OK;
    }
  }
  if constexpr (std::is_same<real, float>::value && GenPk<Sys>::supported) {
    const bool pk_ok = !cand && !generic && !tgt && c.gamma == 1.0 && Sys::ZW_PRESET != 0u &&
                       (P.zero_w & Sys::ZW_PRESET) == Sys::ZW_PRESET && K >= 256 && A.n_tiles % 4 == 0 && A.grid_g > 0 &&
                       (64 % A.grid_g) == 0 && !A.no_multi && !knobs.no_pk;
    if (pk_ok) {
      RCG_LAUNCH(h, (k_actor<Sys, real, false, false, false, true>), dim3(blocks), dim3(64 * wpb), lds, A, P);
      note_launch(h, RCG_KERNEL_ACTOR, RCG_KID_ACTOR, 8, A.G);
      HIPCHK(h, hipGetLastError());
      return RCG_OK;
    }
  }
  if (L.long_row) {
    if (tgt)
      RCG_LAUNCH(h, (k_actor<Sys, real, true, true, true, false, true>), dim3(blocks), dim3(64 * wpb), 0, A, P);
    else
      RCG_LAUNCH(h, (k_actor<Sys, real, true, false, true, false, true>), dim3(blocks), dim3(64 * wpb), 0, A, P);
    note_launch(h, RCG_KERNEL_ACTOR, RCG_KID_ACTOR, 1 | (tgt ? 2 : 0) | 4 | 16, A.G);
    HIPCHK(h, hipGetLastError());
    return RCG_OK;
  }
#define RCG_LAUNCH_ACTOR(GEN, TGT, STR) \
  RCG_LAUNCH(h, (k_actor<Sys, real, GEN, TGT, STR>), dim3(blocks), dim3(64 * wpb), lds, A, P)
#define RCG_LAUNCH_ACTOR2(GEN, TGT)      \
  do {                                   \
    if (cand)                            \
      RCG_LAUNCH_ACTOR(GEN, TGT, true);  \
    else                                 \
      RCG_LAUNCH_ACTOR(GEN, TGT, false); \
  } while (0)
  if (generic) {
    if (tgt)
      RCG_LAUNCH_ACTOR2(true, true);
    else
      RCG_LAUNCH_ACTOR2(true, false);
  } else {
    if (tgt)
      RCG_LAUNCH_ACTOR2(false, true);
    else
      RCG_LAUNCH_ACTOR2(false, false);
  }
#undef RCG_LAUNCH_ACTOR2
#undef RCG_LAUNCH_ACTOR
  note_launch(h, RCG_KERNEL_ACTOR, RCG_KID_ACTOR, (generic ? 1 : 0) | (tgt ? 2 : 0) | (cand ? 4 : 0), A.G);
  HIPCHK(h, hipGetLastError());
  return RCG_OK;
}

template <typename Sys>
int op_actor(rcg_handle* h, const char* who, const void* cand, int K, const void* obs, const void* state_sys,
                    const void* w, void* J, void* action, void* best_J, int32_t* best_idx, bool tick, bool sim_first) {
  return by_dtype(h, [&](auto r) {
    return launch_actor<Sys, decltype(r)>(h, who, cand, K, obs, state_sys, w, J, action, best_J, best_idx, tick,
                                          sim_first);
  });
}

template <typename real>
static int opt_plan(rcg_handle* h, int du, int32_t iters, const void* obs, const void* state_sys, const void* u_init, int shift,
                    void* u_opt, void* action, void* best_J, int32_t* n_iter, bool tick, OptArgs<real>& A, int& wpb, size_t& lds) {
  const rcg_cfg& c = h->cfg;
  memset(&A, 0, sizeof A);
  A.obs = obs ? (const real*)obs : (const real*)h->f[RCG_FIELD_STATE];
  if (state_sys)
    A.state_sys = (const real*)state_sys;
  else if (obs)
    A.state_sys = (const real*)obs;
  else
    A.state_sys = (const real*)h->f[(tick && (c.flags & RCG_FLAG_REF_LAG)) ? RCG_FIELD_STATE_PREV : RCG_FIELD_STATE];
  A.obs_x = obs ? 0 : 1;
  if (obs && !state_sys && h->dy != h->ds)
    return rcg_fail(h, RCG_ERR_BAD_ARG, "rcg_actor_optimize: an observation of dim_output %d != dim_state %d needs state_sys", h->dy,
                    h->ds);
  A.pars_env = (const real*)h->f[RCG_FIELD_PARS];
  A.w = (const real*)h->f[RCG_FIELD_W_CRITIC];
  if (c.mode != RCG_MODE_MPC && !A.w)
    return rcg_fail(h, RCG_ERR_BAD_ARG, "rcg_actor_optimize: RQL/SQL need critic weights (buffer_size > 0)");
  A.u_init = (const real*)u_init;
  A.u_opt = (real*)u_opt;
  A.action_out = (real*)action;
  A.best_J = (real*)best_J;
  A.n_iter = n_iter;
  A.accum = (tick && !(c.flags & RCG_FLAG_ACCUM_EVERY_SUBSTEP)) ? (real*)h->f[RCG_FIELD_ACCUM] : nullptr;
  A.step_idx = tick ? (int32_t*)h->f[RCG_FIELD_STEP_IDX] : nullptr;
  for (int i = 0; i < du; ++i) A.u0[i] = (real)c.action_init[i];
  A.iters = iters;
  A.shift = shift;
  A.memory = opt_memory_of(h);
  A.ftol = (real)h->opt_ftol;
  A.dcw = c.mode != RCG_MODE_MPC ? h->dc : 0;
  const size_t lds_wave = opt_wave_lds_bytes(h);
  wpb = 4;
  size_t on_cu = 0;
  for (int cand_wpb = 4; cand_wpb >= 1; cand_wpb >>= 1) {
    const size_t fit = lds_wave * cand_wpb ? ((size_t)160 * 1024 / (lds_wave * cand_wpb)) * cand_wpb : 0;
    if (fit * 4 > on_cu * 5) {
      on_cu = fit;
      wpb = cand_wpb;
    }
  }
  lds = lds_wave * wpb;
  if (lds > (size_t)160 * 1024)
    return rcg_fail(h, RCG_ERR_UNSUPPORTED,
                    "rcg_actor_optimize: horizon %d with %d curvature pairs needs %zu B of LDS per wave (rcg_set_optimizer)",
                    c.n_actor, opt_memory_of(h), lds_wave);
  return RCG_OK;
}

template <typename Sys>
int op_optimize(rcg_handle* h, int32_t iters, const void* obs, const void* state_sys, const void* u_init,
                       int shift, void* u_opt, void* action, void* best_J, int32_t* n_iter, bool tick, bool sim_first) {
  const rcg_cfg& c = h->cfg;
  return by_dtype(h, [&](auto r) {
    using real = decltype(r);
    const KParams<real>& P = params<real>(h);
    OptArgs<real> A;
    int wpb;
    size_t lds;
    {
      const int rc = opt_plan<real>(h, Sys::DU, iters, obs, state_sys, u_init, shift, u_opt, action, best_J, n_iter, tick, A, wpb, lds);
      if (rc) return rc;
    }
    const bool loop = h->loop_io.on;
    if (loop)
      fill_loop_args<real>(h, A.loop, h->loop_io.act_in, h->loop_io.n_substeps, 1, 1, 1, h->loop_io.dc, h->loop_io.out,
                           h->loop_io.flag, h->loop_io.seq);
    const bool generic = !(c.mode == RCG_MODE_MPC && P.stage_kind == 0);
    const dim3 grid(blocks_for(c.batch, wpb * OPT_G)), block(64 * wpb);
    const bool tgt = c.flags & RCG_FLAG_HAS_TARGET;
    if (tick && sim_first) {
      const int rc = op_sim_step<Sys>(h, c.substeps_per_tick);
      if (rc) return rc;
    }
    const bool pairs = A.memory > 0;
    ProfScope prof_scope(h, RCG_KERNEL_ACTOR);
#define RCG_OPT_LAUNCH(T, GEN, PR)                                                                                  \
  do {                                                                                                              \
    auto fn = k_actor_opt<Sys, real, T, GEN, PR>;                                                                   \
    if (lds > 64 * 1024)                              \
      HIPCHK(h, hipFuncSetAttribute(reinterpret_cast<const void*>(fn), hipFuncAttributeMaxDynamicSharedMemorySize, \
                                    (int)lds));                                                                     \
    RCG_LAUNCH(h, fn, grid, block, lds, A, P);                                                                      \
  } while (0)
    const int sel = (generic ? 4 : 0) | (tgt ? 2 : 0) | (pairs ? 1 : 0);
    if (loop) {
      if (generic || pairs || obs || state_sys != h->f[RCG_FIELD_STATE_PREV] || u_init || tick)
        return rcg_fail(h, RCG_ERR_UNSUPPORTED, "rcg_loop_step: the one-launch sample is the plain MPC instance on the handle's own fields");
      auto fn = tgt ? k_actor_opt<Sys, real, true, false, false, true> : k_actor_opt<Sys, real, false, false, false, true>;
      if (lds > 64 * 1024)
        HIPCHK(h, hipFuncSetAttribute(reinterpret_cast<const void*>(fn), hipFuncAttributeMaxDynamicSharedMemorySize, (int)lds));
// ... 374 lines not shown
```

### rcognita_amd/engine.py

```python
from __future__ import annotations

import ctypes as C
from dataclasses import dataclass
from typing import Optional, Sequence

import numpy as np

from . import _native as N


@dataclass
class EngineConfig:

    sys_id: int
    batch: int = 1
    dtype: str = "f32"
    device: int = 0
    Nactor: int = 5
    mode: str = "MPC"
    stage_obj_struct: str = "quadratic"
    critic_struct: str = "quad-nomix"
    Ncritic: int = 4
    buffer_size: int = 0
    substeps_per_tick: int = 1
# ... 595 lines not shown
        return act.T.copy(), uo, bj, ni

    def control_tick_opt(self, iters=10, warm_start=False):
        N.check(N.lib().rcg_control_tick_opt(self._h, int(iters), 1 if warm_start else 0), self._h)

    def actor_search(self, K=256, rounds=6, obs=None, state_sys=None, centre=None):
        keep = []
        c0 = None if centre is None else np.broadcast_to(
            np.asarray(centre, dtype=self.real).reshape(-1, self.N, self.du), (self.B, self.N, self.du))
        pobs, pxs, pc = self._in_many([self._soa_item(obs, self.dy, "obs"), self._soa_item(state_sys, self.ds, "state_sys"),
                                       (c0, None, None, "centre")], keep)
        (pub, pact, pbj, pbi), fetch = self._out_many([((self.B, self.N, self.du), None), ((self.du, self.B), None),
                                                       ((self.B,), None), ((self.B,), np.int32)])
        N.check(N.lib().rcg_actor_search(self._h, int(K), int(rounds), pobs, pxs, pc, pub, pact, pbj, pbi), self._h)
        ub, act, bj, bi = fetch()
        return act.T.copy(), ub, bj, bi

    def control_tick_search(self, K=256, rounds=6, warm_start=False):
        N.check(N.lib().rcg_control_tick_search(self._h, int(K), int(rounds), 1 if warm_start else 0), self._h)

    def candidates_sample(self, K, round=0, centre=None, out=None):
        keep = []
        c0 = None if centre is None else np.broadcast_to(
            np.asarray(centre, dtype=self.real).reshape(-1, self.N, self.du), (self.B, self.N, self.du))
        (pc,) = self._in_many([(c0, None, (self.B, self.N, self.du), "centre")], keep)
        shape = (self.B, int(K), self.N, self.du)
        if out is not None:
            po = self._check_device_input(out, shape, self.real, "out")
            N.check(N.lib().rcg_candidates_sample(self._h, po, int(K), int(round), pc), self._h)
            if keep:
                self.synchronize()
            return out
        d = self._tmp(shape)
        N.check(N.lib().rcg_candidates_sample(self._h, C.c_void_p(d.ptr), int(K), int(round), pc), self._h)
        return d.to_host()

    def set_optimizer(self, memory=-1, ftol=None):
        N.check(N.lib().rcg_set_optimizer(self._h, int(memory)), self._h)
        if ftol is not None:
            N.check(N.lib().rcg_set_optimizer_tol(self._h, float(ftol)), self._h)

    @staticmethod
    def _ctrl_pars(ctrl_pars):
        if ctrl_pars is None:
            return None
        m, I = (float(v) for v in ctrl_pars)
        return (C.c_double * 2)(m, I)

    def nominal_action(self, obs, ctrl_gain, ctrl_pars=None, clip=False, want_lyap=False):
        obs = np.asarray(obs, dtype=self.real).reshape(-1, self.dy)
        n = obs.shape[0]
        keep = []
        (pact, plyap), fetch = self._out_many([((self.du, n), None), ((n,), None) if want_lyap else None])
        N.check(N.lib().rcg_nominal_action(self._h, self._in(obs, keep, lambda a: a.T), pact, plyap, n, float(ctrl_gain),
                                           self._ctrl_pars(ctrl_pars), 1 if clip else 0), self._h)
        act, lyap = fetch()
        a = act.T.copy()
        return (a, lyap) if want_lyap else a

    def nominal_theta(self, obs):
        obs = np.asarray(obs, dtype=self.real).reshape(-1, self.dy)
        n = obs.shape[0]
        keep = []
        (pth,), fetch = self._out_many([((n,), None)])
        N.check(N.lib().rcg_nominal_theta(self._h, self._in(obs, keep, lambda a: a.T), pth, n), self._h)
        return fetch()[0]

    def control_tick_nominal(self, ctrl_gain, ctrl_pars=None):
        N.check(N.lib().rcg_control_tick_nominal(self._h, float(ctrl_gain), self._ctrl_pars(ctrl_pars)), self._h)

    def critic_update(self, do_fit=True):
        N.check(N.lib().rcg_critic_update(self._h, 1 if do_fit else 0), self._h)

    def critic_fit(self):
        N.check(N.lib().rcg_critic_fit(self._h), self._h)

    def episode_reset(self):
        N.check(N.lib().rcg_episode_reset(self._h), self._h)

    def episode_stats(self, from_accum=False, want_returns=False):
        s = N.RcgSummary()
        out = np.empty((self.B,), dtype=self.real) if want_returns else None
        N.check(N.lib().rcg_episode_stats(self._h, 1 if from_accum else 0, out.ctypes.data if want_returns else None,
                                          C.byref(s)), self._h, allow=(N.ERR_NONFINITE,))
        return {k: getattr(s, k) for k in ("count", "sum", "sumsq", "min", "max", "n_failed")}, out

    def state_dict(self):
        out = {"tick_count": np.int64(N.lib().rcg_tick_count(self._h)), "batch": np.int64(self.B),
               "sys_id": np.int64(self.cfg.sys_id), "dtype": np.str_(self.cfg.dtype)}
        for f in range(N.FIELD_COUNT):
            if N.lib().rcg_field_bytes(self._h, f) > 0:
                out[f"field_{f}"] = self.get_field(f)
        return out

    def load_state_dict(self, sd):
        if int(sd["batch"]) != self.B or int(sd["sys_id"]) != int(self.cfg.sys_id) or str(sd["dtype"]) != self.cfg.dtype:
            raise ValueError("checkpoint was written by a handle with another batch / system / dtype")
        for f in range(N.FIELD_COUNT):
            have = N.lib().rcg_field_bytes(self._h, f) > 0
            if have != (f"field_{f}" in sd):
                raise ValueError(f"checkpoint and handle disagree on field {f} (different mode / flags)")
        order = [N.FIELD_STATE] + [f for f in range(N.FIELD_COUNT) if f != N.FIELD_STATE]
        for f in order:
            if f"field_{f}" in sd:
                self.set_field(f, sd[f"field_{f}"])
        N.check(N.lib().rcg_set_tick_count(self._h, int(sd["tick_count"])), self._h)

    def checkpoint(self, path):
        np.savez(path, **self.state_dict())

    def restore(self, path):
        with np.load(path, allow_pickle=False) as z:
            self.load_state_dict({k: z[k] for k in z.files})

    def profile(self, kernels=(N.KERNEL_ACTOR, N.KERNEL_SIM, N.KERNEL_CRITIC), stride=1, skip=0):
        mask = 0
        if kernels is True:
            mask = 7
        elif kernels:
            for k in kernels:
                mask |= 1 << int(k)
        if mask:
            stride = min(max(int(stride), 1), 0xfff)
            mask |= stride << 8
            mask |= (int(skip) % stride) << 20
        N.check(N.lib().rcg_profile(self._h, mask), self._h)

    def profile_pause(self):
        N.check(N.lib().rcg_profile(self._h, 0x80), self._h)

    def profile_read(self, kernel=N.KERNEL_ACTOR):
        ms, n = C.c_double(), C.c_int64()
        N.check(N.lib().rcg_profile_read(self._h, int(kernel), C.byref(ms), C.byref(n)), self._h)
        return ms.value, n.value

    def profile_samples(self, kernel=N.KERNEL_ACTOR) -> np.ndarray:
        n = C.c_int64()
        N.check(N.lib().rcg_profile_samples(self._h, int(kernel), None, 0, C.byref(n)), self._h)
        out = np.empty(max(n.value, 1), dtype=np.float64)
        N.check(N.lib().rcg_profile_samples(self._h, int(kernel), out.ctypes.data_as(C.POINTER(C.c_double)), n.value,
                                            C.byref(n)), self._h)
        return out[:n.value]

    def last_launch(self, kind=N.KERNEL_ACTOR):
        kid, var, epw = C.c_int32(), C.c_int32(), C.c_int32()
        N.check(N.lib().rcg_last_launch(self._h, int(kind), C.byref(kid), C.byref(var), C.byref(epw)), self._h)
        return {"kernel": N.lib().rcg_kernel_name(kid.value).decode(), "kernel_id": kid.value, "variant": var.value & ~4096,
                "envs_per_wave": epw.value, "split": bool(var.value & 4096)}

    def last_launch_zero_w(self, kind=N.KERNEL_ACTOR):
        m = C.c_uint32()
        N.check(N.lib().rcg_last_launch_zero_w(self._h, int(kind), C.byref(m)), self._h)
        return int(m.value)
```

Before: 162.3 million.

## Add persistent-wave dynamic env claiming to DMA actor kernel

Replaces the static one-chunk-per-wave assignment in the DMA actor kernel with a persistent grid sized to the compute-unit count. Waves claim env ranges through a global atomic ticket counter, using a claim plan that hands out progressively smaller chunks toward the tail. The goal is to balance load and drop launches of many short-lived waves when batches are large. It adds atomic traffic, counter-reset logic and extra kernel template instantiations, and it disables per-candidate J output on the dynamic path.

```diff
diff --git a/include/rcg.h b/include/rcg.h
--- a/include/rcg.h
+++ b/include/rcg.h
@@ -7,7 +7,7 @@
 extern "C" {
 #endif
 
-#define RCG_VERSION 124
+#define RCG_VERSION 125
 
 #define RCG_MAX_DS 5
 #define RCG_MAX_DU 2
@@ -216,6 +216,7 @@
 } rcg_kernel_id;
 int rcg_last_launch(const rcg_handle* h, int32_t kind, int32_t* kernel_id, int32_t* variant, int32_t* envs_per_wave);
 int rcg_last_launch_zero_w(const rcg_handle* h, int32_t kind, uint32_t* mask);
+int rcg_last_launch_claims(const rcg_handle* h, int32_t kind, int32_t* claims, int32_t* waves);
 const char* rcg_kernel_name(int32_t kernel_id);
 
 #ifdef __cplusplus
diff --git a/rcognita_amd/_native.py b/rcognita_amd/_native.py
--- a/rcognita_amd/_native.py
+++ b/rcognita_amd/_native.py
@@ -7,7 +7,7 @@
 _HERE = os.path.dirname(os.path.abspath(__file__))
 LIB_PATH = os.path.join(_HERE, "lib", "librcg.so")
 
-RCG_VERSION = 124
+RCG_VERSION = 125
 OK, ERR_BAD_ARG, ERR_HIP, ERR_NO_DEVICE, ERR_UNSUPPORTED, ERR_NONFINITE = 0, -1, -2, -3, -4, -5
 SYS_3WROBOT, SYS_3WROBOT_NI, SYS_2TANK = 0, 1, 2
 MODE_MPC, MODE_RQL, MODE_SQL = 0, 1, 2
@@ -44,7 +44,7 @@
     "rcg_profile_samples", "rcg_last_launch", "rcg_kernel_name", "rcg_wait_stream", "rcg_nominal_theta", "rcg_set_optimizer", "rcg_set_optimizer_tol", "rcg_set_tick_parts", "rcg_join", "rcg_loop_step", "rcg_loop_step_begin", "rcg_loop_step_end",
     "rcg_actor_search", "rcg_control_tick_search", "rcg_candidates_sample", "rcg_release_stream",
     "rcg_register_system", "rcg_rtc_version", "rcg_system_info", "rcg_system_output_info", "rcg_out",
-    "rcg_system_has_critic", "rcg_system_programs", "rcg_critic_fit", "rcg_last_launch_zero_w", "rcg_system_has_search",
+    "rcg_system_has_critic", "rcg_system_programs", "rcg_critic_fit", "rcg_last_launch_zero_w", "rcg_last_launch_claims", "rcg_system_has_search",
 ]
 KERNEL_ACTOR, KERNEL_SIM, KERNEL_CRITIC = 0, 1, 2
 (KID_NONE, KID_ACTOR, KID_ACTOR_DMA, KID_TICKS, KID_ACTOR_OPT, KID_NOMINAL, KID_SIM, KID_SIM_V, KID_SIM_DIST,
@@ -161,6 +161,7 @@
         "rcg_profile_samples": (C.c_int, [vp, i32, C.POINTER(C.c_double), i64, C.POINTER(i64)]),
         "rcg_last_launch": (C.c_int, [vp, i32, C.POINTER(i32), C.POINTER(i32), C.POINTER(i32)]),
         "rcg_last_launch_zero_w": (C.c_int, [vp, i32, C.POINTER(C.c_uint32)]),
+        "rcg_last_launch_claims": (C.c_int, [vp, i32, C.POINTER(C.c_int32), C.POINTER(C.c_int32)]),
         "rcg_kernel_name": (C.c_char_p, [i32]),
         "rcg_wait_stream": (C.c_int, [vp, vp]),
         "rcg_release_stream": (C.c_int, [vp, vp]),
diff --git a/rcognita_amd/csrc/rcg_actor_dma.hpp b/rcognita_amd/csrc/rcg_actor_dma.hpp
--- a/rcognita_amd/csrc/rcg_actor_dma.hpp
+++ b/rcognita_amd/csrc/rcg_actor_dma.hpp
@@ -122,7 +122,43 @@
 
 __host__ __device__ constexpr int dma_rpl(int r, int esz) { return r * esz <= 24 ? 4 : (r * esz <= 32 ? 2 : 1); }
 
-template <typename Sys, typename real, int R, bool TGT, int V, unsigned ZW = 0u>
+__host__ __device__ inline void dma_claim_plan(int n, int g, int w, int* n_claims, int* n_full, int* n_top) {
+  int p2 = 1;
+  while (p2 < g) p2 *= 2;
+  const long w2 = 2L * w, span = w2 * p2;
+  const int top = (long)n > span ? (int)(n - span) : 0;
+  const int full = (top + g - 1) / g;
+  const long r = (long)(n - top) - 1;
+  long j = r;
+  if (r >= 2 * w2) {
+    int q = 1;
+    while (w2 * (2L << q) <= r) ++q;
+    j = 2 * w2 + w2 * (q - 1) + (r - w2 * (1L << q)) / (1L << q);
+  }
+  *n_claims = full + (int)j + 1;
+  *n_full = full;
+  *n_top = top;
+}
+__device__ __forceinline__ void dma_claim(int tk, int n, int g, int n_claims, int n_full, int n_top, int w2, int& c0, int& c1) {
+  if (tk < n_full) {
+    c0 = tk * g;
+    c1 = c0 + g < n_top ? c0 + g : n_top;
+  } else {
+    const int j = n_claims - 1 - tk;
+    if (j < 2 * w2) {
+      c1 = n - j;
+      c0 = c1 - 1;
+    } else {
+      const int jj = j - 2 * w2;
+      const int ql = (jj >= w2) + (jj >= 2 * w2) + (jj >= 3 * w2) + (jj >= 4 * w2) + (jj >= 5 * w2);
+      const int within = jj - ql * w2, p = 2 << ql;
+      c1 = n - (w2 + within) * p;
+      c0 = c1 - p > n_top ? c1 - p : n_top;
+    }
+  }
+}
+
+template <typename Sys, typename real, int R, bool TGT, int V, unsigned ZW = 0u, bool DYN = false>
 __global__ __launch_bounds__(256) void k_actor_dma(const ActorArgs<real> A, const KParams<real> P) {
   constexpr int DS = Sys::DS, DY = sys_dy<Sys>(), DU = Sys::DU, NCHI = DY + DU, NP = Sys::NP;
   constexpr bool OUT = HasOut<Sys>::value;
@@ -161,10 +197,25 @@
   const int T = (K + TROWS - 1) / TROWS;
   const int rem_rows = K % TROWS;
   const long env_hi = A.env_hi > 0 ? A.env_hi : B;
-  const long env0 = A.env_lo + wave * A.gpw;
-  if (env0 >= env_hi) return;
-  const long env1 = env0 + A.gpw < env_hi ? env0 + A.gpw : env_hi;
+  long env0, env1;
+  const int n_launch = (int)(env_hi - A.env_lo);
+  if constexpr (DYN) {
+    if (wave >= A.claim_w || wave >= A.n_claims) return;
+    int c0, c1;
+    dma_claim((int)wave, n_launch, A.gpw, A.n_claims, A.n_full, A.n_top, 2 * A.claim_w, c0, c1);
+    env0 = A.env_lo + c0;
+    env1 = A.env_lo + c1;
+  } else {
+    env0 = A.env_lo + wave * A.gpw;
+    if (env0 >= env_hi) return;
+    env1 = env0 + A.gpw < env_hi ? env0 + A.gpw : env_hi;
+  }
   const int n_tiles = (int)(env1 - env0) * T;
+  unsigned tkv = 0;
+  auto request_ticket = [&]() {
+    if (lane == 0)
+      asm volatile("global_atomic_add %0, %1, %2, off sc0" : "=&v"(tkv) : "v"(A.claim_ctr), "v"(1u) : "memory");
+  };
 
   unsigned char* const tile = smem_raw + (size_t)wave_in_wg * TILE;
   const size_t env_stride = (size_t)K * (R * ESZ);
@@ -184,6 +235,7 @@
     unsigned o16 = lane16, o4 = lane4;
     if (NFULL) asm volatile("" : "+v"(o16));
     if (NREM) asm volatile("" : "+v"(o4));
+    if constexpr (DYN) rows = __builtin_amdgcn_readfirstlane(rows);
     asm volatile("" : "+s"(rows));
     if (rows == TROWS) {
       dma_pieces<0, NFULL, 16, 1024>(g, o16, tile);
@@ -285,6 +337,9 @@
     return q;
   };
 
+  if constexpr (DYN) {
+    if (env0 + 1 == env1) request_ticket();
+  }
   fetch_env(env0);
   issue_tile(envb, rows_of(0));
 
@@ -384,7 +439,36 @@
   };
   const bool adopt_early = OUT || T == 1;
 
-  for (int g = 0; g < n_tiles; ++g) {
+  auto write_results = [&]() {
+    if (lane < (int)(env1 - env0) && !RCG_DBG(A, 2)) {
+      const long bb = env0 + lane;
+#pragma unroll
+      for (int c = 0; c < DU; ++c)
+        if (A.action_out) A.action_out[(long)c * B + bb] = resU[c];
+      if (A.best_J) A.best_J[bb] = resJ;
+      if (A.best_idx) A.best_idx[bb] = resI;
+      if (A.accum) atomicAdd(&A.accum[bb], resAcc);
+      if (A.step_idx) atomicAdd(&A.step_idx[bb], 1);
+    }
+  };
+  long nenv0 = 0, nenv1 = 0;
+  bool more = false;
+  auto env_done = [&]() -> bool {
+    t = 0;
+    if constexpr (DYN) {
+      if (b + 1 == env1) {
+        write_results();
+        if (!more) return false;
+        env0 = nenv0;
+        env1 = nenv1;
+        b = env0;
+        return true;
+      }
+    }
+    ++b;
+    return true;
+  };
+  for (int g = 0; DYN || g < n_tiles; ++g) {
     if (t == 0) {
       if constexpr (!OUT) {
         if (env_pars) pre_env = Sys::template prepare<real>(pn);
@@ -392,7 +476,10 @@
       if (adopt_early) adopt_regs();
     }
     if constexpr (RCG_DMA_PRIO > 0 && ESZ == 8) __builtin_amdgcn_s_setprio(RCG_DMA_PRIO);
-    asm volatile("s_waitcnt vmcnt(0)" ::: "memory");
+    if constexpr (DYN)
+      asm volatile("s_waitcnt vmcnt(0)" : "+v"(tkv)::"memory");
+    else
+      asm volatile("s_waitcnt vmcnt(0)" ::: "memory");
     real rows[RPL][R];
 #pragma unroll
     for (int j = 0; j < RPL; ++j) {
@@ -402,7 +489,33 @@
     }
     asm volatile("s_waitcnt lgkmcnt(0)" ::: "memory");
     __builtin_amdgcn_wave_barrier();
-    if (g + 1 < n_tiles) {
+    if constexpr (DYN) {
+      if (t == T - 1) {
+        long nb = b + 1, nend = env1;
+        more = true;
+        if (nb == env1) {
+          const unsigned raw = (unsigned)__builtin_amdgcn_readfirstlane((int)tkv);
+          if (raw == (unsigned)(A.n_claims - 1) && lane == 0)
+            __hip_atomic_store(A.claim_ctr, 0u, __ATOMIC_RELAXED, __HIP_MEMORY_SCOPE_AGENT);
+          const unsigned tk = raw + (unsigned)A.claim_w;
+          more = tk < (unsigned)A.n_claims;
+          if (more) {
+            int c0, c1;
+            dma_claim((int)tk, n_launch, A.gpw, A.n_claims, A.n_full, A.n_top, 2 * A.claim_w, c0, c1);
+            nb = nenv0 = A.env_lo + c0;
+            nend = nenv1 = A.env_lo + c1;
+          }
+        }
+        if (more) {
+          if (nb + 1 == nend) request_ticket();
+          fetch_env(nb);
+          envb += (size_t)(nb - b) * env_stride;
+          issue_tile(envb, rows_of(0));
+        }
+      } else {
+        issue_tile(envb + (size_t)(t + 1) * TILE, rows_of(t + 1));
+      }
+    } else if (g + 1 < n_tiles) {
       if (t == T - 1) {
         fetch_env(b + 1);
         envb += env_stride;
@@ -515,7 +628,7 @@
 
       const int k = t * TROWS + j * 64 + lane;
       const bool has_row = k < K;
-      if (A.J && has_row) jstage[(A.jwave ? (int)(b - env0) * K : 0) + k] = J;
+      if (!DYN && A.J && has_row) jstage[(A.jwave ? (int)(b - env0) * K : 0) + k] = J;
       const real Jc = (J != J) ? inf_r<real>() : J;
       if (has_row && (Jc < bestJ || bestI == 0x7fffffff)) {
         bestJ = Jc;
@@ -525,7 +638,7 @@
       }
     }
 
-    if (A.J && (A.jwave ? g == n_tiles - 1 : t == T - 1)) {
+    if (!DYN && A.J && (A.jwave ? g == n_tiles - 1 : t == T - 1)) {
       asm volatile("s_waitcnt lgkmcnt(0)" ::: "memory");
       __builtin_amdgcn_wave_barrier();
       real* const Jout = A.J + (A.jwave ? env0 : b) * K;
@@ -544,8 +657,7 @@
       if (RCG_DBG(A, 2)) {
         if (bestJ == (real)-12345.678f) A.best_J[b] = bestJ;
         if (lane == 0 && A.step_idx) atomicAdd(&A.step_idx[b], 1);
-        t = 0;
-        ++b;
+        if (!env_done()) return;
         continue;
       }
       if constexpr (ZW != 0u)
@@ -571,21 +683,10 @@
 #pragma unroll
         for (int c = 0; c < DU; ++c) resU[c] = bu[c];
       }
-      t = 0;
-      ++b;
-    }
-  }
-
-  if (lane < (int)(env1 - env0) && !RCG_DBG(A, 2)) {
-    const long bb = env0 + lane;
-#pragma unroll
-    for (int c = 0; c < DU; ++c)
-      if (A.action_out) A.action_out[(long)c * B + bb] = resU[c];
-    if (A.best_J) A.best_J[bb] = resJ;
-    if (A.best_idx) A.best_idx[bb] = resI;
-    if (A.accum) atomicAdd(&A.accum[bb], resAcc);
-    if (A.step_idx) atomicAdd(&A.step_idx[bb], 1);
-  }
+      if (!env_done()) return;
+    }
+  }
+  if constexpr (!DYN) write_results();
 }
 
 #if !defined(__HIPCC_RTC__)
diff --git a/rcognita_amd/csrc/rcg_api.hip b/rcognita_amd/csrc/rcg_api.hip
--- a/rcognita_amd/csrc/rcg_api.hip
+++ b/rcognita_amd/csrc/rcg_api.hip
@@ -258,6 +258,7 @@
   h->split_pending = false;
   h->sub_lo = h->sub_hi = 0;
   h->probe = 0;
+  h->n_cu = 0;
   h->d_summary = nullptr;
   h->d_const = nullptr;
   h->fit_scratch = nullptr;
@@ -316,6 +317,12 @@
       rcg_destroy(h);
       return RCG_ERR_HIP;
     }
+  }
+
+  if (hipDeviceGetAttribute(&h->n_cu, hipDeviceAttributeMultiprocessorCount, cfg->device) != hipSuccess || h->n_cu < 1) {
+    rcg_fail(nullptr, RCG_ERR_HIP, "rcg_create: the device's compute-unit count");
+    rcg_destroy(h);
+    return RCG_ERR_HIP;
   }
 
   const size_t B = (size_t)cfg->batch, e = h->esz;
@@ -1271,6 +1278,13 @@
   return RCG_OK;
 }
 
+int rcg_last_launch_claims(const rcg_handle* h, int32_t kind, int32_t* claims, int32_t* waves) {
+  if (!h || kind < 0 || kind >= RCG_KERNEL_COUNT_) return RCG_ERR_BAD_ARG;
+  if (claims) *claims = h->last[kind].claims;
+  if (waves) *waves = h->last[kind].waves;
+  return RCG_OK;
+}
+
 const char* rcg_kernel_name(int32_t kernel_id) {
   static const char* const names[RCG_KID_COUNT_] = {"none",        "k_actor",   "k_actor_dma", "k_ticks",    "k_actor_opt",
                                                     "k_nominal",   "k_sim",     "k_sim_v",     "k_sim_dist", "k_critic_fit",
diff --git a/rcognita_amd/csrc/rcg_dma_launch.hpp b/rcognita_amd/csrc/rcg_dma_launch.hpp
--- a/rcognita_amd/csrc/rcg_dma_launch.hpp
+++ b/rcognita_amd/csrc/rcg_dma_launch.hpp
@@ -32,6 +32,19 @@
     RCG_DMA_LAUNCH((k_actor_dma<Sys, real, R, ((V) >= DMA_MPC_GEND ? true : Sys::TGT), V>))
       if constexpr (GROUP == 0) {
         constexpr unsigned ZWP = dma_zw_preset<Sys, real>();
+        if (A.claim_ctr) {
+          if constexpr (ZWP != 0u) {
+            if (dma_zero_w<real>(ZWP, variant, A, P) != 0u)
+              RCG_DMA_LAUNCH((k_actor_dma<Sys, real, R, Sys::TGT, DMA_MPC_G1, ZWP, true>))
+          }
+          switch (variant) {
+            case DMA_MPC_G1:
+              RCG_DMA_LAUNCH((k_actor_dma<Sys, real, R, Sys::TGT, DMA_MPC_G1, 0u, true>))
+            case DMA_MPC:
+              RCG_DMA_LAUNCH((k_actor_dma<Sys, real, R, Sys::TGT, DMA_MPC, 0u, true>))
+          }
+          return false;
+        }
         if constexpr (ZWP != 0u) {
           if (dma_zero_w<real>(ZWP, variant, A, P) != 0u) RCG_DMA_LAUNCH((k_actor_dma<Sys, real, R, Sys::TGT, DMA_MPC_G1, ZWP>))
         }
diff --git a/rcognita_amd/csrc/rcg_handle.hpp b/rcognita_amd/csrc/rcg_handle.hpp
--- a/rcognita_amd/csrc/rcg_handle.hpp
+++ b/rcognita_amd/csrc/rcg_handle.hpp
@@ -69,10 +69,12 @@
   hipEvent_t split_fork, split_join[2];
   bool split_pending;
   int sub_lo, sub_hi;
+  int n_cu;
   int probe;
   struct LastLaunch {
     int32_t kernel_id, variant, envs_per_wave;
     uint32_t zero_w;
+    int32_t claims, waves;
   } last[RCG_KERNEL_COUNT_];
 };
 static constexpr size_t kProfMaxSamples = 65536;
@@ -85,9 +87,14 @@
   h->last[kind].variant = variant | (h->sub_hi > 0 ? kVariantSplitBit : 0);
   h->last[kind].envs_per_wave = envs_per_wave;
   h->last[kind].zero_w = 0u;
-}
-
-static constexpr size_t kConstR64 = 512, kConstW = 1296, kConstBytes = 2256;
+  h->last[kind].claims = h->last[kind].waves = 0;
+}
+
+static constexpr size_t kConstR64 = 512, kConstW = 1296, kConstClaim = 2304, kConstBytes = 2496;
+static inline unsigned* claim_counter(const rcg_handle* h) {
+  const int part = h->sub_hi > 0 ? (h->sub_lo > 0 ? 2 : 1) : 0;
+  return reinterpret_cast<unsigned*>((unsigned char*)h->d_const + kConstClaim + (size_t)64 * part);
+}
 static constexpr int kFitMaxRows = 8;
 
 int rcg_fail(rcg_handle* h, int code, const char* fmt, ...);
diff --git a/rcognita_amd/csrc/rcg_kernels.hpp b/rcognita_amd/csrc/rcg_kernels.hpp
--- a/rcognita_amd/csrc/rcg_kernels.hpp
+++ b/rcognita_amd/csrc/rcg_kernels.hpp
@@ -310,6 +310,9 @@
   uint32_t* sim_status;
   int sim_n_sub;
   int obs_x;
+  unsigned* claim_ctr;
+  int claim_w;
+  int n_claims, n_full, n_top;
 };
 
 typedef float v4f __attribute__((ext_vector_type(4)));
diff --git a/rcognita_amd/csrc/rcg_rtc.hip b/rcognita_amd/csrc/rcg_rtc.hip
--- a/rcognita_amd/csrc/rcg_rtc.hip
+++ b/rcognita_amd/csrc/rcg_rtc.hip
@@ -176,10 +176,11 @@
          ">";
 }
 template <typename real>
-std::string expr_dma(bool packed, int R, int variant, bool sys_tgt, unsigned zw) {
+std::string expr_dma(bool packed, int R, int variant, bool sys_tgt, unsigned zw, bool dyn) {
   const bool tgt = (!packed && variant >= DMA_MPC_GEND) ? true : sys_tgt;
   return std::string(packed ? "rcg::k_actor_dma_packed<" : "rcg::k_actor_dma<") + kSysExpr + ", " + real_name<real>() + ", " +
-         std::to_string(R) + ", " + tf(tgt) + ", " + std::to_string(variant) + (zw ? ", " + std::to_string(zw) + "u>" : ">");
+         std::to_string(R) + ", " + tf(tgt) + ", " + std::to_string(variant) +
+         (dyn ? ", " + std::to_string(zw) + "u, true>" : (zw ? ", " + std::to_string(zw) + "u>" : ">"));
 }
 
 template <typename real>
@@ -254,15 +255,15 @@
 }
 
 template <typename real>
-int dma_function(rcg_handle* h, bool packed, int R, int variant, unsigned zw, hipFunction_t* fn) {
+int dma_function(rcg_handle* h, bool packed, int R, int variant, unsigned zw, bool dyn, hipFunction_t* fn) {
   RtcSystem& S = *const_cast<RtcSystem*>(h->rtc);
-  const std::string expr = expr_dma<real>(packed, R, variant, S.tgt, zw);
+  const std::string expr = expr_dma<real>(packed, R, variant, S.tgt, zw, dyn);
   auto hit = h->rtc_fn.find(expr);
   if (hit != h->rtc_fn.end()) {
     *fn = hit->second;
     return RCG_OK;
   }
-  const auto key = std::make_tuple(sizeof(real) == 8 ? 1 : 0, packed ? 1 : 0, R, variant | (zw ? 256 : 0));
+  const auto key = std::make_tuple(sizeof(real) == 8 ? 1 : 0, packed ? 1 : 0, R, variant | (zw ? 256 : 0) | (dyn ? 512 : 0));
   bool have;
   {
     std::lock_guard<std::mutex> lock(g_mu);
@@ -468,7 +469,7 @@
   p->dma = !p->packed && L.dma_ok;
   const RtcSystem& S = *h->rtc;
   p->zero_w = (p->dma && sizeof(real) == 8 && !S.dims.has_out) ? dma_zero_w<real>(S.zw, L.variant, A, params<real>(h)) : 0u;
-  if (p->packed || p->dma) return dma_function<real>(h, p->packed, L.R, L.variant, p->zero_w, &p->f);
+  if (p->packed || p->dma) return dma_function<real>(h, p->packed, L.R, L.variant, p->zero_w, p->dma && L.dma_w > 0, &p->f);
   return core_function<real>(h, expr_actor<real>(L.long_row || L.generic, L.tgt, streamed, L.long_row), &p->f);
 }
 
@@ -513,6 +514,10 @@
     if (rc == RCG_OK) {
       note_launch(h, RCG_KERNEL_ACTOR, RCG_KID_ACTOR_DMA, L.variant, (int)L.dma_gpw);
       h->last[RCG_KERNEL_ACTOR].zero_w = pick.zero_w;
+      h->last[RCG_KERNEL_ACTOR].claims = L.dma_claims;
+      h->last[RCG_KERNEL_ACTOR].waves = L.dma_w;
+    } else if (Ad.claim_ctr) {
+      (void)hipMemsetAsync(Ad.claim_ctr, 0, sizeof(unsigned), h->stream);
     }
     return rc;
   }
diff --git a/rcognita_amd/csrc/rcg_sysops.hpp b/rcognita_amd/csrc/rcg_sysops.hpp
--- a/rcognita_amd/csrc/rcg_sysops.hpp
+++ b/rcognita_amd/csrc/rcg_sysops.hpp
@@ -327,6 +327,8 @@
   int dma_min_k = 33;
   bool no_tick_fuse = false;
   bool no_pk = false;
+  bool dma_static = false;
+  int dma_waves = 0;
 };
 static inline const DevKnobs& dev_knobs() {
   static const DevKnobs k = [] {
@@ -346,6 +348,8 @@
     v.no_tick_fuse = getenv("RCG_NO_TICK_FUSE") != nullptr;
     if (const char* e = getenv("RCG_DMA_MINK")) v.dma_min_k = atoi(e);
     if (const char* e = getenv("RCG_FIT_LANES")) v.fit_lanes = atoi(e);
+    v.dma_static = getenv("RCG_DMA_STATIC") != nullptr;
+    if (const char* e = getenv("RCG_DMA_WAVES")) v.dma_waves = atoi(e);
 #endif
     return v;
   }();
@@ -376,6 +380,7 @@
   dim3 dma_grid;
   size_t dma_lds;
   int dma_jwave;
+  int dma_w, dma_claims, dma_full, dma_top;
 };
 
 template <typename real>
@@ -520,6 +525,15 @@
     L.dma_grid = dim3((unsigned)((pw + 3) / 4));
     L.dma_lds = lds_req;
     L.dma_jwave = jwave;
+    L.dma_w = L.dma_claims = L.dma_full = L.dma_top = 0;
+    if (variant <= DMA_MPC && !A.J && !knobs.dma_static && h->n_cu > 0) {
+      long w = (long)per_cu * 4 * h->n_cu;
+      if (w > pw) w = pw;
+      if (knobs.dma_waves > 0 && w > knobs.dma_waves) w = knobs.dma_waves;
+      L.dma_w = (int)w;
+      dma_claim_plan((int)Bn, (int)gpw, L.dma_w, &L.dma_claims, &L.dma_full, &L.dma_top);
+      L.dma_grid = dim3((unsigned)((w + 3) / 4));
+    }
   }
   return RCG_OK;
 }
@@ -546,6 +560,13 @@
   Ad.env_lo = h->sub_lo;
   Ad.env_hi = h->sub_hi;
   Ad.jwave = L.dma_jwave;
+  if (L.dma_w > 0) {
+    Ad.claim_ctr = claim_counter(h);
+    Ad.claim_w = L.dma_w;
+    Ad.n_claims = L.dma_claims;
+    Ad.n_full = L.dma_full;
+    Ad.n_top = L.dma_top;
+  }
   return Ad;
 }
 
@@ -626,6 +647,10 @@
     if (ok) {
       note_launch(h, RCG_KERNEL_ACTOR, RCG_KID_ACTOR_DMA, variant, (int)L.dma_gpw);
       h->last[RCG_KERNEL_ACTOR].zero_w = dma_zero_w<real>(dma_zw_preset<Sys, real>(), variant, Ad, P);
+      h->last[RCG_KERNEL_ACTOR].claims = L.dma_claims;
+      h->last[RCG_KERNEL_ACTOR].waves = L.dma_w;
+      if (Ad.claim_ctr && hipPeekAtLastError() != hipSuccess)
+        (void)hipMemsetAsync(Ad.claim_ctr, 0, sizeof(unsigned), h->stream);
       HIPCHK(h, hipGetLastError());
       return RCG_OK;
     }
diff --git a/rcognita_amd/engine.py b/rcognita_amd/engine.py
--- a/rcognita_amd/engine.py
+++ b/rcognita_amd/engine.py
@@ -771,3 +771,8 @@
         m = C.c_uint32()
         N.check(N.lib().rcg_last_launch_zero_w(self._h, int(kind), C.byref(m)), self._h)
         return int(m.value)
+
+    def last_launch_claims(self, kind=N.KERNEL_ACTOR):
+        c, w = C.c_int32(), C.c_int32()
+        N.check(N.lib().rcg_last_launch_claims(self._h, int(kind), C.byref(c), C.byref(w)), self._h)
+        return int(c.value), int(w.value)
```

Result: slower. 138.8 million (-14.5%).
